# CGLemon/Sayuri

Hardware: AMD Instinct MI355X
Metric: nn_evals_per_sec (higher is better)
Workload: dtype f16

## Files before the change

include/sayuri_hip.h:

```cpp
#ifndef SAYURI_HIP_H
#define SAYURI_HIP_H

#include <stddef.h>
#include <stdint.h>

#ifdef __cplusplus
extern "C" {
#endif

typedef struct sayuri_hip_ctx sayuri_hip_ctx;

enum {
    SAYURI_ACT_IDENTITY = 0, SAYURI_ACT_RELU = 1, SAYURI_ACT_ELU = 2, SAYURI_ACT_SELU = 3,
    SAYURI_ACT_GELU = 4, SAYURI_ACT_MISH = 5, SAYURI_ACT_SWISH = 6, SAYURI_ACT_HARDSWISH = 7
};

enum {
    SAYURI_BLOCK_RESIDUAL = 1, SAYURI_BLOCK_BOTTLENECK = 2, SAYURI_BLOCK_NESTED_BOTTLENECK = 3,
    SAYURI_BLOCK_MIXER = 4
};

typedef struct {
    int32_t type;
    int32_t apply_se;
// ... 42 lines not shown
enum { SAYURI_HIP_LATENCY = 1 };
sayuri_hip_ctx* sayuri_hip_create_ex(int device, const sayuri_hip_netdesc* desc, int max_batch,
                                     int board, int use_fp16, unsigned flags);

int sayuri_hip_load_tensor(sayuri_hip_ctx* ctx, int layer_id, int kind, const float* host, size_t n);

int sayuri_hip_forward(sayuri_hip_ctx* ctx, int n, const float* planes, const int* board_sizes,
                       float* prob, float* pass, float* misc, float* own);

int sayuri_hip_upload(sayuri_hip_ctx* ctx, int n, const float* planes, const int* board_sizes);
int sayuri_hip_run(sayuri_hip_ctx* ctx);
int sayuri_hip_sync(sayuri_hip_ctx* ctx);
int sayuri_hip_download(sayuri_hip_ctx* ctx, float* prob, float* pass, float* misc, float* own);

int sayuri_hip_submit(sayuri_hip_ctx* ctx, int n, const float* planes, const int* board_sizes, float* prob,
                      float* pass, float* misc, float* own, int* ticket);
int sayuri_hip_forward_packed(sayuri_hip_ctx* ctx, int n, const unsigned* records, int binary_planes, const int* board_sizes,
                              float* prob, float* pass, float* misc, float* own);
int sayuri_hip_submit_packed(sayuri_hip_ctx* ctx, int n, const unsigned* records, int binary_planes, const int* board_sizes,
                             float* prob, float* pass, float* misc, float* own, int* ticket);
int sayuri_hip_forward_packed_symm(sayuri_hip_ctx* ctx, int n, const unsigned* records, int n_records, int binary_planes,
                                   const int* board_sizes, const int* src, const int* symm, float* prob, float* pass,
                                   float* misc, float* own);
int sayuri_hip_submit_packed_symm(sayuri_hip_ctx* ctx, int n, const unsigned* records, int n_records, int binary_planes,
                                  const int* board_sizes, const int* src, const int* symm, float* prob, float* pass,
                                  float* misc, float* own, int* ticket);
int sayuri_hip_wait(sayuri_hip_ctx* ctx, int ticket);
int sayuri_hip_query(sayuri_hip_ctx* ctx, int ticket);

int sayuri_hip_time_runs(sayuri_hip_ctx* ctx, int iters, float* total_ms);

typedef struct {
    char name[48];
    int32_t launches;
    float total_ms;
    double flops;
    double bytes;
} sayuri_hip_kernel_stat;
int sayuri_hip_profile_run(sayuri_hip_ctx* ctx, sayuri_hip_kernel_stat* rows, int cap);

int sayuri_hip_mark_kernel(sayuri_hip_ctx* ctx, const char* name);
int sayuri_hip_timed_stat(sayuri_hip_ctx* ctx, sayuri_hip_kernel_stat* row);

void* sayuri_hip_host_alloc(size_t bytes);
void sayuri_hip_host_free(void* p);

size_t sayuri_hip_device_bytes(const sayuri_hip_ctx* ctx);

int sayuri_hip_last_chains(const sayuri_hip_ctx* ctx);

int sayuri_hip_tower_state(const sayuri_hip_ctx* ctx);

int sayuri_hip_latency_state(const sayuri_hip_ctx* ctx);

void sayuri_hip_destroy(sayuri_hip_ctx* ctx);

const char* sayuri_hip_last_error(void);

int sayuri_hip_test_conv(int device, int use_fp16, int n, const int* board_sizes, int max_board,
                         int cin, int cout, int k, int depthwise, int act, int post_residual,
                         const float* x, const float* w, const float* bias, const float* res,
                         float* y);
int sayuri_hip_test_conv_split(int device, int n, const int* board_sizes, int max_board, int cin, int cout, int act,
                               const float* x, const float* w, const float* bias, const float* res, float* y,
                               int channel_tiles, int strips);
int sayuri_hip_test_last_conv_kind(void);
int sayuri_hip_test_se_unit(int device, int use_fp16, int n, const int* board_sizes, int max_board, int channels,
                            int se_size, int act, const float* x, const float* res, const float* w1, const float* b1,
                            const float* w2, const float* b2, float* y, float* gate);
int sayuri_hip_test_head_tail(int device, int use_fp16, int n, const int* board_sizes, int max_board, int policy_channels,
                              int value_channels, int prob_channels, int pass_outs, int misc_outs, int act,
                              const float* pconv, const float* vconv, const float* const* weights12, float* prob,
                              float* pass, float* misc, float* own);

int sayuri_hip_test_conv_se(int device, int n, const int* board_sizes, int max_board, int channels, int se_size, int act,
                            int via_tower, const float* x, const float* w, const float* bias, const float* res, const float* w1,
                            const float* b1, const float* w2, const float* b2, float* y);
int sayuri_hip_test_last_se_form(void);
int sayuri_hip_test_tower_run(int device, int n, const int* board_sizes, int max_board, int channels, int cin0, int nlayers,
                              const int* act, const int* res_from, const float* w, const float* bias, int se_layer, int se_size,
                              const float* w1, const float* b1, const float* w2, const float* b2, int chain, const float* x,
                              float* y);
int sayuri_hip_test_last_tower_run(int out[3]);
int sayuri_hip_test_conv_sx(int device, int n, const int* board_sizes, int max_board, int channels, int se_size, int act,
                            const float* x, const float* w, const float* bias, const float* res, const float* w1,
                            const float* b1, const float* w2, const float* b2, float* y);
int sayuri_hip_test_last_sx_kts(void);
int sayuri_hip_test_head_board(int device, int n, const int* board_sizes, int max_board, int channels, int policy_channels,
                               int value_channels, int prob_channels, int pass_outs, int misc_outs, int act, const float* trunk,
                               const float* p_w, const float* p_b, const float* v_w, const float* v_b,
                               const float* const* weights12, float* prob, float* pass, float* misc, float* own);

#ifdef __cplusplus
}
#endif
#endif
```

sayuri_amd/_lib.py:

```python
from __future__ import annotations

import ctypes
import os

from . import _build

c_float_p = ctypes.POINTER(ctypes.c_float)
c_int_p = ctypes.POINTER(ctypes.c_int)


class KernelStat(ctypes.Structure):
    _fields_ = [("name", ctypes.c_char * 48), ("launches", ctypes.c_int32), ("total_ms", ctypes.c_float),
                ("flops", ctypes.c_double), ("bytes", ctypes.c_double)]


class BlockDesc(ctypes.Structure):
    _fields_ = [(n, ctypes.c_int32) for n in ("type", "apply_se", "se_size", "bottleneck_channels", "feedforward_channels", "dw_filter")]


class NetDesc(ctypes.Structure):
    _fields_ = [(n, ctypes.c_int32) for n in ("version", "input_channels", "residual_channels", "residual_blocks", "policy_head_channels",
                                              "value_head_channels", "probabilities_channels", "pass_probability_outputs",
                                              "ownership_channels", "value_misc_outputs", "default_act", "policy_head_type",
                                              "policy_dw_filter")] + [("blocks", ctypes.POINTER(BlockDesc))]


def fp(a):
    return a.ctypes.data_as(c_float_p)


def ip(a):
    return a.ctypes.data_as(c_int_p)


_I, _U, _Z, _V, _F, _IP = ctypes.c_int, ctypes.c_uint, ctypes.c_size_t, ctypes.c_void_p, c_float_p, c_int_p
_OUT = [_F] * 4
_STAT = ctypes.POINTER(KernelStat)
_W12 = ctypes.POINTER(c_float_p)
HIP_ABI = {
    "sayuri_hip_device_count": (_I, []),
    "sayuri_hip_create": (_V, [_I, _V, _I, _I, _I]),
    "sayuri_hip_create_ex": (_V, [_I, _V, _I, _I, _I, _U]),
    "sayuri_hip_load_tensor": (_I, [_V, _I, _I, _F, _Z]),
    "sayuri_hip_forward": (_I, [_V, _I, _F, _IP] + _OUT),
    "sayuri_hip_upload": (_I, [_V, _I, _F, _IP]),
    "sayuri_hip_run": (_I, [_V]),
    "sayuri_hip_sync": (_I, [_V]),
    "sayuri_hip_download": (_I, [_V] + _OUT),
    "sayuri_hip_submit": (_I, [_V, _I, _F, _IP] + _OUT + [_IP]),
    "sayuri_hip_forward_packed": (_I, [_V, _I, _V, _I, _IP] + _OUT),
    "sayuri_hip_submit_packed": (_I, [_V, _I, _V, _I, _IP] + _OUT + [_IP]),
    "sayuri_hip_forward_packed_symm": (_I, [_V, _I, _V, _I, _I, _IP, _IP, _IP] + _OUT),
    "sayuri_hip_submit_packed_symm": (_I, [_V, _I, _V, _I, _I, _IP, _IP, _IP] + _OUT + [_IP]),
    "sayuri_hip_wait": (_I, [_V, _I]),
    "sayuri_hip_query": (_I, [_V, _I]),
    "sayuri_hip_time_runs": (_I, [_V, _I, _F]),
    "sayuri_hip_profile_run": (_I, [_V, _STAT, _I]),
    "sayuri_hip_mark_kernel": (_I, [_V, ctypes.c_char_p]),
    "sayuri_hip_timed_stat": (_I, [_V, _STAT]),
    "sayuri_hip_host_alloc": (_V, [_Z]),
    "sayuri_hip_host_free": (None, [_V]),
    "sayuri_hip_device_bytes": (_Z, [_V]),
    "sayuri_hip_last_chains": (_I, [_V]),
    "sayuri_hip_tower_state": (_I, [_V]),
    "sayuri_hip_latency_state": (_I, [_V]),
    "sayuri_hip_destroy": (None, [_V]),
    "sayuri_hip_last_error": (ctypes.c_char_p, []),
    "sayuri_hip_test_conv": (_I, [_I] * 3 + [_IP] + [_I] * 7 + [_F] * 5),
    "sayuri_hip_test_conv_split": (_I, [_I] * 2 + [_IP] + [_I] * 4 + [_F] * 5 + [_I] * 2),
    "sayuri_hip_test_last_conv_kind": (_I, []),
    "sayuri_hip_test_se_unit": (_I, [_I] * 3 + [_IP] + [_I] * 4 + [_F] * 8),
    "sayuri_hip_test_head_tail": (_I, [_I] * 3 + [_IP] + [_I] * 7 + [_F, _F, _W12] + _OUT),
    "sayuri_hip_test_conv_se": (_I, [_I] * 2 + [_IP] + [_I] * 5 + [_F] * 9),
    "sayuri_hip_test_last_se_form": (_I, []),
    "sayuri_hip_test_tower_run": (_I, [_I] * 2 + [_IP] + [_I] * 4 + [_IP, _IP, _F, _F, _I, _I] + [_F] * 4 + [_I, _F, _F]),
    "sayuri_hip_test_last_tower_run": (_I, [_IP]),
    "sayuri_hip_test_conv_sx": (_I, [_I] * 2 + [_IP] + [_I] * 4 + [_F] * 9),
    "sayuri_hip_test_last_sx_kts": (_I, []),
    "sayuri_hip_test_head_board": (_I, [_I] * 2 + [_IP] + [_I] * 8 + [_F] * 5 + [_W12] + _OUT),
}
HIP_SYMBOLS = list(HIP_ABI)

_hip = None
_host = None


def _require(path: str) -> str:
    if not os.path.exists(path):
        raise RuntimeError(
            f"native library {path} is missing: run `python -c 'import __graft_entry__ as g; g.build()'` "
            "(there is no CPU fallback for the MI355X forward pipe)")
    return path


def hip() -> ctypes.CDLL:
    global _hip
    if _hip is None:
        path = _build.HIP_SO
        fake = os.environ.get("SAYURI_FAKE_HIP_LIB")
        if fake:
            import sys
            print(f"[sayuri_amd] SAYURI_FAKE_HIP_LIB is set: the device side is the test stand-in {fake}, NOT the MI355X engine",
                  file=sys.stderr)
            path = fake
        lib = ctypes.CDLL(_require(path), mode=ctypes.RTLD_GLOBAL)
        for name, (restype, argtypes) in HIP_ABI.items():
            if hasattr(lib, name):
                fn = getattr(lib, name)
                fn.restype, fn.argtypes = restype, argtypes
        _hip = lib
    return _hip


def host() -> ctypes.CDLL:
    global _host
    if _host is None:
        hip()
        lib = ctypes.CDLL(_require(_build.HOST_SO))
        lib.sayuri_host_last_error.restype = ctypes.c_char_p
        lib.sayuri_weights_load.restype = ctypes.c_void_p
        lib.sayuri_weights_load.argtypes = [ctypes.c_char_p]
        lib.sayuri_weights_free.argtypes = [ctypes.c_void_p]
        lib.sayuri_weights_info.argtypes = [ctypes.c_void_p, c_int_p]
        lib.sayuri_weights_block_info.argtypes = [ctypes.c_void_p, ctypes.c_int, c_int_p]
        lib.sayuri_weights_tensor.restype = ctypes.c_long
        lib.sayuri_weights_tensor.argtypes = [ctypes.c_void_p, ctypes.c_char_p, c_float_p, ctypes.c_long]
        lib.sayuri_pipe_create.restype = ctypes.c_void_p
        lib.sayuri_pipe_create.argtypes = [ctypes.c_char_p, ctypes.c_int, ctypes.c_int, ctypes.c_int, ctypes.c_int,
                                           ctypes.c_int]
        lib.sayuri_pipe_create_ex.restype = ctypes.c_void_p
        lib.sayuri_pipe_create_ex.argtypes = [ctypes.c_char_p, ctypes.c_int, ctypes.c_int, ctypes.c_int, ctypes.c_int,
                                              ctypes.c_int, ctypes.c_uint]
        lib.sayuri_pipe_create_ens.restype = ctypes.c_void_p
        lib.sayuri_pipe_create_ens.argtypes = [ctypes.c_char_p, ctypes.c_int, ctypes.c_int, ctypes.c_int, ctypes.c_int,
                                               ctypes.c_int, ctypes.c_uint, ctypes.c_int]
        lib.sayuri_pipe_accepts_ensemble.argtypes = [ctypes.c_void_p]
        lib.sayuri_pipe_ensemble_fallbacks.restype = ctypes.c_long
        lib.sayuri_pipe_ensemble_fallbacks.argtypes = [ctypes.c_void_p]
        lib.sayuri_pipe_forward_ensemble.argtypes = [ctypes.c_void_p, c_float_p, ctypes.c_int, ctypes.c_float, ctypes.c_int, c_float_p]
        lib.sayuri_pipe_ensemble_mix.argtypes = [ctypes.c_void_p, ctypes.c_int, c_float_p, c_int_p, c_float_p, c_int_p, c_int_p,
                                                 ctypes.c_int, c_float_p, c_int_p]
        lib.sayuri_packed_symmetry.argtypes = [ctypes.c_void_p, ctypes.c_int, ctypes.c_int, ctypes.c_int, ctypes.c_void_p]
        lib.sayuri_pipe_destroy.argtypes = [ctypes.c_void_p]
        lib.sayuri_pipe_num_workers.argtypes = [ctypes.c_void_p]
        lib.sayuri_pipe_ctx.restype = ctypes.c_void_p
        lib.sayuri_pipe_ctx.argtypes = [ctypes.c_void_p, ctypes.c_int]
        lib.sayuri_pipe_reconstruct.argtypes = [ctypes.c_void_p, ctypes.c_int, ctypes.c_int]
        lib.sayuri_pipe_eval.argtypes = [ctypes.c_void_p, ctypes.c_int, ctypes.c_int, ctypes.c_int, c_float_p,
                                         c_int_p, c_float_p, c_int_p, c_float_p]
        lib.sayuri_pipe_pump_times.restype = None
        lib.sayuri_pipe_pump_times.argtypes = [ctypes.c_void_p, ctypes.POINTER(ctypes.c_double),
                                               ctypes.POINTER(ctypes.c_long), ctypes.POINTER(ctypes.c_long)]
        lib.sayuri_pipe_netbench.argtypes = [ctypes.c_void_p, ctypes.c_int, ctypes.c_double, ctypes.c_int,
                                             ctypes.POINTER(ctypes.c_double), ctypes.POINTER(ctypes.c_long)]
        _host = lib
    return _host
```

sayuri_amd/csrc/hip/conv_board.h:

```cpp
#pragma once
#include "common.h"
#include "conv_glds.h"
#include "conv_mfma.h"
#include "small_ops.h"

namespace sayuri {

constexpr int kBoardCols = 24;
constexpr int kBoardPT = kBoardCols * 16;
constexpr int kBoardMaxPos = 512;
constexpr int kBoardMaxSub = 32;
constexpr int kBoardNJ = kBoardCols / 2;
constexpr int kBoardLdsBytes = 160 * 1024;
constexpr int kBoardWaveLds = kBoardLdsBytes / 8;

__host__ __device__ constexpr int board_row_channel(int row) {
    return (row & ~31) + 8 * ((row & 15) >> 2) + 4 * ((row >> 4) & 1) + (row & 3);
}

struct BoardParams {
    ConvParams c;
    const int* tab_src;
    const int2* tab_pix;
    const int* tab_cols;
    int npos;
    int uniform_info;
    unsigned long long* dbg;
    int arith;
    const void* w_next;
    int w_ready;
    int row_order;
};

struct BoardPack {
    int px = 0, pos = 0, cnt = 0, bs0 = 0;
    __host__ __device__ bool fits(int bs) const {
        return (cnt == 0 || bs == bs0) && cnt < kBoardMaxSub && px + bs * bs <= kBoardPT &&
               pos + (bs + 2) * (bs + 2) <= kBoardMaxPos;
    }
    __host__ __device__ void add(int bs) { px += bs * bs; pos += (bs + 2) * (bs + 2); ++cnt; bs0 = bs; }
};

__global__ __launch_bounds__(256) void board_setup_kernel(BatchGeom g, int npos, int* __restrict__ tab_src,
                                                          int2* __restrict__ tab_pix, int* __restrict__ tab_cols) {
    __shared__ int sub[kBoardMaxSub][4];
    __shared__ int hdr[2];
    const int tile = blockIdx.x, tid = threadIdx.x;
    if (tid == 0) {
        int t = 0, s = 0;
        BoardPack pk;
        int cnt = 0;
        for (; s < g.n_samples; ++s) {
            const int bs = g.bsz[s];
            if (pk.cnt > 0 && !pk.fits(bs)) {
                if (t == tile) break;
                ++t;
                pk = BoardPack{};
            }
            if (t == tile) {
                sub[cnt][0] = pk.pos; sub[cnt][1] = pk.px; sub[cnt][2] = bs; sub[cnt][3] = s;
                ++cnt;
            }
            pk.add(bs);
        }
        hdr[0] = cnt;
        hdr[1] = cnt > 0 ? sub[cnt - 1][1] + sub[cnt - 1][2] * sub[cnt - 1][2] : 0;
        tab_cols[tile] = ((hdr[1] + 15) / 16) | (sub[0][2] << 8);
    }
    __syncthreads();
    const int nsub = hdr[0], npx = hdr[1];
    for (int pos = tid; pos < npos; pos += blockDim.x) {
        int src = -1;
        for (int s = 0; s < nsub; ++s) {
            const int bs = sub[s][2], w2 = bs + 2, rel = pos - sub[s][0];
            if (rel >= 0 && rel < w2 * w2) {
                const int r = rel / w2, xc = rel - r * w2;
                const int y = r - 1, x = xc - 1;
                if (y >= 0 && y < bs && x >= 0 && x < bs) src = sub[s][3] * g.slot_pix + y * bs + x;
                break;
            }
        }
        tab_src[(size_t)tile * npos + pos] = src;
    }
    for (int i = tid; i < kBoardPT; i += blockDim.x) {
        int lstr = sub[0][2] + 2, lpos = lstr + 1, orow = -1;
        if (i < npx) {
            for (int s = 0; s < nsub; ++s) {
                const int bs = sub[s][2], pp = i - sub[s][1];
                if (pp >= 0 && pp < bs * bs) {
                    const int y = pp / bs, x = pp - y * bs;
                    lstr = bs + 2;
                    lpos = sub[s][0] + (y + 1) * (bs + 2) + x + 1;
                    orow = sub[s][3] * g.slot_pix + pp;
                    break;
                }
            }
        }
        tab_pix[(size_t)tile * kBoardPT + i] = make_int2(lpos | (lstr << 16), orow);
    }
}

template <int WMT_> struct BoardCfg {
    static constexpr int WMT = WMT_, WAVM = 4, WAVN = 2, NWAVE = 8, NJ = kBoardNJ;
    static constexpr int KO_T = WAVM * WMT * 16;
    static constexpr int A_TAP_BYTES = KO_T * 64;
    static constexpr int A_BYTES = 3 * A_TAP_BYTES;
    static constexpr int A_INSTR = KO_T / 16;
    static constexpr int AI = (A_INSTR + NWAVE - 1) / NWAVE;
    static constexpr int KO_PARTS = KO_T / 64;
    static constexpr size_t ring_bytes(int npos) { return 2 * (size_t)A_BYTES + 2 * (size_t)npos * 64; }
    static constexpr size_t lds_bytes(int npos) { return ring_bytes(npos) <= kBoardLdsBytes ? kBoardLdsBytes : ring_bytes(npos); }
};

#ifndef SAYURI_DROP_STREAM
#define SAYURI_DROP_STREAM 0
#endif
template <int OFF> __device__ __forceinline__ void board_read_a(f16x8& dst, uint32_t addr) {
    if constexpr (SAYURI_DROP_STREAM == 1) asm volatile("" : "+v"(dst) : "v"(addr));
    else ds_read16<OFF>(dst, addr);
}
template <int OFF> __device__ __forceinline__ void board_read_b(f16x8& dst, uint32_t addr) {
    if constexpr (SAYURI_DROP_STREAM == 2) asm volatile("" : "+v"(dst) : "v"(addr));
    else ds_read16<OFF>(dst, addr);
}

namespace board_sched {
constexpr int kNB = 3 * kBoardNJ;
template <int WMT> constexpr int late_a(int b) { return (b >= 0 && b % kBoardNJ == kBoardNJ - 1 && b / kBoardNJ < 2) ? WMT : 0; }
template <int WMT> constexpr int young_b(int b) {
    if (b < 2) return 2;
    return late_a<WMT>(b - 2) + (b + 1 < kNB ? 1 : 0) + late_a<WMT>(b - 1) + (b + 2 < kNB ? 1 : 0);
}
}

template <int N> __device__ __forceinline__ void wait_lgkm1(f16x8& a) {
    asm volatile("s_waitcnt lgkmcnt(%1)" : "+v"(a) : "n"(N));
}
template <int N> __device__ __forceinline__ void wait_lgkm2(f16x8& a, f16x8& b) {
    asm volatile("s_waitcnt lgkmcnt(%2)" : "+v"(a), "+v"(b) : "n"(N));
}
template <int N, int NF, int NA> __device__ __forceinline__ void wait_lgkm_all(f16x8 (&a)[NA], f16x8& b) {
    static_assert(NF >= 2 && NF <= 4 && NF <= NA, "2..4 A fragments per tap");
    if constexpr (NF == 2) asm volatile("s_waitcnt lgkmcnt(%3)" : "+v"(a[0]), "+v"(a[1]), "+v"(b) : "n"(N));
    else if constexpr (NF == 3) asm volatile("s_waitcnt lgkmcnt(%4)" : "+v"(a[0]), "+v"(a[1]), "+v"(a[2]), "+v"(b) : "n"(N));
    else asm volatile("s_waitcnt lgkmcnt(%5)" : "+v"(a[0]), "+v"(a[1]), "+v"(a[2]), "+v"(a[3]), "+v"(b) : "n"(N));
}

__device__ __forceinline__ void swap16(f32x4& a, f32x4& b) {
    float a0 = a[0], a1 = a[1], a2 = a[2], a3 = a[3], b0 = b[0], b1 = b[1], b2 = b[2], b3 = b[3];
    asm("s_nop 1\n\tv_permlane16_swap_b32 %0, %4\n\tv_permlane16_swap_b32 %1, %5\n\tv_permlane16_swap_b32 %2, %6\n\t"
        "v_permlane16_swap_b32 %3, %7"
        : "+v"(a0), "+v"(a1), "+v"(a2), "+v"(a3), "+v"(b0), "+v"(b1), "+v"(b2), "+v"(b3));
    a = f32x4{a0, a1, a2, a3};
    b = f32x4{b0, b1, b2, b3};
}

typedef float f32x2 __attribute__((ext_vector_type(2)));
__device__ __forceinline__ f32x2 mish2(f32x2 x) {
    const f32x2 xl = x * 1.4426950408889634f;
    f32x2 e;
    e[0] = __builtin_amdgcn_exp2f(xl[0]);
    e[1] = __builtin_amdgcn_exp2f(xl[1]);
    const f32x2 t = __builtin_elementwise_fma(e, e + 2.f, f32x2{2.f, 2.f});
    f32x2 r;
    r[0] = __builtin_amdgcn_rcpf(t[0]);
    r[1] = __builtin_amdgcn_rcpf(t[1]);
    return x * __builtin_elementwise_fma(r, f32x2{-2.f, -2.f}, f32x2{1.f, 1.f});
}

__device__ __forceinline__ void mma_agpr(f32x4& acc, const f16x8& a, const f16x8& b) {
    asm volatile("v_mfma_f32_16x16x32_f16 %0, %1, %2, %0" : "+a"(acc) : "v"(a), "v"(b));
}
__device__ __forceinline__ void mma_vgpr(f32x4& acc, const f16x8& a, const f16x8& b) {
    asm volatile("v_mfma_f32_16x16x32_f16 %0, %1, %2, %0" : "+v"(acc) : "v"(a), "v"(b));
}
template <int WMT, int I, int J> __device__ __forceinline__ void mma_tile(f32x4& acc, const f16x8& a, const f16x8& b) {
    if constexpr (WMT * J + I < 32) mma_agpr(acc, a, b);
    else mma_vgpr(acc, a, b);
}

__device__ __forceinline__ void glds16_s(uint32_t voff, const void* sbase, uint32_t lds_dst) {
    unsigned keep;
    asm volatile("s_mov_b32 %0, m0\n\ts_mov_b32 m0, %3\n\ts_nop 4\n\tglobal_load_lds_dwordx4 %1, %2\n\ts_mov_b32 m0, %0"
                 : "=&s"(keep)
                 : "v"(voff), "s"(sbase), "s"(lds_dst)
                 : "memory");
}

__device__ __forceinline__ void gload16_s(f16x8& dst, uint32_t voff, const void* sbase) {
    asm volatile("global_load_dwordx4 %0, %1, %2" : "=v"(dst) : "v"(voff), "s"(sbase) : "memory");
}

template <int N, int ND, int NA> __device__ __forceinline__ void wait_vm_regs(f16x8 (&r)[NA]) {
    static_assert(ND == 0 || ND == 2 || ND == 4, "0, 2 or 4 register pieces");
    if constexpr (ND == 4) asm volatile("s_waitcnt vmcnt(%4)" : "+v"(r[0]), "+v"(r[1]), "+v"(r[2]), "+v"(r[3]) : "n"(N) : "memory");
    else if constexpr (ND == 2) asm volatile("s_waitcnt vmcnt(%2)" : "+v"(r[0]), "+v"(r[1]) : "n"(N) : "memory");
    else asm volatile("s_waitcnt vmcnt(%0)" ::"n"(N) : "memory");
}

template <int WMT, bool DBG = false, int CHAIN = 0>
__device__ __forceinline__ void board_mainloop(const BoardParams& bp, unsigned char* smem, f32x4 (&acc)[WMT][kBoardNJ], int tile,
                                               int kt, int wave, int lane, int col0, bool full, int bs,
                                               unsigned long long* dbg = nullptr,
                                               const __attribute__((address_space(4))) BoardParams* chain = nullptr) {
    using Cfg = BoardCfg<WMT>;
    using namespace board_sched;
    constexpr int KO_T = Cfg::KO_T, NJ = Cfg::NJ, AI = Cfg::AI, NA = WMT;
    const ConvParams& p = bp.c;
    const int npos = bp.npos, b_bytes = npos * 64;
    const uint32_t a_ring = (uint32_t)(uintptr_t)smem;
    const uint32_t b_ring = a_ring + 2 * Cfg::A_BYTES;
    const int wave_m = wave & 3;
    const int kg = lane >> 4;
    const int ls16 = (bs + 2) * 16;

    const unsigned char* gin0 = (const unsigned char*)p.in - kZeroPrefix;
    const unsigned char* gw = (const unsigned char*)p.w;
    const int nbinstr = npos / 64 * 4;
    const int nchunks = p.cin_s / kChunk;
    const int ngroups = nchunks * 3;
    const uint32_t lane16 = lane * 16;
    const size_t tap_stride = (size_t)nchunks * 4 * p.ko_pad * 16;
    const size_t chunk_stride = (size_t)4 * p.ko_pad * 16;
    auto issue_a = [&](int G, int dx, int i) {
        const int q = wave + 8 * i;
        if (q >= Cfg::A_INSTR) return;
        const int kgq = q / Cfg::KO_PARTS, part = q % Cfg::KO_PARTS;
        const int chunk = G / 3, row = G - chunk * 3;
        const unsigned char* base = gw + (size_t)(row * 3 + dx) * tap_stride + (size_t)chunk * chunk_stride +
                                    (size_t)((kgq * p.ko_pad + kt * KO_T + part * 64) * 16);
        glds16_s(lane16, base, a_ring + (G & 1) * Cfg::A_BYTES + dx * Cfg::A_TAP_BYTES + (kgq * KO_T + part * 64) * 16);
    };
    if (!CHAIN || !bp.w_ready) {
#pragma unroll
        for (int dx = 0; dx < 3; ++dx)
#pragma unroll
            for (int i = 0; i < AI; ++i) issue_a(0, dx, i);
    }

    int src[4];
    int lp[NJ];
    if (bp.arith) {
        const int w2 = bs + 2, npix = bs * bs;
        const float r_w2 = __builtin_amdgcn_rcpf((float)w2), r_bs = __builtin_amdgcn_rcpf((float)bs);
#pragma unroll
        for (int i = 0; i < 4; ++i) {
            const int q = wave + 8 * i, pos = (q >> 2) * 64 + lane;
            const int r = (int)(((float)pos + 0.5f) * r_w2), xc = pos - r * w2;
            const bool in = q < nbinstr && r >= 1 && r <= bs && xc >= 1 && xc <= bs;
            src[i] = in ? tile * p.g.slot_pix + (r - 1) * bs + (xc - 1) : -1;
        }
#pragma unroll
        for (int j = 0; j < NJ; ++j) {
            const int px = (col0 + j) * 16 + (lane & 15);
            const int y = (int)(((float)px + 0.5f) * r_bs), x = px - y * bs;
            lp[j] = px < npix ? (y + 1) * w2 + x + 1 : w2 + 1;
        }
    } else {
#pragma unroll
        for (int i = 0; i < 4; ++i) {
            const int q = wave + 8 * i;
            src[i] = q < nbinstr ? bp.tab_src[(size_t)tile * npos + (q >> 2) * 64 + lane] : -1;
        }
#pragma unroll
        for (int j = 0; j < NJ; ++j) lp[j] = bp.tab_pix[(size_t)tile * kBoardPT + (col0 + j) * 16 + (lane & 15)].x;
    }
    f32x4 b4[WMT];
#pragma unroll
    for (int i = 0; i < WMT; ++i) b4[i] = *(const f32x4*)(p.bias + kt * KO_T + (wave_m * WMT + i) * 16 + 4 * kg);

    uint32_t boff[4];
#pragma unroll
    for (int i = 0; i < 4; ++i)
        boff[i] = (src[i] >= 0 ? (uint32_t)kZeroPrefix + (uint32_t)src[i] * (uint32_t)(p.cin_s * 2) : 0u) + ((wave + 8 * i) & 3) * 16;
    auto issue_b = [&](int chunk, int i) {
        const int q = wave + 8 * i;
        if (q >= nbinstr) return;
        glds16_s(boff[i], gin0 + chunk * (kChunk * 2), b_ring + (chunk & 1) * b_bytes + ((q & 3) * npos + (q >> 2) * 64) * 16);
    };
#pragma unroll
    for (int i = 0; i < 4; ++i) issue_b(0, i);

    uint32_t bb[NJ];
#pragma unroll
    for (int j = 0; j < NJ; ++j)
        bb[j] = b_ring + (((uint32_t)lp[j] & 0xffffu) - 1) * 16 + (uint32_t)kg * npos * 16 - ls16;
#pragma unroll
    for (int i = 0; i < WMT; ++i)
#pragma unroll
        for (int j = 0; j < NJ; ++j) acc[i][j] = b4[i];

    const uint32_t arow_off = (uint32_t)((kg * KO_T + wave_m * WMT * 16 + (lane & 15)) * 16);
    unsigned long long t_sync = 0;
    if constexpr (DBG) { if (dbg) dbg[1] = __builtin_amdgcn_s_memtime(); }

    for (int chunk = 0; chunk < nchunks; ++chunk) {
        const bool more_b = chunk + 1 < nchunks;
        static_for<3>([&](auto rowc) {
            constexpr int row = decltype(rowc)::value;
            const int G = chunk * 3 + row;
            unsigned long long t0 = 0;
            if constexpr (DBG) t0 = __builtin_amdgcn_s_memtime();
            wait_vmcnt<0>();
            __builtin_amdgcn_s_barrier();
            if constexpr (DBG) {
                const unsigned long long t1 = __builtin_amdgcn_s_memtime();
                t_sync += t1 - t0;
                if (dbg && G == 0) dbg[2] = t1;
            }
            bool more_a = G + 1 < ngroups;
            int Gn = G + 1;
            if constexpr (CHAIN == 2 && row == 2) {
                if (!more_a) {
                    const __attribute__((address_space(4))) BoardParams* bq = chain;
                    asm volatile("" : "+s"(bq));
                    const unsigned char* wn = (const unsigned char*)bq->w_next;
                    asm volatile("s_waitcnt lgkmcnt(0)" : "+s"(wn)::"memory");
                    if (wn) { gw = wn; Gn = 0; more_a = true; }
                }
            }
            const uint32_t abase = a_ring + (G & 1) * Cfg::A_BYTES + arow_off;
#if SAYURI_DROP_STREAM
            f16x8 afr[NA] = {}, bfr[3] = {};
#else
            f16x8 afr[NA], bfr[3];
#endif
            board_read_b<0>(bfr[0], bb[0]);
            static_for<WMT>([&](auto ic) {
                constexpr int i = decltype(ic)::value;
                board_read_a<i * 256>(afr[i], abase);
            });
            board_read_b<0>(bfr[1], bb[1]);
            static_for<kNB>([&](auto bc) {
                constexpr int b = decltype(bc)::value;
                constexpr int dx = b / NJ, j = b % NJ;
                if constexpr (b % 3 == 0 && b / 3 < 3 * AI) {
                    if (more_a) issue_a(Gn, (b / 3) / AI, (b / 3) % AI);
                }
                if constexpr ((b == 1 || b == 4) && row < 2) {
                    if (more_b) issue_b(chunk + 1, row * 2 + (b == 4 ? 1 : 0));
                }
                if constexpr (b + 2 < kNB) {
                    constexpr int b2 = b + 2;
                    board_read_b<16 * (b2 / NJ)>(bfr[b2 % 3], bb[b2 % NJ]);
                }
                if constexpr (b == 0) wait_lgkm_all<young_b<WMT>(0), WMT>(afr, bfr[0]);
                else if constexpr (j > 0) wait_lgkm1<young_b<WMT>(b)>(bfr[b % 3]);
                static_for<WMT>([&](auto ic) {
                    constexpr int i = decltype(ic)::value;
                    if constexpr (j == 0 && dx > 0) wait_lgkm2<WMT - i>(afr[i], bfr[b % 3]);
                    if constexpr (j == NJ - 1) {
                        if (full) mma_tile<WMT, i, j>(acc[i][j], afr[i], bfr[b % 3]);
                    } else {
                        mma_tile<WMT, i, j>(acc[i][j], afr[i], bfr[b % 3]);
                    }
                    if constexpr (j == NJ - 1 && dx < 2)
                        board_read_a<(dx + 1) * Cfg::A_TAP_BYTES + i * 256>(afr[i], abase);
                });
            });
            const int delta = row < 2 ? ls16 : ((chunk & 1) ? -b_bytes : b_bytes) - 2 * ls16;
#pragma unroll
            for (int j = 0; j < NJ; ++j) bb[j] += (uint32_t)delta;
        });
    }
    asm volatile("s_nop 15\n\ts_nop 15" ::: "memory");
    if constexpr (DBG) { if (dbg) { dbg[3] = __builtin_amdgcn_s_memtime(); dbg[5] = t_sync; } }
}

template <int ACT> __device__ __forceinline__ f16x8 board_act8(const float (&v)[8]) {
    f16x8 h;
    if constexpr (ACT == kMish) {
#pragma unroll
        for (int q = 0; q < 8; q += 2) {
            const f32x2 y = mish2(f32x2{v[q], v[q + 1]});
            h[q] = (f16)y[0];
            h[q + 1] = (f16)y[1];
        }
    } else {
#pragma unroll
        for (int q = 0; q < 8; ++q) h[q] = (f16)activate(v[q], ACT);
    }
    return h;
}

template <int ACT>
__device__ __forceinline__ void board_store_pair(f32x4 a, f32x4 b, bool with_res, const f16x8& rr, unsigned char* __restrict__ gbase,
                                                 uint32_t voff, bool ok) {
    swap16(a, b);
    float v[8] = {a[0], a[1], a[2], a[3], b[0], b[1], b[2], b[3]};
    if (with_res) {
#pragma unroll
        for (int q = 0; q < 8; ++q) v[q] += (float)rr[q];
    }
    const f16x8 h = board_act8<ACT>(v);
    if (ok) *(f16x8*)(gbase + voff) = h;
}

template <int WMT, int ACT>
__device__ __forceinline__ void board_epilogue(const BoardParams& bp, unsigned char* smem, f32x4 (&acc)[WMT][kBoardNJ], int tile, int kt,
                                               int wave, int lane, int col0, int nj) {
    using Cfg = BoardCfg<WMT>;
    constexpr int NJ = Cfg::NJ, NPAIR = WMT / 2;
    constexpr bool LONE = (WMT & 1) != 0;
    const ConvParams& p = bp.c;
    const int R = lane >> 4, px = lane & 15, wave_m = wave & 3;
    const f16* __restrict__ gres = (const f16*)p.res;
    f16* __restrict__ gout = (f16*)p.out;
    const int ko_w = kt * Cfg::KO_T + wave_m * WMT * 16;
    const int2* pix = bp.tab_pix + (size_t)tile * kBoardPT + col0 * 16 + px;
    int cb[NPAIR > 0 ? NPAIR : 1];
#pragma unroll
    for (int pr = 0; pr < NPAIR; ++pr) cb[pr] = ko_w + (2 * pr + (R & 1)) * 16 + (R >> 1) * 8;

    if constexpr (!LONE) {
        constexpr int kWaveLds = kBoardWaveLds, kLdsPieces = kWaveLds / 1024;
        constexpr int kPieces = NJ * NPAIR;
        constexpr int ND = kPieces > kLdsPieces ? kPieces - kLdsPieces : 0;
        static_assert(ND % (NPAIR > 0 ? NPAIR : 1) == 0, "whole column tiles");
        int orow[NJ];
        f16x8 rrd[ND > 0 ? ND : 1];
        const bool with_res = gres != nullptr;
        int row_bytes = p.cout_s * 2;
        asm volatile("" : "+v"(row_bytes));
        uint32_t cb2[NPAIR > 0 ? NPAIR : 1];
        bool cok[NPAIR > 0 ? NPAIR : 1];
#pragma unroll
        for (int pr = 0; pr < NPAIR; ++pr) {
            cb2[pr] = (uint32_t)cb[pr] * 2u;
            cok[pr] = cb[pr] * 2 < row_bytes;
        }
        const uint32_t my_lds = (uint32_t)(uintptr_t)smem + wave * kWaveLds;
        constexpr int JH = NJ / 2, NRT = ND / NPAIR;
        auto load_orow = [&] {
            if (bp.arith) {
                const int npix = (bp.uniform_info >> 8) * (bp.uniform_info >> 8);
#pragma unroll
                for (int j = 0; j < NJ; ++j) {
                    const int pxl = (col0 + j) * 16 + px;
                    orow[j] = (j < nj && pxl < npix) ? tile * p.g.slot_pix + pxl : -1;
                }
            } else {
#pragma unroll
                for (int j = 0; j < NJ; ++j) orow[j] = j < nj ? pix[j * 16].y : -1;
#pragma unroll
                for (int j = 0; j < NJ; ++j) asm volatile("" : "+v"(orow[j]));
            }
        };
        auto lds_slot = [](int j, int pr) { return (j < JH ? j : j - NRT) * NPAIR + pr; };
        if (with_res) {
            asm volatile("s_waitcnt lgkmcnt(0)" ::: "memory");
            __builtin_amdgcn_s_barrier();
            load_orow();
            auto roff = [&](int j, int pr) -> uint32_t {
                return (orow[j] >= 0 && cb[pr] < p.cout_s) ? ((uint32_t)orow[j] * (uint32_t)p.cout_s + (uint32_t)cb[pr]) * 2u : 0u;
            };
            static_for<NJ>([&](auto jc) {
                constexpr int j = decltype(jc)::value;
                if constexpr (j < JH || j >= JH + NRT) {
                    if (j < nj) {
#pragma unroll
                        for (int pr = 0; pr < NPAIR; ++pr) glds16_s(roff(j, pr), gres, my_lds + lds_slot(j, pr) * 1024);
                    }
                }
            });
#pragma unroll
            for (int k = 0; k < ND; ++k)
                if (JH + k / NPAIR < nj) gload16_s(rrd[k], roff(JH + k / NPAIR, k % NPAIR), gres);
            const int late = (nj > JH ? nj - JH : 0) * NPAIR;
            static_for<(NJ - JH) + 1>([&](auto tc) {
                constexpr int t = decltype(tc)::value;
                if (late == t * NPAIR) asm volatile("s_waitcnt vmcnt(%0)" ::"n"(t * NPAIR) : "memory");
            });
        } else {
            load_orow();
        }
        static_for<NJ>([&](auto jc) {
            constexpr int j = decltype(jc)::value;
            if constexpr (j == JH) {
                if (with_res) wait_vm_regs<0, ND>(rrd);
            }
            if (j < nj) {
#pragma unroll
                for (int pr = 0; pr < NPAIR; ++pr) {
                    f16x8 rr = {0, 0, 0, 0, 0, 0, 0, 0};
                    if (with_res) {
                        if constexpr (j >= JH && j < JH + NRT) rr = rrd[(j - JH) * NPAIR + pr];
                        else rr = *(const f16x8*)(smem + wave * kWaveLds + lds_slot(j, pr) * 1024 + lane * 16);
                    }
                    board_store_pair<ACT>(acc[2 * pr][j], acc[2 * pr + 1][j], with_res, rr, (unsigned char*)gout,
                                          __umul24((unsigned)(orow[j] >= 0 ? orow[j] : 0), (unsigned)row_bytes) + cb2[pr], orow[j] >= 0 && cok[pr]);
                }
            }
        });
        return;
    }

    const int cl = ko_w + (WMT - 1) * 16 + 4 * R;
    auto res8 = [&](int orow, int pr) -> f16x8 {
        if (gres && orow >= 0 && cb[pr] < p.cout_s) return *(const f16x8*)(gres + (size_t)orow * p.cout_s + cb[pr]);
        return f16x8{0, 0, 0, 0, 0, 0, 0, 0};
    };
    auto res4 = [&](int orow) -> f16x4 {
        if (gres && orow >= 0 && cl < p.cout_s) return *(const f16x4*)(gres + (size_t)orow * p.cout_s + cl);
        return f16x4{0, 0, 0, 0};
    };
    int orow[3];
    f16x8 rr[2][NPAIR > 0 ? NPAIR : 1];
    f16x4 rl[2];
    orow[0] = nj > 0 ? pix[0].y : -1;
    orow[1] = nj > 1 ? pix[16].y : -1;
#pragma unroll
    for (int pr = 0; pr < NPAIR; ++pr) rr[0][pr] = res8(orow[0], pr);
    rl[0] = res4(orow[0]);
    static_for<NJ>([&](auto jc) {
        constexpr int j = decltype(jc)::value;
        if (j < nj) {
            if constexpr (j + 2 < NJ) orow[(j + 2) % 3] = j + 2 < nj ? pix[(j + 2) * 16].y : -1;
            if constexpr (j + 1 < NJ) {
#pragma unroll
                for (int pr = 0; pr < NPAIR; ++pr) rr[(j + 1) & 1][pr] = res8(orow[(j + 1) % 3], pr);
                rl[(j + 1) & 1] = res4(orow[(j + 1) % 3]);
            }
// ... 180 lines not shown
        __syncthreads();
        if (dbg) dbg[4] = __builtin_amdgcn_s_memtime();
    } else {
        for (int c = tid; c < C; c += 512) {
            const float mean = (psum[c] + psum[KO_T + c]) / npix;
            pool[c] = mean;
            pool[C + c] = mean * (bd / 10.f);
            pool[2 * C + c] = fmaxf(pmax[c], pmax[KO_T + c]);
        }
        __syncthreads();
        se_fc4<U>(sp.squeeze, pool, red, tid);
        __syncthreads();
        for (int o = tid; o < so; o += 512) {
            float a = sp.squeeze.b[o];
            const int parts = 512 / (so / 4);
            for (int k = 0; k < parts; ++k) a += red[k * so + o];
            mid[o] = activate(a, p.act);
        }
        __syncthreads();
        if (dbg) dbg[3] = __builtin_amdgcn_s_memtime();
        se_fc4<U>(sp.excite, mid, red, tid);
        __syncthreads();
        {
            const int eo = sp.excite.out, parts = 512 / (eo / 4);
            for (int o = tid; o < eo; o += 512) {
                float a = sp.excite.b[o];
                for (int k = 0; k < parts; ++k) a += red[k * eo + o];
                gate[o < C ? o : KO_T + (o - C)] = o < C ? 1.0f / (1.0f + fast_exp(-a)) : a;
            }
        }
        __syncthreads();
        if (dbg) dbg[4] = __builtin_amdgcn_s_memtime();
    }
}

template <int WMT>
__device__ __forceinline__ void board_se_gate(const BoardSeParams& sp, unsigned char* smem, f32x4 (&acc)[WMT][kBoardNJ], int wave, int lane) {
    using Cfg = BoardCfg<WMT>;
    constexpr int NJ = Cfg::NJ, KO_T = Cfg::KO_T;
    const int q = lane >> 4, wave_m = wave & 3;
    const int w_bytes = sp.w1h != nullptr ? sp.w1_bytes + sp.w2_bytes : 0;
    const float* gate = (const float*)(smem + w_bytes + SeLds<WMT>::gate);
#pragma unroll
    for (int i = 0; i < WMT; ++i) {
        const int c0 = wave_m * WMT * 16 + i * 16 + 4 * q;
        const f32x4 g = *(const f32x4*)(gate + c0), be = *(const f32x4*)(gate + KO_T + c0);
        static_for<NJ>([&](auto jc) {
            constexpr int j = decltype(jc)::value;
#pragma unroll
            for (int r = 0; r < 4; ++r) acc[i][j][r] = __builtin_fmaf(g[r], acc[i][j][r], be[r]);
        });
    }
}

template <int WMT>
__device__ __forceinline__ void board_se_stage(const BoardSeParams& sp, unsigned char* smem, f32x4 (&acc)[WMT][kBoardNJ], int tile,
                                               int wave, int lane, int col0, int nj, int bs, unsigned long long* dbg = nullptr) {
    board_se_pool<WMT>(sp, smem, acc, tile, wave, lane, col0, nj, bs);
    board_se_fc<WMT>(sp, smem, wave * 64 + lane, bs, dbg);
    board_se_gate<WMT>(sp, smem, acc, wave, lane);
}

template <int WMT>
__global__ __launch_bounds__(512, 2) void conv_board_se_kernel(const BoardSeParams sp) {
    extern __shared__ __attribute__((aligned(16))) unsigned char smem[];
    const BoardParams& bp = sp.b;
    const ConvParams& p = bp.c;
    const int tid = threadIdx.x, lane = tid & 63;
    const int wave = __builtin_amdgcn_readfirstlane(tid >> 6);
    const int tile = blockIdx.x;
    const int info = bp.uniform_info >= 0 ? bp.uniform_info : __builtin_amdgcn_readfirstlane(bp.tab_cols[tile]);
    const int ncols = info & 0xff, bs = info >> 8;
    const int nj0 = (ncols + 1) >> 1;
    const int wave_n = wave >> 2;
    const int col0 = wave_n ? nj0 : 0;
    const int nj = wave_n ? ncols - nj0 : nj0;

    unsigned long long* dbg = nullptr;
    if (bp.dbg && blockIdx.x < 4 && lane == 0) {
        dbg = bp.dbg + ((size_t)blockIdx.x * 8 + wave) * 8;
        dbg[0] = __builtin_amdgcn_s_memtime();
    }
    f32x4 acc[WMT][kBoardNJ];
    board_mainloop<WMT>(bp, smem, acc, tile, 0, wave, lane, col0, nj == kBoardNJ, bs);
    if (dbg) dbg[1] = __builtin_amdgcn_s_memtime();
    board_se_stage<WMT>(sp, smem, acc, tile, wave, lane, col0, nj, bs, dbg);
    asm volatile("s_waitcnt lgkmcnt(0)" ::: "memory");
    __builtin_amdgcn_s_barrier();
    if (dbg) dbg[5] = __builtin_amdgcn_s_memtime();

    switch (p.act) {
    case kMish: board_epilogue<WMT, kMish>(bp, smem, acc, tile, 0, wave, lane, col0, nj); break;
    case kIdentity: board_epilogue<WMT, kIdentity>(bp, smem, acc, tile, 0, wave, lane, col0, nj); break;
    case kReLU: board_epilogue<WMT, kReLU>(bp, smem, acc, tile, 0, wave, lane, col0, nj); break;
    case kSwish: board_epilogue<WMT, kSwish>(bp, smem, acc, tile, 0, wave, lane, col0, nj); break;
    case kELU: board_epilogue<WMT, kELU>(bp, smem, acc, tile, 0, wave, lane, col0, nj); break;
    case kSELU: board_epilogue<WMT, kSELU>(bp, smem, acc, tile, 0, wave, lane, col0, nj); break;
    case kGELU: board_epilogue<WMT, kGELU>(bp, smem, acc, tile, 0, wave, lane, col0, nj); break;
    default: board_epilogue<WMT, kHardSwish>(bp, smem, acc, tile, 0, wave, lane, col0, nj); break;
    }
    if (dbg) {
        asm volatile("s_waitcnt vmcnt(0)" ::: "memory");
        dbg[6] = __builtin_amdgcn_s_memtime();
    }
}

template <int WMT, bool DBG = false>
__global__ __launch_bounds__(512, 2) void conv_board_kernel(const BoardParams bp) {
    extern __shared__ __attribute__((aligned(16))) unsigned char smem[];
    unsigned long long* dbg = nullptr;
    if constexpr (DBG) {
        if (bp.dbg && blockIdx.x < 4 && (threadIdx.x & 63) == 0) {
            dbg = bp.dbg + ((size_t)blockIdx.x * 8 + (threadIdx.x >> 6)) * 8;
            dbg[0] = __builtin_amdgcn_s_memtime();
        }
    }
    const ConvParams& p = bp.c;
    const int tid = threadIdx.x, lane = tid & 63;
    const int wave = __builtin_amdgcn_readfirstlane(tid >> 6);
    const int tile = p.npos + blockIdx.x % p.num_pix_tiles;
    const int kt = blockIdx.x / p.num_pix_tiles;
    const int info = bp.uniform_info >= 0 ? bp.uniform_info : __builtin_amdgcn_readfirstlane(bp.tab_cols[tile]);
    const int ncols = info & 0xff, bs = info >> 8;
    const int nj0 = (ncols + 1) >> 1;
    const int wave_n = wave >> 2;
    const int col0 = wave_n ? nj0 : 0;
    const int nj = wave_n ? ncols - nj0 : nj0;

    f32x4 acc[WMT][kBoardNJ];
    board_mainloop<WMT, DBG>(bp, smem, acc, tile, kt, wave, lane, col0, nj == kBoardNJ, bs, dbg);

    switch (p.act) {
    case kMish: board_epilogue<WMT, kMish>(bp, smem, acc, tile, kt, wave, lane, col0, nj); break;
    case kIdentity: board_epilogue<WMT, kIdentity>(bp, smem, acc, tile, kt, wave, lane, col0, nj); break;
    case kReLU: board_epilogue<WMT, kReLU>(bp, smem, acc, tile, kt, wave, lane, col0, nj); break;
    case kSwish: board_epilogue<WMT, kSwish>(bp, smem, acc, tile, kt, wave, lane, col0, nj); break;
    case kELU: board_epilogue<WMT, kELU>(bp, smem, acc, tile, kt, wave, lane, col0, nj); break;
    case kSELU: board_epilogue<WMT, kSELU>(bp, smem, acc, tile, kt, wave, lane, col0, nj); break;
    case kGELU: board_epilogue<WMT, kGELU>(bp, smem, acc, tile, kt, wave, lane, col0, nj); break;
    default: board_epilogue<WMT, kHardSwish>(bp, smem, acc, tile, kt, wave, lane, col0, nj); break;
    }
    if constexpr (DBG) {
        if (dbg) {
            asm volatile("s_waitcnt vmcnt(0)" ::: "memory");
            dbg[4] = __builtin_amdgcn_s_memtime();
        }
    }
}

}
```

sayuri_amd/csrc/hip/conv_board_sx.h:

```cpp
#pragma once
#include "conv_board.h"

namespace sayuri {

constexpr int kSxMaxSub = 4;
constexpr int kSxSlots = 128;
typedef __attribute__((address_space(1))) unsigned long long sx_gu64;

struct BoardSxParams {
    BoardParams b;
    const void* w1t;
    const void* w2t;
    int w1_bytes, w2_bytes;
    int nsizes;
    int se, kts;
    unsigned long long* xchg;
    unsigned epoch;
    unsigned* err;
    int dbg_stall;
};

struct SxLds {
    static constexpr int kPitch = 68;
    static constexpr int stage = 0, stage_bytes = kBoardPT * kPitch * 4;
    static constexpr int psum = stage + stage_bytes;
    static constexpr int pmax = psum + kSxMaxSub * 8 * 128 * 4;
    static constexpr int red = psum;
    static constexpr int pool = red + kSxMaxSub * 2048 * 4;
    static constexpr int part = pool + kSxMaxSub * 256 * 4;
    static constexpr int mid = part + 4 * kSxMaxSub * 128 * 4;
    static constexpr int gate = mid + kSxMaxSub * 128 * 4;
    static constexpr int end = gate + kSxMaxSub * 256 * 4;
};
static_assert(SxLds::end <= 160 * 1024, "the SE stage must fit the LDS");

__device__ __forceinline__ void sx_barrier() { asm volatile("s_waitcnt lgkmcnt(0)\n\ts_barrier" ::: "memory"); }

template <int WMT>
__global__ __launch_bounds__(512, 2) void conv_board_sx_kernel(const BoardSxParams sp) {
    static_assert(WMT == 2, "128-channel tiles");
    extern __shared__ __attribute__((aligned(16))) unsigned char smem[];
    using Cfg = BoardCfg<WMT>;
    constexpr int NJ = Cfg::NJ;
    const BoardParams& bp = sp.b;
    const ConvParams& p = bp.c;
    const int tid = threadIdx.x, lane = tid & 63;
    const int wave = __builtin_amdgcn_readfirstlane(tid >> 6);
    const int kts = sp.kts;
    const int grp = blockIdx.x / (8 * kts), rem = blockIdx.x - grp * 8 * kts;
    const int kt = rem >> 3, tl = grp * 8 + (rem & 7);
    if (tl >= p.num_pix_tiles) return;
    const int tile = p.npos + tl;
    const int info = bp.uniform_info >= 0 ? bp.uniform_info : __builtin_amdgcn_readfirstlane(bp.tab_cols[tile]);
    const int ncols = info & 0xff, bs = info >> 8;
    const int nj0 = (ncols + 1) >> 1;
    const int wave_m = wave & 3, wave_n = wave >> 2;
    const int col0 = wave_n ? nj0 : 0;
    const int nj = wave_n ? ncols - nj0 : nj0;
    const int npix = bs * bs;
    int nsub = (ncols * 16) / npix;
    nsub = nsub < 1 ? 1 : (nsub > kSxMaxSub ? kSxMaxSub : nsub);

    unsigned long long* dbg = nullptr;
    if (bp.dbg && tid == 0 && (blockIdx.x == 0 || blockIdx.x == 8 || blockIdx.x == 16 || blockIdx.x == 1)) {
        dbg = bp.dbg + (size_t)(blockIdx.x == 1 ? 3 : blockIdx.x >> 3) * 64;
        dbg[0] = __builtin_amdgcn_s_memtime();
    }
    f32x4 acc[WMT][kBoardNJ];
    board_mainloop<WMT>(bp, smem, acc, tile, kt, wave, lane, col0, nj == kBoardNJ, bs);
    if (dbg) dbg[1] = __builtin_amdgcn_s_memtime();

    float* stage = (float*)(smem + SxLds::stage);
    float* psum = (float*)(smem + SxLds::psum);
    float* pmax = (float*)(smem + SxLds::pmax);
    float* pool = (float*)(smem + SxLds::pool);
    float* red = (float*)(smem + SxLds::red);
    float* part = (float*)(smem + SxLds::part);
    float* mid = (float*)(smem + SxLds::mid);
    float* gate = (float*)(smem + SxLds::gate);
    const int q = lane >> 4, px = lane & 15;
    const int se = sp.se;

    const int quads = se >> 2, parts = min(32, 512 / quads);
    const int oq = tid % quads, pt = tid / quads;

    sx_barrier();
    const int per = (npix + 7) >> 3;
#pragma unroll
    for (int half = 0; half < 2; ++half) {
        if ((wave_m >> 1) == half) {
            static_for<NJ>([&](auto jc) {
                constexpr int j = decltype(jc)::value;
                if (j < nj) {
                    const int slot = (col0 + j) * 16 + px;
#pragma unroll
                    for (int i = 0; i < WMT; ++i)
                        *(f32x4*)(stage + slot * SxLds::kPitch + (wave_m & 1) * 32 + i * 16 + 4 * q) = acc[i][j];
                }
            });
        }
        sx_barrier();
        {
            const int c = lane, e = wave;
            const int p0 = e * per, p1 = min(npix, p0 + per);
            for (int s = 0; s < nsub; ++s) {
                const float* src = stage + (s * npix + p0) * SxLds::kPitch + c;
                float a = 0.f, m = -5000.f;
                int pp = p0;
                for (; pp + 8 <= p1; pp += 8) {
                    float v[8];
#pragma unroll
                    for (int u = 0; u < 8; ++u) v[u] = src[u * SxLds::kPitch];
                    src += 8 * SxLds::kPitch;
#pragma unroll
                    for (int u = 0; u < 8; ++u) { a += v[u]; m = max_raw(m, v[u]); }
                }
                for (; pp < p1; ++pp) {
                    const float v = *src;
                    src += SxLds::kPitch;
                    a += v;
                    m = max_raw(m, v);
                }
                psum[(s * 8 + e) * 128 + half * 64 + c] = a;
                pmax[(s * 8 + e) * 128 + half * 64 + c] = m;
            }
        }
        sx_barrier();
    }

    {
        const int n1 = sp.w1_bytes >> 10, n2 = sp.w2_bytes >> 10;
        const unsigned char* g1 = (const unsigned char*)sp.w1t + ((size_t)kt * sp.nsizes + (bs - 2)) * sp.w1_bytes;
        const unsigned char* g2 = (const unsigned char*)sp.w2t + (size_t)kt * sp.w2_bytes;
        const uint32_t l0 = (uint32_t)(uintptr_t)smem;
        for (int k = wave; k < n1; k += 8) glds16_s(lane * 16, g1 + k * 1024, l0 + k * 1024);
        for (int k = wave; k < n2; k += 8) glds16_s(lane * 16, g2 + k * 1024, l0 + sp.w1_bytes + k * 1024);
    }
    {
        const float inv = 1.0f / (float)npix;
        for (int k = tid; k < nsub * 128; k += 512) {
            const int s = k >> 7, c = k & 127;
            const float* a = psum + s * 8 * 128 + c;
            const float* m = pmax + s * 8 * 128 + c;
            float t = a[0], x = m[0];
#pragma unroll
            for (int e = 1; e < 8; ++e) { t += a[e * 128]; x = max_raw(x, m[e * 128]); }
            pool[s * 256 + c] = t * inv;
            pool[s * 256 + 128 + c] = x;
        }
    }
    asm volatile("s_waitcnt vmcnt(0)" ::: "memory");
    sx_barrier();
// ... 124 lines not shown
```

sayuri_amd/csrc/hip/conv_tower.h:

```cpp
#pragma once
#include "conv_board.h"

namespace sayuri {

constexpr int kTowerStride = 320;

struct alignas(16) TowerLayer {
    const TowerLayer* self;
    int last;
    int has_se;
    BoardSeParams sp;
    char pad[kTowerStride - 16 - sizeof(BoardSeParams)];
};
static_assert(sizeof(TowerLayer) == kTowerStride, "tower_seam.py steps the table by kTowerStride bytes");
static_assert(offsetof(TowerLayer, self) == 0, "the compiled bodies load their argument from s[0:1] + 0: the element itself");

typedef const __attribute__((address_space(4))) TowerLayer* TowerLayerCP;
__device__ __forceinline__ TowerLayerCP tower_launder(TowerLayerCP p) {
    asm volatile("" : "+s"(p));
    return p;
}

constexpr int kTowerFreeVgpr = 66;
constexpr int kTowerFreeSgprs = 64;
#define SAYURI_TOWER_CLOBBER_V                                                                                                            \
    "v66", "v67", "v68", "v69", "v70", "v71", "v72", "v73", "v74", "v75", "v76", "v77", "v78", "v79", "v80", "v81", "v82", "v83", "v84",   \
        "v85", "v86", "v87", "v88", "v89", "v90", "v91", "v92", "v93", "v94", "v95", "v96", "v97", "v98", "v99", "v100", "v101", "v102",  \
        "v103", "v104", "v105", "v106", "v107", "v108", "v109", "v110", "v111", "v112", "v113", "v114", "v115", "v116", "v117", "v118",   \
        "v119", "v120", "v121", "v122", "v123", "v124", "v125", "v126", "v127"
#define SAYURI_TOWER_CLOBBER_S                                                                                                            \
    "s0", "s1", "s2", "s3", "s4", "s5", "s6", "s7", "s8", "s9", "s10", "s11", "s12", "s13", "s14", "s15", "s16", "s17", "s18", "s19",     \
        "s20", "s21", "s22", "s23", "s24", "s25", "s26", "s27", "s28", "s29", "s30", "s31", "s32", "s33", "s34", "s35", "s36", "s37",     \
        "s38", "s39", "s40", "s41", "s42", "s43", "s44", "s45", "s46", "s47", "s48", "s49", "s50", "s51", "s52", "s53", "s54", "s55",     \
        "s56", "s57", "s58", "s59", "s60", "s61", "s62", "s63"

template <int WMT, int SIDE, int K> __device__ __forceinline__ void tower_anchor_tile(f32x4& t) {
    constexpr int i = K % WMT, j = K / WMT;
    if constexpr (K < 32) asm volatile("; TOWER_ACC %1 %2 %3 %0" : "+a"(t) : "n"(SIDE), "n"(i), "n"(j));
    else asm volatile("; TOWER_ACC %1 %2 %3 %0" : "+v"(t) : "n"(SIDE), "n"(i), "n"(j));
}
template <int WMT, int SIDE> __device__ __forceinline__ void tower_anchor(f32x4 (&acc)[WMT][kBoardNJ]) {
    static_for<WMT * kBoardNJ>([&](auto kc) {
        constexpr int k = decltype(kc)::value;
        tower_anchor_tile<WMT, SIDE, k>(acc[k % WMT][k / WMT]);
    });
}

template <int WMT>
__global__ __launch_bounds__(512, 2) void conv_tower_kernel(const TowerLayer* layer) {
    extern __shared__ __attribute__((aligned(16))) unsigned char smem[];
    const TowerLayerCP L = (TowerLayerCP)layer;
    const int tid = threadIdx.x, lane = tid & 63;
    const int wave = __builtin_amdgcn_readfirstlane(tid >> 6);
    const int tile = blockIdx.x;
    const int ui = L->sp.b.uniform_info;
    const int info = ui >= 0 ? ui : __builtin_amdgcn_readfirstlane(L->sp.b.tab_cols[tile]);
    const int ncols = info & 0xff, bs = info >> 8;
    const int nj0 = (ncols + 1) >> 1;
    const int wave_n = wave >> 2;
    const int col0 = wave_n ? nj0 : 0;
    const int nj = wave_n ? ncols - nj0 : nj0;

    f32x4 acc[WMT][kBoardNJ];
    {
        const BoardParams& bp = *(const BoardParams*)&L->sp.b;
        board_mainloop<WMT, false, 2>(bp, smem, acc, tile, 0, wave, lane, col0, nj == kBoardNJ, bs, nullptr,
                                      (const __attribute__((address_space(4))) BoardParams*)&L->sp.b);
    }
    TowerLayerCP L2 = L;
    int tid2 = tid;
    tower_anchor<WMT, 0>(acc);
    asm volatile("; TOWER_SE_HOOK elem=%0 tid=%1 wmt=%2 ui=%3 cols=%4 w1h=%5 w2h=%6 w1b=%7 w2b=%8 psum=%9 pmax=%10 gate=%11 kot=%12 "
                 "res=%13 out=%14 couts=%15 slotpix=%16 act=%17 arith=%18 mish=%19 roword=%20 relu=%21 identity=%22 "
                 "stride=%23 last=%24 hasse=%25 freev=%26 frees=%27 nj=%28 epilds=%29 lds=%30"
                 : "+s"(L2), "+v"(tid2)
                 : "n"(WMT), "n"(offsetof(TowerLayer, sp.b.uniform_info)), "n"(offsetof(TowerLayer, sp.b.tab_cols)),
                   "n"(offsetof(TowerLayer, sp.w1h)), "n"(offsetof(TowerLayer, sp.w2h)), "n"(offsetof(TowerLayer, sp.w1_bytes)),
                   "n"(offsetof(TowerLayer, sp.w2_bytes)), "n"(SeLds<WMT>::psum), "n"(SeLds<WMT>::pmax), "n"(SeLds<WMT>::gate),
                   "n"(BoardCfg<WMT>::KO_T), "n"(offsetof(TowerLayer, sp.b.c.res)), "n"(offsetof(TowerLayer, sp.b.c.out)),
                   "n"(offsetof(TowerLayer, sp.b.c.cout_s)), "n"(offsetof(TowerLayer, sp.b.c.g.slot_pix)), "n"(offsetof(TowerLayer, sp.b.c.act)),
                   "n"(offsetof(TowerLayer, sp.b.arith)), "n"((int)kMish), "n"(offsetof(TowerLayer, sp.b.row_order)), "n"((int)kReLU), "n"((int)kIdentity),
                   "n"(kTowerStride), "n"(offsetof(TowerLayer, last)), "n"(offsetof(TowerLayer, has_se)), "n"(kTowerFreeVgpr),
                   "n"(kTowerFreeSgprs), "n"(kBoardNJ), "n"(kBoardWaveLds), "n"(kBoardLdsBytes)
                 : "memory", "vcc", "scc", SAYURI_TOWER_CLOBBER_V, SAYURI_TOWER_CLOBBER_S);
    const BoardSeParams& sp = *(const BoardSeParams*)&L2->sp;
    const BoardParams& bp = sp.b;
    const int lane2 = tid2 & 63, wave2 = __builtin_amdgcn_readfirstlane(tid2 >> 6);
    const int ui2 = bp.uniform_info;
    const int info2 = ui2 >= 0 ? ui2 : __builtin_amdgcn_readfirstlane(bp.tab_cols[tile]);
    const int ncols2 = info2 & 0xff, nj02 = (ncols2 + 1) >> 1;
    const int col02 = (wave2 >> 2) ? nj02 : 0, nj2 = (wave2 >> 2) ? ncols2 - nj02 : nj02;
    switch (bp.c.act) {
    case kMish: board_epilogue<WMT, kMish>(bp, smem, acc, tile, 0, wave2, lane2, col02, nj2); break;
    case kIdentity: board_epilogue<WMT, kIdentity>(bp, smem, acc, tile, 0, wave2, lane2, col02, nj2); break;
    case kReLU: board_epilogue<WMT, kReLU>(bp, smem, acc, tile, 0, wave2, lane2, col02, nj2); break;
    case kSwish: board_epilogue<WMT, kSwish>(bp, smem, acc, tile, 0, wave2, lane2, col02, nj2); break;
    case kELU: board_epilogue<WMT, kELU>(bp, smem, acc, tile, 0, wave2, lane2, col02, nj2); break;
    case kSELU: board_epilogue<WMT, kSELU>(bp, smem, acc, tile, 0, wave2, lane2, col02, nj2); break;
    case kGELU: board_epilogue<WMT, kGELU>(bp, smem, acc, tile, 0, wave2, lane2, col02, nj2); break;
    default: board_epilogue<WMT, kHardSwish>(bp, smem, acc, tile, 0, wave2, lane2, col02, nj2); break;
    }
}

template <int WMT>
__global__ __launch_bounds__(512) void tower_se_fc_kernel(const TowerLayer* layer) {
    extern __shared__ __attribute__((aligned(16))) unsigned char smem[];
    const int tid = threadIdx.x, tile = blockIdx.x;
    const BoardSeParams& sp = layer->sp;
    const int ui = sp.b.uniform_info;
    const int info = ui >= 0 ? ui : __builtin_amdgcn_readfirstlane(sp.b.tab_cols[tile]);
    board_se_fc<WMT, 4>(sp, smem, tid, info >> 8);
}

}
```

sayuri_amd/csrc/hip/engine_graph.h:

```cpp
#pragma once
#include "engine_plan.h"

namespace sayuri {

struct SymmReq {
    int n_records = 0;
    const int* src = nullptr;
    const int* symm = nullptr;
};

class EngineBase {
public:
    virtual ~EngineBase() {}
    virtual int load_tensor(int layer, int kind, const float* host, size_t n) = 0;
    virtual int upload(int n, const float* planes, const int* board_sizes, const unsigned* packed = nullptr, int binary = 0,
                       const SymmReq* sy = nullptr) = 0;
    virtual int run() = 0;
    virtual int sync() = 0;
    virtual int download(float* prob, float* pass, float* misc, float* own) = 0;
    virtual int time_runs(int iters, float* ms) = 0;
    virtual int profile_run(sayuri_hip_kernel_stat* rows, int cap) = 0;
    virtual int submit(int n, const float* planes, const int* bsz, float* prob, float* pass, float* misc, float* own,
                       int* ticket, const unsigned* packed = nullptr, int binary = 0, const SymmReq* sy = nullptr) = 0;
    virtual int wait(int ticket) = 0;
// ... 844 lines not shown
            if (match) {
                group_counts_.back() += 1;
                light_flops_ = flops;
                light_bytes_ = bytes;
            }
            return 0;
        }
        HIP_OK(hipEventRecord(ev0_, f.stream));
        launch();
        HIP_OK(hipGetLastError());
        rows_reset();
        HIP_OK(hipEventRecord(ev1_, f.stream));
        HIP_OK(hipEventSynchronize(ev1_));
        float ms = 0.f;
        HIP_OK(hipEventElapsedTime(&ms, ev0_, ev1_));
        Stat& s = stats_[name];
        s.launches += 1;
        s.ms += ms;
        s.flops += flops;
        s.bytes += bytes;
        return 0;
    }

    int choose_tile(int wmt, int kot_tiles, TileChoice<T>* out) {
        auto it = tile_cache_.find(wmt * 1024 + kot_tiles);
        if (it != tile_cache_.end()) { *out = it->second; return 0; }
        if (!pick_tile<T>(geom_, wmt, kot_tiles, false, out)) return fail("no conv tile configuration fits this batch geometry");
        tile_cache_[wmt * 1024 + kot_tiles] = *out;
        return 0;
    }

    int tile_tabs(Fwd& f, const GldsEntry& e, const TileTabs** out) {
        TileTabs& t = f.io.tabs[e.wnt];
        if (!t.src) {
            const size_t max_tiles = ((size_t)max_batch_ * slot_pix_ + e.pt - 1) / e.pt;
            if (dev_alloc(&t.src, max_tiles * e.npos) || dev_alloc(&t.pix, max_tiles * e.pt)) return -1;
        }
        if (!t.fresh) {
            const int ntiles = (geom_.total + e.pt - 1) / e.pt;
            hipLaunchKernelGGL(e.setup, dim3(ntiles), dim3(256), 0, f.stream, dgeom(f.io), t.src, t.pix);
            HIP_OK(hipGetLastError());
            t.fresh = true;
        }
        *out = &t;
        return 0;
    }
    int board_tabs(Fwd& f, const BoardTabs** out) {
        BoardTabs& t = f.io.board;
        if (!t.src) {
            if (dev_alloc(&t.src, (size_t)max_batch_ * kBoardMaxPos) || dev_alloc(&t.pix, (size_t)max_batch_ * kBoardPT) ||
                dev_alloc(&t.cols, max_batch_))
                return -1;
        }
        if (!t.fresh || t.npos_built != board_plan_.npos || board_plan_.ntiles > t.ntiles_built) {
            hipLaunchKernelGGL(board_setup_kernel, dim3(board_plan_.ntiles), dim3(256), 0, f.stream, dgeom(f.io), board_plan_.npos, t.src,
                               t.pix, t.cols);
            HIP_OK(hipGetLastError());
            t.fresh = true;
            t.npos_built = board_plan_.npos;
            t.ntiles_built = board_plan_.ntiles;
        }
        *out = &t;
        return 0;
    }
    const BoardPlan& plan() {
        if (!board_plan_valid_) { board_plan_ = board_plan(geom_, flags_.conv); board_plan_valid_ = true; }
        return board_plan_;
    }
    const ConvRoute& route(const ConvLayerDev& L) {
        const BoardPlan& bp = plan();
        auto it = route_cache_.find(L.k * 65536 + L.ko_pad);
        if (it == route_cache_.end())
            it = route_cache_.emplace(L.k * 65536 + L.ko_pad, route_conv(sizeof(T) == 2, L.k, L.ko_pad, geom_, bp, flags_.conv, flags_.board_kot, flags_.latency)).first;
        return it->second;
    }

    int board_launch(Fwd& f, const char* name, const ConvLayerDev& L, const BoardEntry* be, BoardFn fn, BoardSeParams& sp, bool has_se,
                     bool to_run, int grid, double flops, double bytes) {
        BoardParams& bp = sp.b;
        ConvParams& p = bp.c;
        if (!f.chained && tower_ok(be->kot) && L.w_board && L.bias_board && board_row_order_ok(bp, be->kot, flags_.tower_gen_epi)) {
            p.w = L.w_board; p.bias = L.bias_board; bp.row_order = 1;
        }
        if (!f.run.empty() && !(to_run && f.run_kot == be->kot) && tower_flush(f)) return -1;
        if (rows_use(f, p, name)) return -1;
        if (to_run) return tower_append(f, be->kot, sp, has_se, flops, bytes);
        const size_t lds = be->lds(board_plan_.npos);
        return timed(f, name, flops, bytes, [&] {
            if (has_se) hipLaunchKernelGGL(be->fn_se, dim3(grid), dim3(512), lds, f.stream, sp);
            else hipLaunchKernelGGL(fn, dim3(grid), dim3(512), lds, f.stream, bp);
        });
    }

    struct SeSplit { int f0, f1, r0, r1; };
    template <typename Rule> SeSplit se_split(const Fwd& f, Rule fused) const {
        int s = 0, tile = 0;
        while (s < geom_.n && fused(geom_.bsz[s])) ++s;
        while (tile < board_plan_.ntiles && board_plan_.tile_first[tile] < s) ++tile;
        const int t1 = f.tile0 + f.ntiles;
        return SeSplit{f.tile0, std::min(t1, tile), std::max(f.tile0, tile), t1};
    }
    int se_tail(Fwd& f, const ConvLayerDev& L, const FcLayerDev& sq, const FcLayerDev& ex, const BoardEntry* be, const BoardParams& bp,
                int kts, int r0, int r1, T* out, const T* res, int C, int act) {
        BoardParams rest = bp;
        rest.row_order = 0;
        rest.c.w = L.w; rest.c.bias = L.bias; rest.c.res = nullptr; rest.c.act = kIdentity;
        rest.c.npos = r0; rest.c.num_pix_tiles = r1 - r0;
        const int s0 = board_plan_.tile_first[r0], s1 = board_plan_.tile_first[r1];
        const ConvCost cost = conv_cost(geom_.off[s1] - geom_.off[s0], L.cin, L.cout, 9, false, sizeof(T));
        const auto fn = be->fn;
        const size_t lds = be->lds(board_plan_.npos);
        const int grid = (r1 - r0) * kts;
        if (timed(f, "conv3x3_tower", cost.flops, cost.bytes, [&] { hipLaunchKernelGGL(fn, dim3(grid), dim3(512), lds, f.stream, rest); }))
            return -1;
        return se_unit(f, sq, ex, out, res, C, round_up(C, 32), act, s0, s1 - s0);
    }

    int conv_se(Fwd& f, const ConvLayerDev& L, const FcLayerDev& sq, const FcLayerDev& ex, const T* in, T* out, const T* res, int C, int act) {
        const bool off = !flags_.se_fused;
        const BoardEntry* be = nullptr;
        if (!off && route(L).board)
            for (const auto& e : kBoardEntries)
                if (e.fn_se && e.kot == L.ko_pad && e.lds(board_plan_.npos) <= kMaxLds) be = &e;
        if (!be || C > be->kot) return 1;
        const bool staged = sq.img16 && ex.img16;
        if (!staged && (sq.out % 4 || sq.out > 512 || ex.out % 4 || ex.out > 2048 || 512 % (sq.out / 4) || 512 % (ex.out / 4))) return 1;
        if constexpr (sizeof(T) != 2) return 1;
        const auto [f0, f1, r0, r1] = se_split(f, [](int bs) { return 2 * bs * bs > kBoardPT; });
        if (f1 <= f0) return 1;
        if (f0 > 0) return fail("chained forward: conv_board_se_kernel starts at tile 0");
        const BoardTabs* tabs = nullptr;
        if (board_tabs(f, &tabs)) return -1;
        BoardSeParams sp;
        std::memset(&sp, 0, sizeof(sp));
        BoardParams& bp = sp.b;
        board_params(bp, board_plan_, tabs->src, tabs->pix, tabs->cols, flags_.arith);
        ConvParams& p = bp.c;
        conv_params(p, in, L.w, L.bias, res, out, dgeom(f.io), L.cin_s, L.cout_s, L.ko_pad, 9, act);
        p.npos = 0; p.num_pix_tiles = f.ntiles;
        sp.squeeze = sq.dev(); sp.excite = ex.dev(); sp.C = C;
        sp.w1h = staged ? sq.img16 : nullptr; sp.w2h = staged ? ex.img16 : nullptr;
        sp.w1_bytes = sq.img_bytes; sp.w2_bytes = ex.img_bytes;
#ifdef SAYURI_EXPERIMENTS
        if (flags_.board_dbg < 0) {
            if (!d_dbg_ && dev_alloc(&d_dbg_, 4 * 8 * 8)) return -1;
            if (++f.dbg_se_call == -flags_.board_dbg) { bp.dbg = d_dbg_; dbg_is_se_ = true; }
        }
#endif
        const ConvCost cost = conv_cost(f.px, L.cin, L.cout, 9, res, sizeof(T));
        const double flops = cost.flops + 2.0 * f.ns * ((double)sq.in * sq.out + (double)ex.in * ex.out);
        const bool to_run = r1 <= r0 && !f.chained && tower_ok(be->kot) && !bp.dbg;
        if (board_launch(f, "conv3x3_tower_se", L, be, be->fn, sp, true, to_run, f1 - f0, flops, cost.bytes)) return -1;
        if (r1 > r0 && se_tail(f, L, sq, ex, be, bp, 1, r0, r1, out, res, C, act)) return -1;
        return 0;
    }

    int conv_sx(Fwd& f, const ConvLayerDev& L, const FcLayerDev& sq, const FcLayerDev& ex, const T* in, T* out, const T* res, int C, int act) {
        if constexpr (sizeof(T) != 2) return 1;
        if (!flags_.se_split || sx_disabled_ || !sq.sx_img || !ex.sx_img || !sx_kts_ || L.ko_pad != sx_kts_ * 128 || L.cout_s != L.ko_pad) return 1;
        if (!route(L).board) return 1;
        const BoardEntry* be = sx_board_entry(board_plan_.npos);
        if (!be) return 1;
        const auto [f0, f1, r0, r1] = se_split(f, sx_board_fused);
        if (!f.run.empty() && tower_flush(f)) return -1;
        const BoardTabs* tabs = nullptr;
        if (board_tabs(f, &tabs)) return -1;
// ... 480 lines not shown
```

sayuri_amd/csrc/hip/engine_plan.h:

```cpp
#pragma once
namespace sayuri {

static thread_local std::string g_err;
static std::atomic<unsigned> g_host_free_gen{0};
static thread_local int g_test_conv_kind = 0;
static int fail(const std::string& m) { g_err = m; return -1; }

#define HIP_OK(expr)                                                                      \
    do {                                                                                  \
        hipError_t e_ = (expr);                                                           \
        if (e_ != hipSuccess) {                                                           \
            g_err = std::string(#expr) + ": " + hipGetErrorString(e_);                    \
            return -1;                                                                    \
        }                                                                                 \
    } while (0)

static inline int round_up(int v, int m) { return (v + m - 1) / m * m; }
constexpr size_t kMaxLds = 160 * 1024;
constexpr int kNumCU = 256;

template <typename T> struct ConvKernelTable {
    typedef void (*Fn)(const ConvParams);
    struct Entry { int wmt, wnt; Fn fn; size_t (*lds)(int); int npos_cap; };
    static std::vector<Entry>& entries() {
        static std::vector<Entry> e;
        return e;
    }
};

template <typename T, int WMT, int WNT> static void register_conv() {
    typedef ConvCfg<T, WMT, WNT> Cfg;
    auto fn = &conv_mfma_kernel<T, WMT, WNT>;
    ConvKernelTable<T>::entries().push_back({WMT, WNT, fn, &Cfg::lds_bytes, Cfg::NPOS_CAP});
}

template <typename T> static void register_all_convs();
template <> void register_all_convs<f16>() {
    if (!ConvKernelTable<f16>::entries().empty()) return;
    register_conv<f16, 1, 4>(); register_conv<f16, 2, 4>(); register_conv<f16, 3, 4>();
    register_conv<f16, 4, 4>(); register_conv<f16, 6, 4>(); register_conv<f16, 8, 4>();
    register_conv<f16, 1, 2>(); register_conv<f16, 2, 2>(); register_conv<f16, 3, 2>();
    register_conv<f16, 4, 2>(); register_conv<f16, 6, 2>(); register_conv<f16, 8, 2>();
    register_conv<f16, 6, 3>(); register_conv<f16, 8, 3>();
}
template <> void register_all_convs<float>() {
    if (!ConvKernelTable<float>::entries().empty()) return;
    register_conv<float, 1, 4>(); register_conv<float, 2, 4>(); register_conv<float, 3, 4>();
    register_conv<float, 4, 4>();
    register_conv<float, 1, 2>(); register_conv<float, 2, 2>(); register_conv<float, 3, 2>();
    register_conv<float, 4, 2>();
}

struct GldsEntry {
    int wmt, wnt;
    void (*fn)(const GldsParams);
    void (*setup)(BatchGeom, int*, int2*);
    size_t lds;
    int npos_cap, npos, pt;
};
static std::vector<GldsEntry>& glds_entries() {
    static std::vector<GldsEntry> e;
    return e;
}
template <int WMT, int WNT> static void register_glds() {
    typedef GldsCfg<WMT, WNT> Cfg;
    glds_entries().push_back({WMT, WNT, &conv_glds_kernel<WMT, WNT>, &tile_setup_kernel<Cfg::PT, Cfg::NPOS>, Cfg::lds_bytes(),
                              Cfg::NPOS_CAP, Cfg::NPOS, Cfg::PT});
}
static void register_all_glds() {
    if (!glds_entries().empty()) return;
    register_glds<8, 3>(); register_glds<8, 2>(); register_glds<8, 1>();
    register_glds<4, 3>(); register_glds<4, 2>(); register_glds<4, 1>();
}
template <typename T> static std::vector<T> board_row_order(const std::vector<T>& img, int ko_pad, int row = 8) {
    std::vector<T> out(img.size());
    const size_t planes = img.size() / ((size_t)ko_pad * row);
    for (size_t pl = 0; pl < planes; ++pl)
        for (int r = 0; r < ko_pad; ++r)
            std::copy_n(img.begin() + (pl * ko_pad + board_row_channel(r)) * row, row, out.begin() + (pl * ko_pad + r) * row);
    return out;
}
static bool board_uses_row_order(int kot) { return (kot / 64) % 2 == 0; }
typedef void (*BoardFn)(const BoardParams);
typedef void (*BoardSeFn)(const BoardSeParams);
struct BoardEntry { int kot; BoardFn fn; BoardSeFn fn_se; size_t (*lds)(int); };
static const BoardEntry kBoardEntries[] = {
    {256, &conv_board_kernel<4>, &conv_board_se_kernel<4>, &BoardCfg<4>::lds_bytes},
    {192, &conv_board_kernel<3>, nullptr, &BoardCfg<3>::lds_bytes},
    {128, &conv_board_kernel<2>, &conv_board_se_kernel<2>, &BoardCfg<2>::lds_bytes},
};
typedef void (*SplitFn)(const SplitParams);
struct SplitEntry { int nj; SplitFn fn; };
static const SplitEntry kSplitEntries[] = {
    {1, &conv_split_kernel<1>}, {2, &conv_split_kernel<2>}, {3, &conv_split_kernel<3>}, {6, &conv_split_kernel<6>}, {12, &conv_split_kernel<12>},
};
typedef void (*HeadFn)(const HeadBoardParams);
struct HeadEntry { int rt, depth; HeadFn fn; };
static const HeadEntry kHeadEntries[] = {
    {2, 5, &head_board_kernel<2, 5>}, {4, 5, &head_board_kernel<4, 5>}, {4, 3, &head_board_kernel<4, 3>},
    {6, 3, &head_board_kernel<6, 3>}, {6, 2, &head_board_kernel<6, 2>},
};
static void enable_big_lds_glds() {
    register_all_glds();
    for (const auto& e : glds_entries())
        (void)hipFuncSetAttribute((const void*)e.fn, hipFuncAttributeMaxDynamicSharedMemorySize, (int)kMaxLds);
    (void)hipFuncSetAttribute((const void*)&conv_board_kernel<4, true>, hipFuncAttributeMaxDynamicSharedMemorySize, (int)kMaxLds);
    for (const auto& e : kHeadEntries) (void)hipFuncSetAttribute((const void*)e.fn, hipFuncAttributeMaxDynamicSharedMemorySize, (int)kMaxLds);
    (void)hipFuncSetAttribute((const void*)&conv_board_sx_kernel<2>, hipFuncAttributeMaxDynamicSharedMemorySize, (int)kMaxLds);
    for (const auto& e : kSplitEntries) (void)hipFuncSetAttribute((const void*)e.fn, hipFuncAttributeMaxDynamicSharedMemorySize, (int)kMaxLds);
    for (const auto& e : kBoardEntries) {
        (void)hipFuncSetAttribute((const void*)e.fn, hipFuncAttributeMaxDynamicSharedMemorySize, (int)kMaxLds);
        if (e.fn_se) (void)hipFuncSetAttribute((const void*)e.fn_se, hipFuncAttributeMaxDynamicSharedMemorySize, (int)kMaxLds);
    }
}
struct ConvOverride {
    bool v0 = false, no_board = false;
    int wnt = 0;
};
struct EngineFlags {
    ConvOverride conv;
    bool tower = true, se_fused = true, heads_fused = true, arith = true;
    bool latency = false;
    int latency_split = 0;
    bool tower_chain = true;
    bool tower_gen_epi = true;
    bool se_split = true;
    int tower_noepi_after = -1;
    unsigned dbg_sx_epoch0 = 0;
    bool dbg_sx_stall = false;
    int sx_dbg = 0;
    int dbg_recycle_input = 0;
    int chains = 0;
    bool chains_serial = false;
    bool tower_sync = false;
    bool fwdstat = false;
    int board_kot = 0;
    int act_override = -1;
    int board_dbg = 0, heads_dbg = 0;
    static bool off(const char* name) { const char* e = getenv(name); return e && atoi(e) == 0; }
    static EngineFlags from_env() {
        EngineFlags f;
        if (const char* e = getenv("SAYURI_CONV")) {
            if (!strncmp(e, "v0", 2)) { f.conv.v0 = true; f.conv.no_board = true; }
            else if (!strncmp(e, "glds", 4)) { f.conv.no_board = true; (void)sscanf(e, "glds:%d", &f.conv.wnt); }
        }
        f.tower = !off("SAYURI_TOWER");
        f.tower_chain = !off("SAYURI_TOWER_CHAIN");
        f.tower_gen_epi = !off("SAYURI_TOWER_GEN_EPI");
        if (const char* e = getenv("SAYURI_DEBUG_RECYCLE_INPUT")) f.dbg_recycle_input = atoi(e);
        f.se_split = !off("SAYURI_SE_SPLIT");
        if (const char* e = getenv("SAYURI_SX_DBG")) f.sx_dbg = atoi(e);
        f.dbg_sx_stall = getenv("SAYURI_DEBUG_SX_STALL") != nullptr;
        if (const char* e = getenv("SAYURI_DEBUG_SX_EPOCH0")) f.dbg_sx_epoch0 = (unsigned)strtoul(e, nullptr, 0);
        if (const char* e = getenv("SAYURI_TOWER_NOEPI_AFTER")) f.tower_noepi_after = atoi(e);
        f.se_fused = !off("SAYURI_SE_FUSED");
        f.heads_fused = !off("SAYURI_HEADS_FUSED");
        f.arith = !getenv("SAYURI_NO_ARITH");
        if (const char* e = getenv("SAYURI_CHAINS")) f.chains = std::max(0, std::min(atoi(e), 4));
        f.chains_serial = getenv("SAYURI_CHAINS_SERIAL") != nullptr;
        f.tower_sync = getenv("SAYURI_TOWER_SYNC") != nullptr;
        f.fwdstat = getenv("SAYURI_HIP_FWDSTAT") != nullptr;
        if (const char* e = getenv("SAYURI_LATENCY_SPLIT")) f.latency_split = std::max(0, atoi(e));
#ifdef SAYURI_EXPERIMENTS
        if (const char* e = getenv("SAYURI_BOARD_KOT")) f.board_kot = atoi(e);
        if (const char* e = getenv("SAYURI_ACT_OVERRIDE")) f.act_override = atoi(e);
        if (const char* e = getenv("SAYURI_BOARD_DBG")) f.board_dbg = atoi(e);
        if (getenv("SAYURI_HEADS_DBG")) f.heads_dbg = 1;
        if (f.board_dbg || f.heads_dbg || f.act_override >= 0) f.tower = false;
#endif
        return f;
    }
    EngineFlags for_latency() const {
        EngineFlags f = *this;
        f.latency = true;
        f.tower = false; f.se_fused = false; f.se_split = false; f.chains = 1;
        return f;
    }
};

template <typename T> static void enable_big_lds() {
    register_all_convs<T>();
    for (const auto& e : ConvKernelTable<T>::entries())
        (void)hipFuncSetAttribute((const void*)e.fn, hipFuncAttributeMaxDynamicSharedMemorySize, (int)kMaxLds);
}

static int pick_wmt(int cout_s, bool fp16) {
    const int opts16[] = {1, 2, 3, 4, 6, 8};
    const int opts32[] = {1, 2, 3, 4};
    const int* opts = fp16 ? opts16 : opts32;
    const int nopts = fp16 ? 6 : 4;
    for (int i = 0; i < nopts; ++i)
        if (opts[i] * 32 >= cout_s) return opts[i];
    int best = opts[nopts - 1], best_pad = 1 << 30;
    for (int i = nopts - 1; i >= 0; --i) {
        const int kot = opts[i] * 32, pad = round_up(cout_s, kot) - cout_s;
        if (pad < best_pad) { best_pad = pad; best = opts[i]; }
    }
    return best;
}

struct HostGeom {
    std::vector<int> bsz, off;
    int n = 0, total = 0;
    void tile_bounds(int PT, int* npos_out, int* nsub_out) const {
        int max_pos = 0, max_sub = 0;
        int s = 0;
        for (int g0 = 0; g0 < total; g0 += PT) {
            const int g1 = std::min(g0 + PT, total);
            while (s + 1 < n && off[s + 1] <= g0) ++s;
            int pos = 0, sub = 0;
            for (int m = s; m < n && off[m] < g1; ++m) {
                const int bs = bsz[m];
                const int a = std::max(g0, off[m]) - off[m], b = std::min(g1, off[m + 1]) - off[m];
                const int rows = (b - 1) / bs - a / bs + 3;
                pos += rows * (bs + 2);
                ++sub;
            }
            max_pos = std::max(max_pos, pos);
            max_sub = std::max(max_sub, sub);
        }
        *npos_out = round_up(std::max(max_pos, 16), 16);
        *nsub_out = max_sub;
    }
};

static bool tile_fits(const HostGeom& geom, int PT, int npos_cap, int* npos) {
    int nsub;
    geom.tile_bounds(PT, npos, &nsub);
    return *npos <= npos_cap && nsub <= kMaxSub;
}
static double tile_cost(const HostGeom& geom, int PT, int kot_tiles, int* ntiles) {
// ... 67 lines not shown
    bp.single = bp.ntiles == geom.n;
    bp.ok = true;
    return bp;
}
static const BoardEntry* pick_board(const BoardPlan& bp, int ko_pad, int* kot_tiles, int force = 0) {
    if (!bp.ok) return nullptr;
    const BoardEntry* best = nullptr;
    long best_cost = 0;
    for (const auto& e : kBoardEntries) {
        if (ko_pad % e.kot != 0 || e.lds(bp.npos) > kMaxLds) continue;
        if (force && force != e.kot) continue;
        const long kts = ko_pad / e.kot, rounds = (bp.ntiles * kts + kNumCU - 1) / kNumCU, cost = rounds * e.kot;
        if (!best || cost < best_cost) { best = &e; best_cost = cost; *kot_tiles = (int)kts; }
    }
    return best;
}
enum ConvFamily { kConvGeneric = 0, kConvGlds = 1, kConvBoard = 2, kConvDepthwise = 3, kConvSplit = 4, kConvBoardSx = 5 };
struct ConvRoute {
    ConvFamily family = kConvGeneric;
    const BoardEntry* board = nullptr;
    const GldsEntry* glds = nullptr;
    int tiles = 0;
};
static ConvRoute route_conv(bool fp16, int k, int ko_pad, const HostGeom& geom, const BoardPlan& plan, const ConvOverride& ov, int force_kot = 0,
                            bool latency = false) {
    ConvRoute r;
    if (!fp16 || k != 3) return r;
    if (latency && ko_pad % kSplitKO == 0) { r.family = kConvSplit; return r; }
    if ((r.board = pick_board(plan, ko_pad, &r.tiles, force_kot))) r.family = kConvBoard;
    else if ((r.glds = pick_glds(geom, ko_pad, &r.tiles, ov))) r.family = kConvGlds;
    return r;
}

constexpr int kSplitAutoMax = 19;
struct SplitPlan {
    bool ok = false;
    int strips = 0, smax = 0, kts = 0, npos = 0, grid = 0;
    const SplitEntry* e = nullptr;
    size_t lds = 0;
};
static int split_auto(int ns, int kts) { return std::max(1, std::min(kSplitAutoMax, kNumCU / std::max(1, ns * kts))); }
static SplitPlan split_plan(const HostGeom& geom, int n0, int ns, int ko_pad, int strips) {
    SplitPlan sp;
    if (ns <= 0 || n0 < 0 || n0 + ns > geom.n || ko_pad <= 0 || ko_pad % kSplitKO) return sp;
    sp.kts = ko_pad / kSplitKO;
    sp.strips = strips > 0 ? strips : split_auto(ns, sp.kts);
    int max_pos = 0, max_cols = 0;
    for (int s = n0; s < n0 + ns; ++s) {
        const int bs = geom.bsz[s], rp = split_rows(bs, sp.strips);
        sp.smax = std::max(sp.smax, (bs + rp - 1) / rp);
        max_pos = std::max(max_pos, (rp + 2) * (bs + 2));
        max_cols = std::max(max_cols, (rp * bs + 15) / 16);
    }
    sp.npos = round_up(max_pos, 64);
    if (sp.npos > kSplitMaxPos || max_cols > kSplitMaxCols) return sp;
    for (const auto& e : kSplitEntries)
        if (!sp.e && 2 * e.nj >= max_cols) sp.e = &e;
    sp.lds = split_lds_bytes(sp.npos);
    sp.grid = ns * sp.smax * sp.kts;
    sp.ok = sp.e != nullptr && sp.lds <= kMaxLds;
    return sp;
}
static void split_params(SplitParams& q, const SplitPlan& sp, int n0) {
    q.c.npos = sp.npos; q.c.num_pix_tiles = 0;
    q.strips = sp.strips; q.smax = sp.smax; q.kts = sp.kts; q.n0 = n0;
}
static void split_launch(const SplitPlan& sp, const SplitParams& q, hipStream_t s) {
    hipLaunchKernelGGL(sp.e->fn, dim3(sp.grid), dim3(256), sp.lds, s, q);
}

static void conv_params(ConvParams& p, const void* in, const void* w, const float* bias, const void* res, void* out, const BatchGeom& g,
                        int cin_s, int cout_s, int ko_pad, int taps, int act) {
    p.in = in; p.w = w; p.bias = bias; p.res = res; p.out = out;
    p.g = g;
    p.cin_s = cin_s; p.cout_s = cout_s; p.ko_pad = ko_pad;
    p.taps = taps; p.act = act;
}
static void board_params(BoardParams& bp, const BoardPlan& plan, const int* tab_src, const int2* tab_pix, const int* tab_cols, bool arith) {
    std::memset(&bp, 0, sizeof(bp));
    bp.tab_src = tab_src; bp.tab_pix = tab_pix; bp.tab_cols = tab_cols;
    bp.npos = plan.npos;
    bp.uniform_info = plan.uniform_info;
    bp.arith = plan.single && plan.uniform_info >= 0 && arith ? 1 : 0;
}
static bool board_row_order_ok(const BoardParams& bp, int kot, bool gen_epi) {
    const ConvParams& p = bp.c;
    return gen_epi && !bp.dbg && board_uses_row_order(kot) && bp.arith && (p.act == kMish || p.act == kReLU || p.act == kIdentity) &&
           p.cout_s == kot && p.ko_pad == kot;
}
static TowerLayer tower_element(const BoardSeParams& sp, bool has_se) {
    TowerLayer t;
    std::memset(&t, 0, sizeof(t));
    t.sp = sp;
    t.has_se = has_se ? 1 : 0;
    ConvParams& c = t.sp.b.c;
    c.num_pix_tiles = 0;
    c.g.n_samples = 0;
    c.g.total_pix = 0;
    return t;
}
static int tower_link(std::vector<TowerLayer>& run, const TowerLayer* dev_base, bool chain) {
    const int n = (int)run.size();
    for (int i = 0; i < n; ++i) {
        run[i].self = dev_base + i;
        run[i].last = i + 1 == n ? 1 : 0;
    }
    int links = 0;
    for (int i = 0; i + 1 < n && chain; ++i) {
        const ConvParams &a = run[i].sp.b.c, &b = run[i + 1].sp.b.c;
        if (run[i].has_se || a.res || a.cin_s != b.cin_s || a.ko_pad != b.ko_pad || (a.cin_s / kChunk) % 2) continue;
        run[i].sp.b.w_next = b.w;
        run[i + 1].sp.b.w_ready = 1;
        ++links;
    }
    return links;
}
static int glds_params(GldsParams& gp, const GldsEntry& e, const int* tab_src, const int2* tab_pix, const float* zeros, int ntiles) {
    gp.tab_src = tab_src; gp.tab_pix = tab_pix; gp.zeros = zeros;
    gp.c.npos = 0; gp.c.num_pix_tiles = ntiles;
    return ntiles * (gp.c.ko_pad / (e.wmt * 32));
}
static bool sx_board_fused(int bs) {
    BoardPack pk;
    int k = 0;
    while (pk.fits(bs)) { pk.add(bs); ++k; }
    return k <= kSxMaxSub;
}
static const BoardEntry* sx_board_entry(int npos) {
    const BoardEntry* be = nullptr;
    for (const auto& e : kBoardEntries)
        if (e.kot == 128 && e.lds(npos) <= kMaxLds) be = &e;
    return be;
}
static void sx_params(BoardSxParams& sp, const void* w1t, const void* w2t, int w1_bytes, int w2_bytes, int board, int se, int kts,
                      unsigned long long* xchg, unsigned epoch, unsigned* err, bool dbg_stall) {
    sp.w1t = w1t; sp.w2t = w2t; sp.w1_bytes = w1_bytes; sp.w2_bytes = w2_bytes;
    sp.nsizes = board - 1; sp.se = se; sp.kts = kts;
    sp.xchg = xchg; sp.epoch = epoch; sp.err = err;
    sp.dbg_stall = dbg_stall ? 1 : 0;
}
static int sx_grid(int tiles, int kts) { return (tiles + 7) / 8 * 8 * kts; }

struct ConvCost { double flops, bytes; };
static ConvCost conv_cost(double px, int cin, int cout, int taps, bool res, size_t elem_bytes) {
    return ConvCost{2.0 * px * cin * cout * taps, elem_bytes * (px * cin + px * cout * (res ? 2 : 1) + (double)cin * cout * taps)};
}

struct Stat {
    int launches = 0;
    float ms = 0.f;
    double flops = 0, bytes = 0;
};

struct ConvLayerDev {
    int cin = 0, cout = 0, k = 0;
    bool depthwise = false;
    std::vector<float> hw, hb;
    int cin_s = 0, cout_s = 0, wmt = 0, ko_pad = 0;
    void* w = nullptr;
    void* w_board = nullptr;
    float* bias_board = nullptr;
    float* bias = nullptr;
    float* w32 = nullptr;
};
struct FcLayerDev {
    int in = 0, out = 0;
// ... 190 lines not shown
```

sayuri_amd/csrc/hip/engine_taps.h:

```cpp
#pragma once
#include "engine_graph.h"

namespace sayuri {

struct TestGeom {
    HostGeom hg;
    int slot = 0;
    int* d_off = nullptr;
    int* d_bsz = nullptr;
    BatchGeom g{};
};

class TestArena {
public:
    ~TestArena() { for (void* p : ptrs_) (void)hipFree(p); }
    void* alloc(size_t bytes) {
        void* p = nullptr;
        if (hipMalloc(&p, std::max<size_t>(bytes, 256)) != hipSuccess) return nullptr;
        (void)hipMemset(p, 0, std::max<size_t>(bytes, 256));
        ptrs_.push_back(p);
        return p;
    }
    template <typename U> U* upload(const std::vector<U>& h) {
        U* d = (U*)alloc(h.size() * sizeof(U));
        if (d && hipMemcpy(d, h.data(), h.size() * sizeof(U), hipMemcpyHostToDevice) != hipSuccess) return nullptr;
        return d;
    }
    template <typename U> U* upload_prefixed(const std::vector<U>& h) {
        U* d = (U*)alloc(h.size() * sizeof(U) + kZeroPrefix);
        if (!d) return nullptr;
        d += kZeroPrefix / sizeof(U);
        return hipMemcpy(d, h.data(), h.size() * sizeof(U), hipMemcpyHostToDevice) == hipSuccess ? d : nullptr;
    }
private:
    std::vector<void*> ptrs_;
};

static int make_test_geom(TestArena& A, int n, const int* board_sizes, int max_board, TestGeom* tg) {
    tg->hg.n = n;
    tg->hg.bsz.assign(board_sizes, board_sizes + n);
    tg->hg.off.assign(n + 1, 0);
    for (int i = 0; i < n; ++i) {
        if (tg->hg.bsz[i] < 2 || tg->hg.bsz[i] > max_board) return fail("test tap: bad board size");
        tg->hg.off[i + 1] = tg->hg.off[i] + tg->hg.bsz[i] * tg->hg.bsz[i];
    }
    tg->hg.total = tg->hg.off[n];
    tg->slot = max_board * max_board;
    tg->d_off = A.upload(tg->hg.off);
    tg->d_bsz = A.upload(tg->hg.bsz);
    if (!tg->d_off || !tg->d_bsz) return fail("test tap: hipMalloc failed");
    tg->g = BatchGeom{tg->d_off, tg->d_bsz, n, tg->hg.total, tg->slot};
    return 0;
}
template <typename T> static std::vector<T> nchw_to_nhwc(const TestGeom& tg, const float* src, int C, int cs) {
    std::vector<T> h((size_t)tg.hg.n * tg.slot * cs, (T)0.f);
    size_t so = 0;
    for (int i = 0; i < tg.hg.n; ++i) {
        const int S = tg.hg.bsz[i] * tg.hg.bsz[i];
        for (int c = 0; c < C; ++c)
            for (int p = 0; p < S; ++p) h[((size_t)i * tg.slot + p) * cs + c] = (T)src[so + (size_t)c * S + p];
        so += (size_t)C * S;
    }
    return h;
}
template <typename T> static int nhwc_to_nchw(const TestGeom& tg, const T* dev, int C, int cs, float* dst) {
    std::vector<T> h((size_t)tg.hg.n * tg.slot * cs);
    HIP_OK(hipMemcpy(h.data(), dev, h.size() * sizeof(T), hipMemcpyDeviceToHost));
    size_t so = 0;
    for (int i = 0; i < tg.hg.n; ++i) {
        const int S = tg.hg.bsz[i] * tg.hg.bsz[i];
        for (int c = 0; c < C; ++c)
            for (int p = 0; p < S; ++p) dst[so + (size_t)c * S + p] = (float)h[((size_t)i * tg.slot + p) * cs + c];
        so += (size_t)C * S;
    }
    return 0;
}
struct TestBoardTabs { int* src; int2* pix; int* cols; };
static bool make_board_tabs(TestArena& A, const TestGeom& tg, const BoardPlan& plan, TestBoardTabs* t) {
    t->src = (int*)A.alloc(sizeof(int) * (size_t)plan.ntiles * plan.npos);
    t->pix = (int2*)A.alloc(sizeof(int2) * (size_t)plan.ntiles * kBoardPT);
    t->cols = (int*)A.alloc(sizeof(int) * (size_t)plan.ntiles);
    if (!t->src || !t->pix || !t->cols) return false;
    hipLaunchKernelGGL(board_setup_kernel, dim3(plan.ntiles), dim3(256), 0, 0, tg.g, plan.npos, t->src, t->pix, t->cols);
    return true;
}

template <typename T>
static int test_conv_impl(int device, int n, const int* board_sizes, int max_board, int cin, int cout, int k,
                          int depthwise, int act, int post_residual, const float* x, const float* w, const float* bias,
                          const float* res, float* y) {
    HIP_OK(hipSetDevice(device));
    enable_big_lds<T>();
    if (sizeof(T) == 2 && k == 3) enable_big_lds_glds();
    TestArena A;
    TestGeom tg;
    if (make_test_geom(A, n, board_sizes, max_board, &tg)) return -1;
    const HostGeom& hg = tg.hg;
    const int cin_s = round_up(depthwise ? cout : cin, 32), cout_s = round_up(cout, 32);
    const T* dx = A.upload_prefixed(nchw_to_nhwc<T>(tg, x, depthwise ? cout : cin, cin_s));
    const T* dres = res ? A.upload(nchw_to_nhwc<T>(tg, res, cout, cout_s)) : nullptr;
    T* dy = (T*)A.alloc((size_t)n * tg.slot * cout_s * sizeof(T));
    if (!dx || !dy || (res && !dres)) return fail("test_conv: hipMalloc failed");
    if (depthwise) {
        g_test_conv_kind = kConvDepthwise;
        const float* dw = A.upload(depthwise_image(w, cout, k * k, cout_s));
        const float* db = A.upload(padded_bias(bias, cout, cout_s));
        if (!dw || !db) return fail("test_conv: hipMalloc failed");
        const size_t total = (size_t)hg.total * (cout_s / ElemTraits<T>::kPieceElems);
        hipLaunchKernelGGL(depthwise_kernel<T>, dim3((unsigned)((total + 255) / 256)), dim3(256), 0, 0, dx, post_residual ? dres : (const T*)nullptr,
                           dy, dw, db, tg.g, cout, cout_s, k, act);
    } else {
        int wmt, ko_pad;
        conv_tile(cout_s, sizeof(T) == 2, &wmt, &ko_pad);
        const T* dw = A.upload(conv_image<T>(w, cin, cout, k * k, ko_pad));
        const float* db = A.upload(padded_bias(bias, cout, ko_pad));
        if (!dw || !db) return fail("test_conv: hipMalloc failed");
        const ConvOverride ov = EngineFlags::from_env().conv;
        const BoardPlan plan = board_plan(hg, ov);
        const ConvRoute r = route_conv(sizeof(T) == 2, k, ko_pad, hg, plan, ov);
        g_test_conv_kind = r.family;
        if (r.board) {
            TestBoardTabs tabs;
            if (!make_board_tabs(A, tg, plan, &tabs)) return fail("test_conv: hipMalloc failed");
            BoardParams bp;
            board_params(bp, plan, tabs.src, tabs.pix, tabs.cols, true);
            conv_params(bp.c, dx, dw, db, dres, dy, tg.g, cin_s, cout_s, ko_pad, 9, act);
            bp.c.npos = 0; bp.c.num_pix_tiles = plan.ntiles;
            hipLaunchKernelGGL(r.board->fn, dim3(plan.ntiles * r.tiles), dim3(512), r.board->lds(plan.npos), 0, bp);
        } else if (r.glds) {
            const float* dz = (const float*)A.alloc(256);
            int* tsrc = (int*)A.alloc(sizeof(int) * (size_t)r.tiles * r.glds->npos);
            int2* tpix = (int2*)A.alloc(sizeof(int2) * (size_t)r.tiles * r.glds->pt);
            if (!dz || !tsrc || !tpix) return fail("test_conv: hipMalloc failed");
            hipLaunchKernelGGL(r.glds->setup, dim3(r.tiles), dim3(256), 0, 0, tg.g, tsrc, tpix);
            GldsParams gp;
            conv_params(gp.c, dx, dw, db, dres, dy, tg.g, cin_s, cout_s, ko_pad, 9, act);
            const int grid = glds_params(gp, *r.glds, tsrc, tpix, dz, r.tiles);
            hipLaunchKernelGGL(r.glds->fn, dim3(grid), dim3(512), r.glds->lds, 0, gp);
        } else {
            TileChoice<T> tc;
            if (!pick_tile<T>(hg, wmt, ko_pad / (wmt * 32), true, &tc)) return fail("test_conv: no tile configuration fits");
            ConvParams p;
            conv_params(p, dx, dw, db, dres, dy, tg.g, cin_s, cout_s, ko_pad, k * k, act);
            p.npos = tc.npos; p.num_pix_tiles = tc.ntiles;
            hipLaunchKernelGGL(tc.e->fn, dim3(tc.ntiles * (ko_pad / (wmt * 32))), dim3(512), tc.e->lds(tc.npos), 0, p);
        }
    }
    HIP_OK(hipGetLastError());
    HIP_OK(hipDeviceSynchronize());
    return nhwc_to_nchw(tg, dy, cout, cout_s, y);
}

static int test_conv_split_impl(int device, int n, const int* board_sizes, int max_board, int cin, int cout, int act, const float* x,
                                const float* w, const float* bias, const float* res, float* y, int channel_tiles, int strips) {
    typedef f16 T;
    HIP_OK(hipSetDevice(device));
    enable_big_lds_glds();
    TestArena A;
    TestGeom tg;
    if (make_test_geom(A, n, board_sizes, max_board, &tg)) return -1;
    const int cin_s = round_up(cin, 32), cout_s = round_up(cout, 32);
    int wmt, ko_pad;
    conv_tile(cout_s, true, &wmt, &ko_pad);
    const ConvRoute r = route_conv(true, 3, ko_pad, tg.hg, BoardPlan{}, ConvOverride{}, 0, true);
    if (r.family != kConvSplit) return fail("test_conv_split: a layer of " + std::to_string(ko_pad) + " weight rows is not whole 64-channel tiles: it keeps the default route");
    if (channel_tiles && channel_tiles != ko_pad / kSplitKO)
        return fail("test_conv_split: the split kernel's channel tile is 64: this layer has " + std::to_string(ko_pad / kSplitKO) + " channel tiles");
    if (strips < 0) return fail("test_conv_split: bad strip count");
    const SplitPlan sp = split_plan(tg.hg, 0, n, ko_pad, strips);
    if (!sp.ok) return fail("test_conv_split: no split fits this batch geometry");
    const T* dx = A.upload_prefixed(nchw_to_nhwc<T>(tg, x, cin, cin_s));
    const T* dres = res ? A.upload(nchw_to_nhwc<T>(tg, res, cout, cout_s)) : nullptr;
    T* dy = (T*)A.alloc((size_t)n * tg.slot * cout_s * sizeof(T));
    const T* dw = A.upload(conv_image<T>(w, cin, cout, 9, ko_pad));
    const float* db = A.upload(padded_bias(bias, cout, ko_pad));
    if (!dx || !dy || (res && !dres) || !dw || !db) return fail("test_conv_split: hipMalloc failed");
    g_test_conv_kind = kConvSplit;
    SplitParams q;
    std::memset(&q, 0, sizeof(q));
    conv_params(q.c, dx, dw, db, dres, dy, tg.g, cin_s, cout_s, ko_pad, 9, act);
    split_params(q, sp, 0);
    split_launch(sp, q, nullptr);
    HIP_OK(hipGetLastError());
    HIP_OK(hipDeviceSynchronize());
    return nhwc_to_nchw(tg, dy, cout, cout_s, y);
}

template <typename T>
static int test_se_unit_impl(int device, int n, const int* board_sizes, int max_board, int C, int se, int act, const float* x,
                             const float* res, const float* w1, const float* b1, const float* w2, const float* b2, float* y,
                             float* gate_out) {
    HIP_OK(hipSetDevice(device));
    TestArena A;
    TestGeom tg;
    if (make_test_geom(A, n, board_sizes, max_board, &tg)) return -1;
    const int cs = round_up(C, 32);
    T* dx = A.upload(nchw_to_nhwc<T>(tg, x, C, cs));
    T* dres = res ? A.upload(nchw_to_nhwc<T>(tg, res, C, cs)) : nullptr;
    float* dw1 = A.upload(fc_transposed(w1, 3 * C, se));
    float* dw2 = A.upload(fc_transposed(w2, se, 2 * C));
    float* db1 = A.upload(std::vector<float>(b1, b1 + se));
    float* db2 = A.upload(std::vector<float>(b2, b2 + 2 * C));
    float* separt = (float*)A.alloc(sizeof(float) * (size_t)n * kSeSplit * 2 * cs);
    float* gate = (float*)A.alloc(sizeof(float) * (size_t)n * 2 * cs);
    if (!dx || (res && !dres) || !dw1 || !dw2 || !db1 || !db2 || !separt || !gate) return fail("test_se_unit: hipMalloc failed");
    if (se_unit_launches<T>(nullptr, tg.g, tg.hg.total, dx, dres, separt, gate, FcDev{dw1, db1, 3 * C, se}, FcDev{dw2, db2, se, 2 * C}, C, cs, act, 0, n,
                            [](const char*, double, double, auto&& launch) { launch(); return 0; }))
        return -1;
    HIP_OK(hipGetLastError());
    HIP_OK(hipDeviceSynchronize());
// ... 67 lines not shown
    HIP_OK(hipDeviceSynchronize());
    return o.download(prob, pass, misc, own);
}

static thread_local int g_test_se_form = 0;
static int test_conv_se_impl(int device, int n, const int* board_sizes, int max_board, int C, int se, int act, int via_tower,
                             const float* x, const float* w, const float* bias, const float* res, const float* w1, const float* b1,
                             const float* w2, const float* b2, float* y) {
    typedef f16 T;
    g_test_se_form = 0;
    HIP_OK(hipSetDevice(device));
    enable_big_lds_glds();
    TestArena A;
    TestGeom tg;
    if (make_test_geom(A, n, board_sizes, max_board, &tg)) return -1;
    const int cs = round_up(C, 32);
    int wmt, ko_pad;
    conv_tile(cs, true, &wmt, &ko_pad);
    const BoardPlan plan = board_plan(tg.hg, ConvOverride{});
    const BoardEntry* be = nullptr;
    if (plan.ok)
        for (const auto& e : kBoardEntries)
            if (e.fn_se && e.kot == ko_pad && e.lds(plan.npos) <= kMaxLds) be = &e;
    if (!be || !plan.single || C > be->kot) return 1;
    std::vector<f16> img1;
    std::vector<unsigned char> img2;
    int w1_bytes = 0, w2_bytes = 0;
    const bool staged = make_se_images(C, se, max_board, w1, b1, w2, b2, &img1, &img2, &w1_bytes, &w2_bytes);
    if (!staged && (se % 4 || se > 512 || (2 * C) % 4 || 512 % (se / 4) || 512 % (2 * C / 4))) return 1;
    const T* dx = A.upload_prefixed(nchw_to_nhwc<T>(tg, x, C, cs));
    const T* dres = res ? A.upload(nchw_to_nhwc<T>(tg, res, C, cs)) : nullptr;
    T* dy = (T*)A.alloc((size_t)n * tg.slot * cs * sizeof(T));
    TestBoardTabs tabs;
    if (!dx || (res && !dres) || !dy || !make_board_tabs(A, tg, plan, &tabs)) return fail("test_conv_se: hipMalloc failed");
    BoardSeParams sp;
    std::memset(&sp, 0, sizeof(sp));
    BoardParams& bp = sp.b;
    board_params(bp, plan, tabs.src, tabs.pix, tabs.cols, true);
    ConvParams& p = bp.c;
    conv_params(p, dx, nullptr, nullptr, dres, dy, tg.g, cs, cs, ko_pad, 9, act);
    p.num_pix_tiles = plan.ntiles;
    bp.row_order = via_tower && board_row_order_ok(bp, be->kot, !EngineFlags::off("SAYURI_TOWER_GEN_EPI")) ? 1 : 0;
    const std::vector<T> img = conv_image<T>(w, C, C, 9, ko_pad);
    const std::vector<float> hb = padded_bias(bias, C, ko_pad);
    p.w = A.upload(bp.row_order ? board_row_order(img, ko_pad) : img);
    p.bias = A.upload(bp.row_order ? board_row_order(hb, ko_pad, 1) : hb);
    sp.squeeze = FcDev{A.upload(fc_transposed(w1, 3 * C, se)), A.upload(std::vector<float>(b1, b1 + se)), 3 * C, se};
    sp.excite = FcDev{A.upload(fc_transposed(w2, se, 2 * C)), A.upload(std::vector<float>(b2, b2 + 2 * C)), se, 2 * C};
    sp.C = C;
    sp.w1h = staged ? A.upload(img1) : nullptr;
    sp.w2h = staged ? A.upload(img2) : nullptr;
    sp.w1_bytes = w1_bytes; sp.w2_bytes = w2_bytes;
    if (!p.w || !p.bias || !sp.squeeze.wt || !sp.squeeze.b || !sp.excite.wt || !sp.excite.b || (staged && (!sp.w1h || !sp.w2h)))
        return fail("test_conv_se: hipMalloc failed");
    hipModule_t mod = nullptr;
    g_test_se_form = sp.w1h ? 1 : 2;
    if (via_tower) {
        hipFunction_t fn[2] = {nullptr, nullptr};
        if (load_tower_module(&mod, fn)) return -1;
        TowerLayer t;
        std::memset(&t, 0, sizeof(t));
        TowerLayer* dt = (TowerLayer*)A.alloc(sizeof(TowerLayer));
        if (!dt) return fail("test_conv_se: hipMalloc failed");
        t.self = dt; t.last = 1; t.has_se = 1; t.sp = sp;
        HIP_OK(hipMemcpy(dt, &t, sizeof(t), hipMemcpyHostToDevice));
        const TowerLayer* arg = dt;
        void* params[] = {(void*)&arg};
        HIP_OK(hipModuleLaunchKernel(fn[be->kot == 256 ? 0 : 1], plan.ntiles, 1, 1, 512, 1, 1, 0, nullptr, params, nullptr));
    } else {
        hipLaunchKernelGGL(be->fn_se, dim3(plan.ntiles), dim3(512), be->lds(plan.npos), 0, sp);
    }
    HIP_OK(hipGetLastError());
    HIP_OK(hipDeviceSynchronize());
    if (mod) (void)hipModuleUnload(mod);
    return nhwc_to_nchw(tg, dy, C, cs, y);
}

static thread_local int g_test_tower_run[3] = {0, 0, 0};
struct TestSeUnit { int layer, se; const float *w1, *b1, *w2, *b2; };
static int test_tower_run_impl(int device, int n, const int* board_sizes, int max_board, int C, int cin0, int nlayers, const int* act,
                               const int* res_from, const float* w, const float* bias, const TestSeUnit& se, int chain, const float* x, float* y) {
    typedef f16 T;
    g_test_tower_run[0] = g_test_tower_run[1] = g_test_tower_run[2] = 0;
    g_test_se_form = 0;
    if (C != 128 && C != 256) return fail("test_tower_run: the run's channels are a channel tile of the tower kernel, 128 or 256");
    if (nlayers < 1 || nlayers > 8) return fail("test_tower_run: 1 to 8 layers");
    if (cin0 < 1 || cin0 > 512) return fail("test_tower_run: bad input channel count");
    if (se.layer >= nlayers) return fail("test_tower_run: the SE layer is not a layer of the run");
    for (int l = 0; l < nlayers; ++l) {
        if (act[l] < 0 || act[l] > 7) return fail("test_tower_run: bad activation");
        if (res_from[l] < -1 || res_from[l] > l) return fail("test_tower_run: a layer's residual is the run's input or an earlier layer's output");
        if (res_from[l] == 0 && cin0 != C) return fail("test_tower_run: the run's input has " + std::to_string(cin0) + " channels, a residual has " + std::to_string(C));
    }
    HIP_OK(hipSetDevice(device));
    TestArena A;
    TestGeom tg;
    if (make_test_geom(A, n, board_sizes, max_board, &tg)) return -1;
    const EngineFlags flags = EngineFlags::from_env();
    const int cin0_s = round_up(cin0, 32);
    int wmt, ko_pad;
    conv_tile(C, true, &wmt, &ko_pad);
    const BoardPlan plan = board_plan(tg.hg, ConvOverride{});
    const BoardEntry* be = nullptr;
    if (plan.ok)
        for (const auto& e : kBoardEntries)
            if (e.kot == ko_pad && e.lds(plan.npos) <= kMaxLds) be = &e;
    if (!be) return 1;
    const bool has_unit = se.layer >= 0;
    std::vector<f16> img1;
    std::vector<unsigned char> img2;
    int w1_bytes = 0, w2_bytes = 0;
    bool staged = false;
    if (has_unit) {
        if (!se.w1 || !se.b1 || !se.w2 || !se.b2) return fail("test_tower_run: the SE layer's weights are missing");
        if (!be->fn_se || !plan.single) return fail("test_tower_run: the SE stage needs one sample per tile");
        staged = make_se_images(C, se.se, max_board, se.w1, se.b1, se.w2, se.b2, &img1, &img2, &w1_bytes, &w2_bytes);
        if (!staged && (se.se <= 0 || se.se % 4 || se.se > 512 || (2 * C) % 4 || 512 % (se.se / 4) || 512 % (2 * C / 4)))
            return fail("test_tower_run: no form of the SE stage takes this SE width");
    }
    const size_t act_bytes = (size_t)n * tg.slot * C * sizeof(T);
    const T* dx = A.upload_prefixed(nchw_to_nhwc<T>(tg, x, cin0, cin0_s));
    TestBoardTabs tabs;
    if (!dx || !make_board_tabs(A, tg, plan, &tabs)) return fail("test_tower_run: hipMalloc failed");
    T* out[8];
    for (int l = 0; l < nlayers; ++l) {
        unsigned char* raw = (unsigned char*)A.alloc(act_bytes + kZeroPrefix);
        if (!raw) return fail("test_tower_run: hipMalloc failed");
        out[l] = (T*)(raw + kZeroPrefix);
        HIP_OK(hipMemset(out[l], 0xff, act_bytes));
    }
    std::vector<TowerLayer> run;
    size_t w_off = 0;
    int row_ordered = 0;
    for (int l = 0; l < nlayers; ++l) {
        const int cin = l ? C : cin0, cin_s = l ? C : cin0_s;
        const bool unit = l == se.layer;
        BoardSeParams sp;
        std::memset(&sp, 0, sizeof(sp));
        BoardParams& bp = sp.b;
        board_params(bp, plan, tabs.src, tabs.pix, tabs.cols, flags.arith);
        ConvParams& p = bp.c;
        const T* res = res_from[l] < 0 ? nullptr : res_from[l] == 0 ? dx : out[res_from[l] - 1];
        conv_params(p, l ? out[l - 1] : dx, nullptr, nullptr, res, out[l], tg.g, cin_s, C, ko_pad, 9, act[l]);
        p.npos = 0; p.num_pix_tiles = plan.ntiles;
        bp.row_order = board_row_order_ok(bp, be->kot, flags.tower_gen_epi) ? 1 : 0;
        row_ordered += bp.row_order;
        const std::vector<T> img = conv_image<T>(w + w_off, cin, C, 9, ko_pad);
        const std::vector<float> hb = padded_bias(bias + (size_t)l * C, C, ko_pad);
        w_off += (size_t)C * cin * 9;
        p.w = A.upload(bp.row_order ? board_row_order(img, ko_pad) : img);
        p.bias = A.upload(bp.row_order ? board_row_order(hb, ko_pad, 1) : hb);
        if (!p.w || !p.bias) return fail("test_tower_run: hipMalloc failed");
        if (unit) {
            sp.squeeze = FcDev{A.upload(fc_transposed(se.w1, 3 * C, se.se)), A.upload(std::vector<float>(se.b1, se.b1 + se.se)), 3 * C, se.se};
            sp.excite = FcDev{A.upload(fc_transposed(se.w2, se.se, 2 * C)), A.upload(std::vector<float>(se.b2, se.b2 + 2 * C)), se.se, 2 * C};
            sp.C = C;
            sp.w1h = staged ? A.upload(img1) : nullptr;
            sp.w2h = staged ? A.upload(img2) : nullptr;
            sp.w1_bytes = w1_bytes; sp.w2_bytes = w2_bytes;
            if (!sp.squeeze.wt || !sp.squeeze.b || !sp.excite.wt || !sp.excite.b || (staged && (!sp.w1h || !sp.w2h)))
                return fail("test_tower_run: hipMalloc failed");
        }
        run.push_back(tower_element(sp, unit));
    }
    TowerLayer* dt = (TowerLayer*)A.alloc(sizeof(TowerLayer) * nlayers);
    if (!dt) return fail("test_tower_run: hipMalloc failed");
    const int links = tower_link(run, dt, chain != 0);
    HIP_OK(hipMemcpy(dt, run.data(), sizeof(TowerLayer) * nlayers, hipMemcpyHostToDevice));
    hipModule_t mod = nullptr;
    hipFunction_t fn[2] = {nullptr, nullptr};
    if (load_tower_module(&mod, fn)) return -1;
    if (has_unit) g_test_se_form = staged ? 1 : 2;
    g_test_tower_run[0] = nlayers; g_test_tower_run[1] = row_ordered; g_test_tower_run[2] = links;
    const TowerLayer* arg = dt;
    void* params[] = {(void*)&arg};
    hipError_t rc = hipModuleLaunchKernel(fn[be->kot == 256 ? 0 : 1], plan.ntiles, 1, 1, 512, 1, 1, 0, nullptr, params, nullptr);
    if (rc == hipSuccess) rc = hipGetLastError();
    if (rc == hipSuccess) rc = hipDeviceSynchronize();
    (void)hipModuleUnload(mod);
    if (rc != hipSuccess) return fail(std::string("test_tower_run: ") + hipGetErrorString(rc));
    const size_t per_layer = (size_t)C * tg.hg.total;
    for (int l = 0; l < nlayers; ++l)
        if (nhwc_to_nchw(tg, out[l], C, C, y + l * per_layer)) return -1;
    return 0;
}

struct TestHostWord {
    unsigned *host = nullptr, *dev = nullptr;
    ~TestHostWord() { if (host) (void)hipHostFree(host); }
    bool alloc() {
        if (hipHostMalloc((void**)&host, 64, hipHostMallocMapped) != hipSuccess) { host = nullptr; return false; }
        std::memset(host, 0, 64);
        return hipHostGetDevicePointer((void**)&dev, host, 0) == hipSuccess;
    }
};
static thread_local int g_test_sx_kts = 0;
static int test_conv_sx_impl(int device, int n, const int* board_sizes, int max_board, int C, int se, int act, const float* x,
                             const float* w, const float* bias, const float* res, const float* w1, const float* b1, const float* w2,
                             const float* b2, float* y) {
    typedef f16 T;
    constexpr unsigned kEpoch = 0x5e17u;
    g_test_sx_kts = 0;
    HIP_OK(hipSetDevice(device));
    enable_big_lds_glds();
    TestArena A;
    TestGeom tg;
    if (make_test_geom(A, n, board_sizes, max_board, &tg)) return -1;
    const int cs = round_up(C, 32), kts = round_up(C, 128) / 128;
    int wmt, ko_pad;
    conv_tile(cs, true, &wmt, &ko_pad);
    if (cs != kts * 128 || ko_pad != kts * 128) return 1;
    std::vector<f16> img1;
    std::vector<unsigned char> img2;
    int w1_bytes = 0, w2_bytes = 0;
    if (!make_sx_images(C, se, kts, max_board, w1, b1, w2, b2, &img1, &img2, &w1_bytes, &w2_bytes)) return 1;
    const BoardPlan plan = board_plan(tg.hg, ConvOverride{});
    const BoardEntry* be = plan.ok ? sx_board_entry(plan.npos) : nullptr;
    if (!be) return 1;
    for (int i = 0; i < n; ++i)
        if (!sx_board_fused(tg.hg.bsz[i])) return 1;
    const T* dx = A.upload_prefixed(nchw_to_nhwc<T>(tg, x, C, cs));
    const T* dres = res ? A.upload(nchw_to_nhwc<T>(tg, res, C, cs)) : nullptr;
    T* dy = (T*)A.alloc((size_t)n * tg.slot * cs * sizeof(T));
    const T* dw = A.upload(conv_image<T>(w, C, C, 9, ko_pad));
    const float* db = A.upload(padded_bias(bias, C, ko_pad));
    const f16* d1 = A.upload(img1);
    const unsigned char* d2 = A.upload(img2);
    unsigned long long* xchg = (unsigned long long*)A.alloc(sizeof(unsigned long long) * (size_t)plan.ntiles * kts * kSxMaxSub * kSxSlots);
    TestBoardTabs tabs;
    TestHostWord err;
    if (!dx || (res && !dres) || !dy || !dw || !db || !d1 || !d2 || !xchg || !make_board_tabs(A, tg, plan, &tabs) || !err.alloc())
        return fail("test_conv_sx: hipMalloc failed");
    BoardSxParams sp;
    std::memset(&sp, 0, sizeof(sp));
    board_params(sp.b, plan, tabs.src, tabs.pix, tabs.cols, true);
    conv_params(sp.b.c, dx, dw, db, dres, dy, tg.g, cs, cs, ko_pad, 9, act);
    sp.b.c.npos = 0; sp.b.c.num_pix_tiles = plan.ntiles;
    sx_params(sp, d1, d2, w1_bytes, w2_bytes, max_board, se, kts, xchg, kEpoch, err.dev, false);
    HIP_OK(hipMemset(dy, 0xff, (size_t)n * tg.slot * cs * sizeof(T)));
    g_test_conv_kind = kConvBoardSx;
    g_test_sx_kts = kts;
    hipLaunchKernelGGL(conv_board_sx_kernel<2>, dim3(sx_grid(plan.ntiles, kts)), dim3(512), be->lds(plan.npos), 0, sp);
    HIP_OK(hipGetLastError());
    HIP_OK(hipDeviceSynchronize());
    if (*(volatile unsigned*)err.host) return fail("test_conv_sx: a workgroup's wait for its sibling channel tiles ran out");
    return nhwc_to_nchw(tg, dy, C, cs, y);
}

static int test_head_board_impl(int device, int n, const int* board_sizes, int max_board, int C, int Cp, int Cv, int prob_ch,
                                int pass_outs, int misc_outs, int act, const float* trunk, const float* p_w, const float* p_b,
                                const float* v_w, const float* v_b, const float* const* w, float* prob, float* pass, float* misc,
                                float* own) {
    typedef f16 T;
    HIP_OK(hipSetDevice(device));
    enable_big_lds_glds();
    TestArena A;
    TestGeom tg;
    if (make_test_geom(A, n, board_sizes, max_board, &tg)) return -1;
    HeadImages hi;
    const HeadFn fn = make_head_images(C, Cp, Cv, prob_ch, max_board, p_w, p_b, v_w, v_b, w[8], w[10], &hi);
    if (!fn) return 1;
    const int cs = round_up(C, 32);
    const T* dt = A.upload(nchw_to_nhwc<T>(tg, trunk, C, cs));
    const f16* d_img = A.upload(hi.img);
    const f16* d_img2 = A.upload(hi.img2);
    const float* d_bias = A.upload(hi.bias);
    HeadWeights hw;
    TestHeadOut o;
    if (!dt || !d_img || !d_img2 || !d_bias || !upload_head_weights(A, w, Cp, Cv, prob_ch, pass_outs, misc_outs, &hw) ||
        !o.alloc(A, n, prob_ch, pass_outs, misc_outs, max_board * max_board))
        return fail("test_head_board: hipMalloc failed");
    HeadBoardParams hp;
    std::memset(&hp, 0, sizeof(hp));
    hp.h = head_params(hw, Cp, Cv, prob_ch, act, max_board, o.prob, o.pass, o.misc, o.own, nullptr);
    hp.trunk = dt; hp.w = d_img; hp.w2 = d_img2; hp.bias = d_bias; hp.g = tg.g; hp.cs = cs; hp.PT = hi.PT; hp.VT = hi.VT;
    hipLaunchKernelGGL(fn, dim3(n), dim3(512), kMaxLds, 0, hp);
    HIP_OK(hipGetLastError());
    HIP_OK(hipDeviceSynchronize());
    return o.download(prob, pass, misc, own);
}

}

extern "C" int sayuri_hip_test_conv_se(int device, int n, const int* board_sizes, int max_board, int channels, int se_size, int act,
                                       int via_tower, const float* x, const float* w, const float* bias, const float* res,
                                       const float* w1, const float* b1, const float* w2, const float* b2, float* y) {
    if (!board_sizes || !x || !w || !w1 || !b1 || !w2 || !b2 || !y || n <= 0) return fail("test_conv_se: bad argument");
    return test_conv_se_impl(device, n, board_sizes, max_board, channels, se_size, act, via_tower, x, w, bias, res, w1, b1, w2, b2, y);
}

extern "C" int sayuri_hip_test_conv_sx(int device, int n, const int* board_sizes, int max_board, int channels, int se_size, int act,
                                       const float* x, const float* w, const float* bias, const float* res, const float* w1,
                                       const float* b1, const float* w2, const float* b2, float* y) {
    if (!board_sizes || !x || !w || !w1 || !b1 || !w2 || !b2 || !y || n <= 0) return fail("test_conv_sx: bad argument");
    return test_conv_sx_impl(device, n, board_sizes, max_board, channels, se_size, act, x, w, bias, res, w1, b1, w2, b2, y);
}

extern "C" int sayuri_hip_test_last_se_form(void) { return sayuri::g_test_se_form; }

extern "C" int sayuri_hip_test_tower_run(int device, int n, const int* board_sizes, int max_board, int channels, int cin0, int nlayers,
                                         const int* act, const int* res_from, const float* w, const float* bias, int se_layer, int se_size,
                                         const float* w1, const float* b1, const float* w2, const float* b2, int chain, const float* x,
                                         float* y) {
    if (!board_sizes || !act || !res_from || !w || !bias || !x || !y || n <= 0 || (chain != 0 && chain != 1))
        return fail("test_tower_run: bad argument");
    return test_tower_run_impl(device, n, board_sizes, max_board, channels, cin0, nlayers, act, res_from, w, bias,
                               TestSeUnit{se_layer < 0 ? -1 : se_layer, se_size, w1, b1, w2, b2}, chain, x, y);
}
extern "C" int sayuri_hip_test_last_tower_run(int out[3]) {
    if (!out) return fail("test_last_tower_run: bad argument");
    std::copy(sayuri::g_test_tower_run, sayuri::g_test_tower_run + 3, out);
    return 0;
}

extern "C" int sayuri_hip_test_last_sx_kts(void) { return sayuri::g_test_sx_kts; }

extern "C" int sayuri_hip_test_head_board(int device, int n, const int* board_sizes, int max_board, int channels, int policy_channels,
                                          int value_channels, int prob_channels, int pass_outs, int misc_outs, int act, const float* trunk,
                                          const float* p_w, const float* p_b, const float* v_w, const float* v_b,
                                          const float* const* weights12, float* prob, float* pass, float* misc, float* own) {
    if (!board_sizes || !trunk || !p_w || !p_b || !v_w || !v_b || !weights12 || !prob || !pass || !misc || !own || n <= 0)
        return fail("test_head_board: bad argument");
    return test_head_board_impl(device, n, board_sizes, max_board, channels, policy_channels, value_channels, prob_channels, pass_outs,
                                misc_outs, act, trunk, p_w, p_b, v_w, v_b, weights12, prob, pass, misc, own);
}

extern "C" int sayuri_hip_test_se_unit(int device, int use_fp16, int n, const int* board_sizes, int max_board, int channels, int se_size,
                                       int act, const float* x, const float* res, const float* w1, const float* b1, const float* w2,
                                       const float* b2, float* y, float* gate) {
    if (!board_sizes || !x || !w1 || !b1 || !w2 || !b2 || !y || n <= 0) return fail("test_se_unit: bad argument");
    if (use_fp16) return test_se_unit_impl<f16>(device, n, board_sizes, max_board, channels, se_size, act, x, res, w1, b1, w2, b2, y, gate);
    return test_se_unit_impl<float>(device, n, board_sizes, max_board, channels, se_size, act, x, res, w1, b1, w2, b2, y, gate);
}

extern "C" int sayuri_hip_test_head_tail(int device, int use_fp16, int n, const int* board_sizes, int max_board, int policy_channels,
                                         int value_channels, int prob_channels, int pass_outs, int misc_outs, int act, const float* pconv,
                                         const float* vconv, const float* const* weights12, float* prob, float* pass, float* misc,
                                         float* own) {
    if (!board_sizes || !pconv || !vconv || !weights12 || !prob || !pass || !misc || !own || n <= 0) return fail("test_head_tail: bad argument");
    if (use_fp16)
        return test_head_tail_impl<f16>(device, n, board_sizes, max_board, policy_channels, value_channels, prob_channels, pass_outs,
                                        misc_outs, act, pconv, vconv, weights12, prob, pass, misc, own);
    return test_head_tail_impl<float>(device, n, board_sizes, max_board, policy_channels, value_channels, prob_channels, pass_outs,
                                      misc_outs, act, pconv, vconv, weights12, prob, pass, misc, own);
}

extern "C" int sayuri_hip_test_conv_split(int device, int n, const int* board_sizes, int max_board, int cin, int cout, int act, const float* x,
                                          const float* w, const float* bias, const float* res, float* y, int channel_tiles, int strips) {
    if (!board_sizes || !x || !w || !y || n <= 0) return fail("test_conv_split: bad argument");
    return test_conv_split_impl(device, n, board_sizes, max_board, cin, cout, act, x, w, bias, res, y, channel_tiles, strips);
}

extern "C" int sayuri_hip_test_last_conv_kind(void) { return sayuri::g_test_conv_kind; }

extern "C" int sayuri_hip_test_conv(int device, int use_fp16, int n, const int* board_sizes, int max_board, int cin,
                                    int cout, int k, int depthwise, int act, int post_residual, const float* x,
                                    const float* w, const float* bias, const float* res, float* y) {
    if (!board_sizes || !x || !w || !y || n <= 0) return fail("test_conv: bad argument");
    if (use_fp16)
        return test_conv_impl<f16>(device, n, board_sizes, max_board, cin, cout, k, depthwise, act, post_residual, x, w,
                                   bias, res, y);
    return test_conv_impl<float>(device, n, board_sizes, max_board, cin, cout, k, depthwise, act, post_residual, x, w,
                                 bias, res, y);
}
```

sayuri_amd/csrc/hip/tower_seam.py:

```python
#!/usr/bin/env python3
import argparse
import re
import sys
from types import SimpleNamespace

FC_SGPR_CAP = 40

CONV_RE = re.compile(r"^(_ZN6sayuri17conv_tower_kernelILi(\d+)EEEvPKNS_10TowerLayerE):")
FC_RE = re.compile(r"^(_ZN6sayuri18tower_se_fc_kernelILi(\d+)EEEvPKNS_10TowerLayerE):")

ABI = (("user_sgpr_count", 2), ("user_sgpr_kernarg_segment_ptr", 1), ("system_sgpr_workgroup_id_x", 1),
       ("system_sgpr_workgroup_id_y", 0), ("system_sgpr_workgroup_id_z", 0), ("system_vgpr_workitem_id", 0),
       ("kernarg_size", 8), ("group_segment_fixed_size", 0), ("user_sgpr_kernarg_preload_length", 0),
       ("uses_dynamic_stack", 0), ("private_segment_fixed_size", 0))

HOOK_KEYS = ("elem", "tid", "wmt", "ui", "cols", "w1h", "w2h", "w1b", "w2b", "psum", "pmax", "gate", "kot", "res", "out", "couts",
             "slotpix", "act", "arith", "mish", "relu", "identity", "roword",
             "stride", "last", "hasse", "freev", "frees", "nj", "epilds", "lds")


def die(msg):
    sys.stderr.write("tower_seam.py: " + msg + "\n")
    sys.exit(1)


class Reg:

    def __init__(self, cls, lo, n=1):
        self.cls, self.lo, self.n = cls, lo, n

    def __str__(self):
        return f"{self.cls}{self.lo}" if self.n == 1 else f"{self.cls}[{self.lo}:{self.lo + self.n - 1}]"

    def __getitem__(self, k):
        if isinstance(k, slice):
            return Reg(self.cls, self.lo + k.start, k.stop - k.start)
        return Reg(self.cls, self.lo + k)

    def __iter__(self):
        return (self[k] for k in range(self.n))


def far_jump(sym, t=Reg("s", 4, 2)):
    return [f"\ts_getpc_b64 {t}",
            f"\ts_add_u32 {t[0]}, {t[0]}, {sym}@rel32@lo+4",
            f"\ts_addc_u32 {t[1]}, {t[1]}, {sym}@rel32@hi+12",
            f"\ts_setpc_b64 {t}"]


def is_instruction(ln):
    s = ln.strip()
    return bool(s) and ln.startswith("\t") and not s.startswith(".") and not s.startswith(";")


def rename_vgprs(ln, shift):
    code, sep, comment = ln.partition(";")
    code = re.sub(r"\bv\[(\d+):(\d+)\]", lambda m: f"v[{int(m.group(1)) + shift}:{int(m.group(2)) + shift}]", code)
    code = re.sub(r"\bv(\d+)\b", lambda m: f"v{int(m.group(1)) + shift}", code)
    return code + sep + comment


def max_reg(body, cls):
    hi = -1
    for ln in body:
        code = ln.split(";")[0]
        for m in re.finditer(r"\b%s\[(\d+):(\d+)\]" % cls, code):
            hi = max(hi, int(m.group(2)))
        for m in re.finditer(r"\b%s(\d+)\b" % cls, code):
            hi = max(hi, int(m.group(1)))
    return hi


def quad_channel(i):
    return (i >> 1) * 32 + 4 * (i & 1)


def lds_slot(j, pr, p):
    return (j if j < p.JH else j - p.NRT) * p.npair + pr



class Index:

    def __init__(self, lines):
        self.lines, self.funcs, self.desc, self.meta = lines, {}, {}, {}
        body = block = entry = None
        for k, ln in enumerate(lines):
            if body is None:
                m = CONV_RE.match(ln) or FC_RE.match(ln)
                if m:
                    body = dict(name=m.group(1), begin=k)
                    self.funcs[(int(m.group(2)), "conv" if m.re is CONV_RE else "fc")] = body
            elif ln.startswith("\t.section\t.rodata"):
                body["end"] = k
                body = None
            s = ln.strip()
            if s.startswith(".amdhsa_kernel "):
                block = self.desc.setdefault(s[len(".amdhsa_kernel "):], {})
            elif s == ".end_amdhsa_kernel":
                block = None
            elif block is not None and s.startswith(".amdhsa_"):
# ... 51 lines not shown
    for tok in lines[hooks[0]].split("TOWER_SE_HOOK", 1)[1].split():
        key, _, val = tok.partition("=")
        named[key] = val if key in ("elem", "tid") else int(val, 0)
    for key in HOOK_KEYS:
        if key not in named:
            die(f"{name}: the hook statement names no `{key}`")
    hook = SimpleNamespace(**named)
    if hook.wmt != w:
        die(f"{name}: the hook says wmt={hook.wmt}")
    m = re.match(r"^s\[(\d+):(\d+)\]$", hook.elem)
    if not m or int(m.group(1)) < hook.frees or not re.match(r"^v\d+$", hook.tid) or int(hook.tid[1:]) >= hook.freev:
        die(f"{name}: hook operands {hook.elem} / {hook.tid} sit inside the clobbered ranges")
    hook.elem = Reg("s", int(m.group(1)), int(m.group(2)) - int(m.group(1)) + 1)
    hook.tid = Reg("v", int(hook.tid[1:]))
    if w % 2:
        die("the SE hook is written for even row-tile counts (board_row_channel order)")
    if hook.w2b != hook.w1b + 4:
        die("w1_bytes / w2_bytes are not adjacent in BoardSeParams")
    if epi_pieces(hook).nd % (w // 2):
        die("epilogue: register pieces are not whole column tiles")
    return hooks[0], hook


def check_fc_body(ix, fc, hook):
    name = fc["name"]
    fbody = [ix.lines[k] for k in ix.body(fc)]
    if any(re.search(r"\ba\d+\b|\ba\[\d+:\d+\]|v_accvgpr|v_mfma", ln.split(";")[0]) for ln in fbody):
        die(f"{name}: touches AGPRs (they hold the accumulators)")
    fv, fs = max_reg(fbody, "v"), max_reg(fbody, "s")
    if fv + hook.freev > 127:
        die(f"{name}: v{fv} does not fit behind v{hook.freev} (128 - {hook.freev} VGPRs belong to the hook)")
    if fs >= FC_SGPR_CAP:
        die(f"{name}: s{fs} -- the hook keeps its own values from s{FC_SGPR_CAP} on")
    if any(re.search(r"\bm0\b|ttmp|flat_scratch|s_getpc|s_setpc|s_swappc|s_call", ln.split(";")[0]) for ln in fbody):
        die(f"{name}: uses m0 / calls (not expected in the FC body)")
    return fv


def read_anchors(ix, conv, hk, hook):
    lines, name, w = ix.lines, conv["name"], hook.wmt
    acc, first_anchor = {}, None
    for k in ix.body(conv):
        m = re.search(r"; TOWER_ACC (\d+) (\d+) (\d+) ([av])\[(\d+):(\d+)\]", lines[k])
        if not m:
            continue
        side, ti, tj, kind, lo, hi = int(m.group(1)), int(m.group(2)), int(m.group(3)), m.group(4), int(m.group(5)), int(m.group(6))
        if side != 0 or hi != lo + 3 or (ti, tj) in acc or k > hk:
            die(f"{name}: unexpected anchor {lines[k].strip()!r}")
        if kind == "v" and lo + 3 >= hook.freev:
            die(f"{name}: accumulator tile ({ti}, {tj}) lives in v[{lo}:{hi}], inside the hook's range")
        acc[(ti, tj)] = Reg(kind, lo, 4)
        first_anchor = k if first_anchor is None else first_anchor
    if len(acc) != w * hook.nj:
        die(f"{name}: {len(acc)} anchors for {w * hook.nj} output tiles")
    regs = sorted((t.cls, t.lo) for t in acc.values())
    if any(regs[n][0] == regs[n + 1][0] and regs[n][1] + 4 > regs[n + 1][1] for n in range(len(regs) - 1)):
        die(f"{name}: overlapping accumulator tiles")
    stray = [lines[k].strip() for k in range(first_anchor, hk) if is_instruction(lines[k])]
    if stray:
        die(f"{name}: instructions between the anchors and the hook ({stray[:3]}): the tiles may have moved")
    before = [lines[k].strip() for k in range(conv["begin"] + 1, first_anchor) if is_instruction(lines[k])][-2:]
    if before != ["s_nop 15", "s_nop 15"]:
        die(f"{name}: {before} in front of the anchors, expected the K loop's two s_nop 15")
    written = set()
    for k in range(conv["begin"] + 1, first_anchor):
        m = re.match(r"\tv_mfma_\w+ ([av])\[(\d+):(\d+)\]", lines[k])
        if m:
            written.add((m.group(1), int(m.group(2))))
    if written != set(regs):
        die(f"{name}: the MFMA stream writes {len(written)} tiles, the anchors name {len(set(regs))} (or others)")
    if any(t.cls == "v" and t.lo % 2 for t in acc.values()):
        die("epilogue: an accumulator tile in VGPRs is not even-aligned")
    return acc


def find_exits(ix, conv):
    ends = [k for k in ix.body(conv) if ix.lines[k].strip() == "s_endpgm"]
    if not ends:
        die(f"{conv['name']}: no s_endpgm")
    return ends


def choose_parked(w, conv, fc, fv, hook):
    B = (max(conv["sgprs"], fc["sgprs"]) + 1) & ~1
    if B + 5 > 102:
        die(f"width {w}: no five SGPRs left above the compiler's {B}")
    B = max(B, hook.frees + 2)
    if conv["accum"] < hook.freev + fv + 1:
        die(f"width {w}: accum_offset {conv['accum']} below the FC body's renamed VGPRs")
    s = Reg("s", B, 5)
    return SimpleNamespace(all=s, tab=s[0:2], wg=s[2], wave=s[3], has_se=s[4])



class Emitter:

    def __init__(self, prefix, hook):
        self.lines, self.prefix, self.freev, self.frees = [], prefix, hook.freev, hook.frees
        self.s_keep = FC_SGPR_CAP
        self.release()

    def release(self):
        self.v_next, self.s_low = self.freev, 4

    def __call__(self, text):
        self.lines.append("\t" + text)

    def at(self, name):
        return f"{self.prefix}_{name}"

    def label(self, name):
        self.lines.append(self.at(name) + ":")

    def v(self, n=1, align=1):
        lo = (self.v_next + align - 1) // align * align
        self.v_next = lo + n
        if self.v_next > 128:
            die("the hook ran out of VGPRs")
        return Reg("v", lo, n)

    def s(self, n=1, keep=False):
        lo = ((self.s_keep if keep else self.s_low) + n - 1) // n * n
        if keep:
            self.s_keep = lo + n
            if self.s_keep > self.frees:
                die("the hook ran out of SGPRs")
        else:
            self.s_low = lo + n
            if self.s_low > FC_SGPR_CAP:
                die("the hook ran out of scratch SGPRs")
        return Reg("s", lo, n)


def wave_geometry(e, g, info, wave, t0):
    e(f"s_and_b32 {g.ncols}, {info}, 0xff")
    e(f"s_lshr_b32 {g.bs}, {info}, 8")
    e(f"s_add_u32 {g.nj0}, {g.ncols}, 1")
    e(f"s_lshr_b32 {g.nj0}, {g.nj0}, 1")
    e(f"s_lshr_b32 {g.wave_n}, {wave}, 2")
    e(f"s_and_b32 {g.wave_m}, {wave}, 3")
    e(f"s_sub_u32 {t0}, {g.ncols}, {g.nj0}")
    e(f"s_cmp_eq_u32 {g.wave_n}, 0")
    e(f"s_cselect_b32 {g.col0}, 0, {g.nj0}")
    e(f"s_cselect_b32 {g.nj}, {g.nj0}, {t0}")


def read_tile(e, t, tmp):
    if t.cls == "v":
        return t
    for r in range(4):
        e(f"v_accvgpr_read_b32 {tmp[r]}, {t[r]}")
    return tmp


def se_hook(w, hook, acc, park, fc_label):
    e = Emitter(f".Ltower{w}_se", hook)
    r = SimpleNamespace()
    r.m0 = e.s(keep=True)
    r.w1h, r.w2h = e.s(2, keep=True), e.s(2, keep=True)
    r.wb = e.s(2, keep=True)
    r.wbytes = e.s(keep=True)
    r.wave_m = e.s(keep=True)
    r.info, r.ncols, r.bs, r.nj0, r.wave_n, r.col0, r.nj, r.njm1 = (e.s() for _ in range(8))
    r.t0, r.t1, r.k, r.n = (e.s() for _ in range(4))
    r.p = e.s(2)
    r.valid, r.px0, r.save = e.s(2), e.s(2), e.s(2)
    r.lane, r.lane16, r.px, r.q, r.t, r.addr, r.addr2 = (e.v() for _ in range(7))
    r.ro = e.s(keep=True)
    r.sets = [(e.v(4, 4), e.v(4, 4)) for _ in range(2)]
    r.xs = [e.v(4, 4) for _ in range(2)]

    e(f"; ---- tower_seam.py: the SE unit (width {w}: {hook.wmt} row tiles x {hook.nj} column tiles per wave)")
    e(f"s_cmp_eq_u32 {park.has_se}, 0")
# ... 132 lines not shown
        e(f"ds_write_b128 {r.addr}, {M4} offset:{i * 64 + hook.pmax - hook.psum}")
        e.label(f"pse{i}")
        e(f"s_mov_b64 exec, {r.save}")
    e("s_waitcnt vmcnt(0) lgkmcnt(0)")
    e("s_barrier")


def se_call_fc(e, w, hook, park, fc_label):
    e(f"s_mov_b32 s0, {hook.elem[0]}")
    e(f"s_mov_b32 s1, {hook.elem[1]}")
    e(f"s_mov_b32 s2, {park.wg}")
    e(f"v_mov_b32_e32 v{hook.freev}, {hook.tid}")
    e("s_mov_b64 exec, -1")
    e.lines.extend(far_jump(fc_label))
    e.lines.append(f"tower{w}_se_return:")
    e("s_mov_b64 exec, -1")
    e.release()


def se_gate(e, hook, acc, r):
    wmt, kot = hook.wmt, hook.kot
    g_lane, g_q, g_addr = e.v(), e.v(), e.v()
    gs = [(e.v(4, 4), e.v(4, 4)) for _ in range(wmt)]
    gx = [e.v(4, 4) for _ in range(2)]
    s_t = e.s()
    e(f"v_and_b32_e32 {g_lane}, 63, {hook.tid}")
    e(f"v_lshrrev_b32_e32 {g_q}, 4, {g_lane}")
    e(f"s_mul_i32 {s_t}, {r.wave_m}, {wmt * 16 * 4}")
    e(f"s_add_u32 {s_t}, {s_t}, {r.wbytes}")
    e(f"s_add_u32 {s_t}, {s_t}, {hook.gate}")
    e(f"s_cmp_eq_u32 {r.ro}, 0")
    e(f"s_cbranch_scc1 {e.at('gnat')}")
    e(f"v_lshl_add_u32 {g_addr}, {g_q}, 5, {s_t}")
    for i in range(wmt):
        e(f"ds_read_b128 {gs[i][0]}, {g_addr} offset:{quad_channel(i) * 4}")
        e(f"ds_read_b128 {gs[i][1]}, {g_addr} offset:{quad_channel(i) * 4 + kot * 4}")
    e(f"s_branch {e.at('gread')}")
    e.label("gnat")
    e(f"v_lshl_add_u32 {g_addr}, {g_q}, 4, {s_t}")
    for i in range(wmt):
        e(f"ds_read_b128 {gs[i][0]}, {g_addr} offset:{i * 64}")
        e(f"ds_read_b128 {gs[i][1]}, {g_addr} offset:{i * 64 + kot * 4}")
    e.label("gread")
    e("s_waitcnt lgkmcnt(0)")
    e("s_barrier")

    def fma_tile(i, t):
        G, Bt = gs[i]
        if t.lo % 2 == 0:
            e(f"v_pk_fma_f32 {t[0:2]}, {G[0:2]}, {t[0:2]}, {Bt[0:2]}")
            e(f"v_pk_fma_f32 {t[2:4]}, {G[2:4]}, {t[2:4]}, {Bt[2:4]}")
        else:
            for k in range(4):
                e(f"v_fma_f32 {t[k]}, {G[k]}, {t[k]}, {Bt[k]}")

    tiles = [(i, j) for i in range(wmt) for j in range(hook.nj)]
    agpr = [t for t in tiles if acc[t].cls == "a"]
    for k in range(0, len(agpr), 2):
        pair = list(zip(agpr[k:k + 2], gx))
        for t, x in pair:
            read_tile(e, acc[t], x)
        for t, x in pair:
            fma_tile(t[0], x)
        for t, x in pair:
            for k4 in range(4):
                e(f"v_accvgpr_write_b32 {acc[t][k4]}, {x[k4]}")
    for t in tiles:
        if acc[t].cls == "v":
            fma_tile(t[0], acc[t])


def epi_pieces(hook):
    npair = hook.wmt // 2
    nd = max(hook.nj * npair - hook.epilds // 1024, 0)
    return SimpleNamespace(npair=npair, nd=nd, JH=hook.nj // 2, NRT=nd // npair)


def epi_hook(w, hook, acc, park):
    p = epi_pieces(hook)
    e = Emitter(f".Ltower{w}_ep", hook)
    r = SimpleNamespace()
    r.res, r.out, r.l2e, r.valid, r.save = e.s(2), e.s(2), e.s(2), e.s(2), e.s(2)
    (r.arith, r.act, r.couts, r.slotpix, r.ui, r.ncols, r.bs, r.nj0, r.wave_n, r.wave_m, r.col0, r.nj, r.npix, r.t0, r.t1, r.late,
     r.step, r.mylds) = (e.s() for _ in range(18))
    r.lane, r.R, r.px, r.cb, r.off, r.pxl, r.t, r.lds, r.a, r.r, r.so = (e.v() for _ in range(11))
    r.rreg = [e.v(4, 4) for _ in range(p.nd)]
    r.X, r.Y, r.RR = e.v(4, 4), e.v(4, 4), e.v(4, 4)
    r.Tm, r.U = e.v(8, 2), e.v(8, 4)

    E = hook.elem
    e(f"; ---- tower_seam.py: the epilogue (width {w}) for Mish layers with computed table entries; others take the compiled one below")
    e(f"s_load_dword {r.arith}, {E}, {hex(hook.roword)}")
    e(f"s_load_dword {r.act}, {E}, {hex(hook.act)}")
    e(f"s_load_dword {r.couts}, {E}, {hex(hook.couts)}")
    e(f"s_load_dword {r.slotpix}, {E}, {hex(hook.slotpix)}")
    e(f"s_load_dword {r.ui}, {E}, {hex(hook.ui)}")
    e(f"s_load_dwordx2 {r.res}, {E}, {hex(hook.res)}")
    e(f"s_load_dwordx2 {r.out}, {E}, {hex(hook.out)}")
    e("s_waitcnt lgkmcnt(0)")
    e(f"s_cmp_eq_u32 {r.arith}, 0")
    e(f"s_cbranch_scc1 {e.at('compiled')}")
    e(f"s_cmp_eq_u32 {r.arith}, 3")
    e(f"s_cbranch_scc1 {e.at('done')}")
    epi_geometry(e, hook, park, r)
    e(f"s_cmp_eq_u64 {r.res}, 0")
    e(f"s_cbranch_scc1 {e.at('tiles_nores')}")
    epi_request_residual(e, hook, p, r)
    epi_wait_ladder(e, hook, p, r)
    kinds = (("mish", hook.mish), ("relu", hook.relu), ("identity", hook.identity))
    for with_res in (True, False):
        e.label("tiles" if with_res else "tiles_nores")
        tags = {kind: ("r" if with_res else "n") + kind for kind, _ in kinds}
        for kind, code in kinds[1:]:
            e(f"s_cmp_eq_u32 {r.act}, {code}")
            e(f"s_cbranch_scc1 {e.at(tags[kind])}")
        for kind, _ in kinds:
            if kind != "mish":
                e.label(tags[kind])
            epi_tiles(e, hook, p, acc, r, with_res, kind)
    e.label("done")
    e.lines.extend(far_jump(f"tower{w}_seam"))
    e.label("compiled")
    return e.lines


def epi_geometry(e, hook, park, r):
    e(f"v_and_b32_e32 {r.lane}, 63, {hook.tid}")
    e(f"v_lshrrev_b32_e32 {r.R}, 4, {r.lane}")
    e(f"v_and_b32_e32 {r.px}, 15, {r.lane}")
    wave_geometry(e, r, r.ui, park.wave, r.t0)
    e(f"s_mul_i32 {r.npix}, {r.bs}, {r.bs}")
    e(f"s_mul_i32 {r.t0}, {r.wave_m}, {hook.wmt * 16}")
    e(f"v_lshl_add_u32 {r.cb}, {r.R}, 3, {r.t0}")
    e(f"s_lshl_b32 {r.t1}, {r.col0}, 4")
    e(f"v_add_u32_e32 {r.pxl}, {r.t1}, {r.px}")
    e(f"s_mul_i32 {r.t0}, {park.wg}, {r.slotpix}")
    e(f"v_add_u32_e32 {r.off}, {r.t0}, {r.pxl}")
    e(f"v_mul_lo_u32 {r.off}, {r.off}, {r.couts}")
    e(f"v_add_u32_e32 {r.off}, {r.off}, {r.cb}")
    e(f"v_lshlrev_b32_e32 {r.off}, 1, {r.off}")
    e(f"s_lshl_b32 {r.step}, {r.couts}, 5")
    e(f"s_mul_i32 {r.mylds}, {park.wave}, {hook.epilds}")
    e(f"v_lshlrev_b32_e32 {r.lds}, 4, {r.lane}")
    e(f"v_add_u32_e32 {r.lds}, {r.mylds}, {r.lds}")
    e(f"s_mov_b32 {r.l2e[0]}, 0x3fb8aa3b")
    e(f"s_mov_b32 {r.l2e[1]}, 0x3fb8aa3b")


def epi_request_residual(e, hook, p, r):
    e("s_waitcnt lgkmcnt(0)")
    e("s_barrier")

    def tile_offset(j):
        e(f"v_add_u32_e32 {r.t}, {16 * j}, {r.pxl}")
        e(f"v_cmp_gt_u32_e32 vcc, {r.npix}, {r.t}")
        e(f"s_mul_i32 {r.t0}, {r.step}, {j}")
        e(f"v_add_u32_e32 {r.a}, {r.t0}, {r.off}")

    for j in (j for j in range(hook.nj) if not p.JH <= j < p.JH + p.NRT):
        e(f"s_cmp_le_u32 {r.nj}, {j}")
        e(f"s_cbranch_scc1 {e.at('lds_issued')}")
        tile_offset(j)
        for pr in range(p.npair):
            if pr:
                e(f"v_add_u32_e32 {r.a}, 64, {r.a}")
            e(f"v_cndmask_b32_e32 {r.r}, 0, {r.a}, vcc")
            e(f"s_add_u32 {r.t1}, {r.mylds}, {lds_slot(j, pr, p) * 1024}")
            e(f"s_mov_b32 m0, {r.t1}")
            e("s_nop 1")
            e(f"global_load_lds_dwordx4 {r.r}, {r.res}")
    e.label("lds_issued")
    for k in range(p.nd):
        j, pr = p.JH + k // p.npair, k % p.npair
        if pr == 0:
            e(f"s_cmp_le_u32 {r.nj}, {j}")
            e(f"s_cbranch_scc1 {e.at('reg_issued')}")
            tile_offset(j)
        else:
            e(f"v_add_u32_e32 {r.a}, 64, {r.a}")
        e(f"v_cndmask_b32_e32 {r.r}, 0, {r.a}, vcc")
        e(f"global_load_dwordx4 {r.rreg[k]}, {r.r}, {r.res}")
    e.label("reg_issued")


def epi_wait_ladder(e, hook, p, r):
    e(f"s_sub_i32 {r.late}, {r.nj}, {p.JH}")
    e(f"s_max_i32 {r.late}, {r.late}, 0")
    for t in range(hook.nj - p.JH + 1):
        e(f"s_cmp_eq_u32 {r.late}, {t}")
        e(f"s_cbranch_scc1 {e.at(f'late{t}')}")
    e(f"s_branch {e.at('late0')}")
    for t in range(hook.nj - p.JH, -1, -1):
        e.label(f"late{t}")
        e(f"s_waitcnt vmcnt({t * p.npair})")
        e(f"s_branch {e.at('tiles')}")


def act8(e, r, kind, x_pairs, h):
    if kind == "mish":
        t = [r.Tm[2 * k:2 * k + 2] for k in range(4)]
        u = [r.U[2 * k:2 * k + 2] for k in range(4)]
        for k in range(4):
            e(f"v_pk_mul_f32 {t[k]}, {x_pairs[k]}, {r.l2e}")
        for k in range(8):
            e(f"v_exp_f32_e32 {r.Tm[k]}, {r.Tm[k]}")
        for k in range(4):
            e(f"v_pk_add_f32 {u[k]}, {t[k]}, 2.0 op_sel_hi:[1,0]")
        for k in range(4):
            e(f"v_pk_fma_f32 {t[k]}, {t[k]}, {u[k]}, 2.0 op_sel_hi:[1,1,0]")
        for k in range(8):
            e(f"v_rcp_f32_e32 {r.Tm[k]}, {r.Tm[k]}")
        for k in range(4):
            e(f"v_pk_fma_f32 {t[k]}, {t[k]}, -2.0, 1.0 op_sel_hi:[1,0,0]")
        for k in range(4):
            e(f"v_pk_mul_f32 {x_pairs[k]}, {x_pairs[k]}, {t[k]}")
    elif kind == "relu":
        for x in (x for pair in x_pairs for x in pair):
            e(f"v_cmp_lt_f32_e32 vcc, 0, {x}")
            e(f"v_cndmask_b32_e32 {x}, 0, {x}, vcc")
    for k in range(4):
        e(f"v_cvt_pk_f16_f32 {h[k]}, {x_pairs[k][0]}, {x_pairs[k][1]}")


def epi_tiles(e, hook, p, acc, r, with_res, kind):
    Hs = [r.U[0:4], r.U[4:8]]
    nstore = 0
    for j in range(hook.nj):
        e(f"s_cmp_le_u32 {r.nj}, {j}")
        e(f"s_cbranch_scc1 {e.at('done')}")
        if j == p.JH and with_res:
            e("s_waitcnt vmcnt(0)")
        e(f"v_add_u32_e32 {r.t}, {16 * j}, {r.pxl}")
        e(f"v_cmp_gt_u32_e64 {r.valid}, {r.npix}, {r.t}")
        e(f"s_mul_i32 {r.t0}, {r.step}, {j}")
        e(f"v_add_u32_e32 {r.so}, {r.t0}, {r.off}")
        for pr in range(p.npair):
            in_lds = not (p.JH <= j < p.JH + p.NRT)
            rr = r.RR
            if with_res and in_lds:
                e(f"ds_read_b128 {r.RR}, {r.lds} offset:{lds_slot(j, pr, p) * 1024}")
            elif with_res:
                rr = r.rreg[(j - p.JH) * p.npair + pr]
            xa, xb = read_tile(e, acc[(2 * pr, j)], r.X), read_tile(e, acc[(2 * pr + 1, j)], r.Y)
            if with_res:
                if in_lds:
                    e("s_waitcnt lgkmcnt(0)")
                for q, x in enumerate([*xa, *xb]):
                    e(f"v_fma_mix_f32 {x}, {rr[q // 2]}, 1.0, {x} op_sel:[{q & 1},0,0] op_sel_hi:[1,0,0]")
            h = Hs[nstore & 1]
            nstore += 1
            act8(e, r, kind, [xa[0:2], xa[2:4], xb[0:2], xb[2:4]], h)
            e(f"s_and_saveexec_b64 {r.save}, {r.valid}")
            e(f"global_store_dwordx4 {r.so}, {h}, {r.out}" + (f" offset:{64 * pr}" if pr else ""))
            e(f"s_mov_b64 exec, {r.save}")
    e(f"s_branch {e.at('done')}")



def fc_body_edits(ix, fc, w, hook):
    lines, edits = ix.lines, {}
    for k in ix.body(fc):
        if lines[k].strip() == "s_endpgm":
            edits[k] = far_jump(f"tower{w}_se_return")
        elif is_instruction(lines[k]):
            edits[k] = [rename_vgprs(lines[k], hook.freev)]
    edits[fc["begin"]] = [lines[fc["begin"]], f"tower{w}_body_fc:", "\t; ---- compiled body (FCs of the SE unit), VGPRs renamed by tower_seam.py"]
    return edits


def entry_edits(ix, conv, w, hook, park, opt):
    disp, body_conv = f"tower{w}_dispatch", f"tower{w}_body_conv"
    place = ([f"\t.p2align {opt.align}"] if opt.align else []) + (["\ts_nop 0"] * (opt.pad // 4))
    entry = [f"\t; ---- tower_seam.py: entry stub (table {park.tab}, workgroup {park.wg}, wave {park.wave}, has_se {park.has_se})",
             f"\ts_load_dwordx2 {park.tab}, s[0:1], 0x0",
             f"\ts_mov_b32 {park.wg}, s2",
             f"\tv_readfirstlane_b32 {park.wave}, v0",
             "\ts_nop 0",
             f"\ts_lshr_b32 {park.wave}, {park.wave}, 6",
             "\ts_waitcnt lgkmcnt(0)",
             f"{disp}:",
             f"\ts_load_dword {park.has_se}, {park.tab}, {hex(hook.hasse)}",
             "\ts_mov_b64 exec, -1",
             f"\ts_mov_b32 s0, {park.tab[0]}",
             f"\ts_mov_b32 s1, {park.tab[1]}",
             f"\ts_mov_b32 s2, {park.wg}",
             "\tv_mbcnt_lo_u32_b32 v0, -1, 0",
             "\tv_mbcnt_hi_u32_b32 v0, -1, v0",
             f"\tv_lshl_or_b32 v0, {park.wave}, 6, v0",
             "\ts_waitcnt lgkmcnt(0)",
             f"\ts_branch {body_conv}"] + place + [
             f"{body_conv}:",
             "\t; ---- compiled body (convolution: K loop, hook, epilogue)"]
    return {conv["begin"]: [ix.lines[conv["begin"]]] + entry}


def seam_edits(ends, w, hook, park, opt):
    seam, done = f".Ltower{w}_seam", f".Ltower{w}_done"
    tail = [f"{seam}:",
            f"tower{w}_seam:",
            "\ts_waitcnt vmcnt(0) lgkmcnt(0)",
            f"\ts_load_dword s4, {park.tab}, {hex(hook.last)}",
            "\ts_waitcnt lgkmcnt(0)",
            "\ts_barrier"]
    if opt.inv:
        tail.append("\tbuffer_inv sc1")
    tail += ["\ts_sleep 127"] * (opt.sleep // 127) + ([f"\ts_sleep {opt.sleep % 127}"] if opt.sleep % 127 else [])
    tail += ["\ts_cmp_lg_u32 s4, 0",
             f"\ts_cbranch_scc1 {done}",
             f"\ts_add_u32 {park.tab[0]}, {park.tab[0]}, {hook.stride}",
             f"\ts_addc_u32 {park.tab[1]}, {park.tab[1]}, 0"] + far_jump(f"tower{w}_dispatch") + [
             f"{done}:",
             "\ts_endpgm"]
    edits = {k: [f"\ts_branch {seam}"] for k in ends}
    edits[ends[-1]] = edits[ends[-1]] + tail
    return edits


def resource_edits(ix, conv, hook, park):
# ... 66 lines not shown
```

Baseline: 74650.

## Reorder board pixels so edge tiles let 3x3 conv skip zero-padding MFMAs

Adds an edge-first slot-to-pixel permutation for 17-19 boards so that some 16-pixel tiles hold only border pixels, whose out-of-board taps are all zero. The board conv mainloop then skips those MFMA taps via a scalar skip mask, and the load and epilogue paths (including the generated tower seam assembly) map slots back to real pixel addresses through per-tile packed words. This aims to cut wasted matrix work on padding. In exchange it adds scalar branches around MFMAs, extra address arithmetic in the epilogue, and a larger tower layer stride.

```diff
diff --git a/include/sayuri_hip.h b/include/sayuri_hip.h
--- a/include/sayuri_hip.h
+++ b/include/sayuri_hip.h
@@ -148,6 +148,8 @@
                               const float* w1, const float* b1, const float* w2, const float* b2, int chain, const float* x,
                               float* y);
 int sayuri_hip_test_last_tower_run(int out[3]);
+int sayuri_hip_test_last_edge_layers(void);
+int sayuri_hip_test_edge_map(int board_size, int n, int* slot_pixel, int* pixel_slot, int* tile_words);
 int sayuri_hip_test_conv_sx(int device, int n, const int* board_sizes, int max_board, int channels, int se_size, int act,
                             const float* x, const float* w, const float* bias, const float* res, const float* w1,
                             const float* b1, const float* w2, const float* b2, float* y);
diff --git a/sayuri_amd/_lib.py b/sayuri_amd/_lib.py
--- a/sayuri_amd/_lib.py
+++ b/sayuri_amd/_lib.py
@@ -75,6 +75,8 @@
     "sayuri_hip_test_last_se_form": (_I, []),
     "sayuri_hip_test_tower_run": (_I, [_I] * 2 + [_IP] + [_I] * 4 + [_IP, _IP, _F, _F, _I, _I] + [_F] * 4 + [_I, _F, _F]),
     "sayuri_hip_test_last_tower_run": (_I, [_IP]),
+    "sayuri_hip_test_last_edge_layers": (_I, []),
+    "sayuri_hip_test_edge_map": (_I, [_I, _I, _IP, _IP, _IP]),
     "sayuri_hip_test_conv_sx": (_I, [_I] * 2 + [_IP] + [_I] * 4 + [_F] * 9),
     "sayuri_hip_test_last_sx_kts": (_I, []),
     "sayuri_hip_test_head_board": (_I, [_I] * 2 + [_IP] + [_I] * 8 + [_F] * 5 + [_W12] + _OUT),
diff --git a/sayuri_amd/csrc/hip/conv_board.h b/sayuri_amd/csrc/hip/conv_board.h
--- a/sayuri_amd/csrc/hip/conv_board.h
+++ b/sayuri_amd/csrc/hip/conv_board.h
@@ -17,6 +17,70 @@
 __host__ __device__ constexpr int board_row_channel(int row) {
     return (row & ~31) + 8 * ((row & 15) >> 2) + 4 * ((row >> 4) & 1) + (row & 3);
 }
+
+__host__ __device__ constexpr bool board_edge_size(int bs) { return bs >= 17 && bs <= 19; }
+__host__ __device__ constexpr bool board_edge_member(int bs, int pixel) {
+    const int y = pixel / bs, x = pixel - y * bs, ncols = (bs * bs + 15) / 16, used = bs * bs - 16 * (ncols - 1);
+    return (y == 0 && x < 16) || (x == 0 && y >= 1 && y <= 16) || (x == bs - 1 && y >= bs - 17 && y <= bs - 2) ||
+           (y == bs - 1 && x >= bs - used);
+}
+__host__ __device__ constexpr int board_edge_pixel(int bs, int slot) {
+    const int npix = bs * bs, ncols = (npix + 15) / 16, used = npix - 16 * (ncols - 1), r0 = 16 * (ncols - 2);
+    if (!board_edge_size(bs) || slot < 0 || slot >= npix) return slot;
+    if (slot < 16) return slot;
+    if (slot < 32) return (slot - 15) * bs;
+    if (slot >= r0 + 16) return npix - used + (slot - r0 - 16);
+    if (slot >= r0) return (bs - 17 + slot - r0) * bs + bs - 1;
+    int k = slot - 32;
+    for (int p = 0; p < npix; ++p)
+        if (!board_edge_member(bs, p) && k-- == 0) return p;
+    return -1;
+}
+__host__ __device__ constexpr int board_edge_slot(int bs, int pixel) {
+    const int npix = bs * bs, ncols = (npix + 15) / 16, used = npix - 16 * (ncols - 1), r0 = 16 * (ncols - 2);
+    if (!board_edge_size(bs) || pixel < 0 || pixel >= npix) return pixel;
+    const int y = pixel / bs, x = pixel - y * bs;
+    if (y == 0 && x < 16) return x;
+    if (x == 0 && y >= 1 && y <= 16) return 15 + y;
+    if (x == bs - 1 && y >= bs - 17 && y <= bs - 2) return r0 + y - (bs - 17);
+    if (y == bs - 1 && x >= bs - used) return r0 + 16 + x - (bs - used);
+    int k = 32;
+    for (int p = 0; p < pixel; ++p)
+        if (!board_edge_member(bs, p)) ++k;
+    return k;
+}
+struct BoardSlotTab { unsigned w[kBoardCols]; };
+__host__ __device__ constexpr int board_slot_pixel(unsigned word, int px, int bs) {
+    return (int)(word & 0x3ffu) + ((word >> 20 & 1u) ? px * bs : px) + (px >= (int)(word >> 10 & 31u) ? 1 : 0) + (px >= (int)(word >> 15 & 31u) ? 1 : 0);
+}
+constexpr BoardSlotTab board_slot_tab(int bs, bool edge) {
+    BoardSlotTab tab{};
+    for (int t = 0; t < kBoardCols; ++t) tab.w[t] = (unsigned)(t * 16) | 16u << 10 | 16u << 15;
+    if (!edge || !board_edge_size(bs)) return tab;
+    const int npix = bs * bs, ncols = (npix + 15) / 16;
+    int pix[kBoardPT] = {};
+    for (int s = 0; s < npix; ++s)
+        if (s < 32 || s >= 16 * (ncols - 2)) pix[s] = board_edge_pixel(bs, s);
+    for (int p = 0, s = 32; p < npix; ++p)
+        if (!board_edge_member(bs, p)) pix[s++] = p;
+    for (int t = 0; t < ncols; ++t) {
+        const int n = npix - t * 16 < 16 ? npix - t * 16 : 16;
+        const bool strided = n > 1 && pix[t * 16 + 1] - pix[t * 16] == bs;
+        unsigned th[2] = {16, 16};
+        int nth = 0;
+        for (int px = 1; px < n; ++px)
+            for (int extra = pix[t * 16 + px] - pix[t * 16 + px - 1] - (strided ? bs : 1); extra > 0 && nth < 2; --extra) th[nth++] = (unsigned)px;
+        tab.w[t] = (unsigned)pix[t * 16] | th[0] << 10 | th[1] << 15 | (strided ? 1u << 20 : 0u);
+    }
+    return tab;
+}
+constexpr bool board_slot_tab_spot(int bs) {
+    const BoardSlotTab t = board_slot_tab(bs, true);
+    const int ncols = (bs * bs + 15) / 16;
+    return board_slot_pixel(t.w[0], 15, bs) == 15 && board_slot_pixel(t.w[1], 15, bs) == 16 * bs && board_slot_pixel(t.w[2], 0, bs) == board_edge_pixel(bs, 32) &&
+           board_slot_pixel(t.w[ncols - 2], 15, bs) == (bs - 2) * bs + bs - 1 && board_slot_pixel(t.w[ncols - 1], 0, bs) == 16 * (ncols - 1);
+}
+static_assert(board_slot_tab_spot(17) && board_slot_tab_spot(18) && board_slot_tab_spot(19), "board_slot_tab against board_edge_pixel");
 
 struct BoardParams {
     ConvParams c;
@@ -30,6 +94,8 @@
     const void* w_next;
     int w_ready;
     int row_order;
+    int edge;
+    unsigned slot_tab[kBoardCols];
 };
 
 struct BoardPack {
@@ -179,6 +245,30 @@
     else mma_vgpr(acc, a, b);
 }
 
+template <int WMT, int I, int J, int B0, int B1 = -1>
+__device__ __forceinline__ void mma_tile_unless(f32x4& acc, const f16x8& a, const f16x8& b, unsigned mask) {
+    if constexpr (B1 < 0) {
+        if constexpr (WMT * J + I < 32)
+            asm volatile("s_bitcmp1_b32 %3, %4\n\ts_cbranch_scc1 .Lmma_skip%=\n\tv_mfma_f32_16x16x32_f16 %0, %1, %2, %0\n.Lmma_skip%=:"
+                         : "+a"(acc) : "v"(a), "v"(b), "s"(mask), "n"(B0) : "scc");
+        else
+            asm volatile("s_bitcmp1_b32 %3, %4\n\ts_cbranch_scc1 .Lmma_skip%=\n\tv_mfma_f32_16x16x32_f16 %0, %1, %2, %0\n.Lmma_skip%=:"
+                         : "+v"(acc) : "v"(a), "v"(b), "s"(mask), "n"(B0) : "scc");
+    } else {
+        if constexpr (WMT * J + I < 32)
+            asm volatile("s_bitcmp1_b32 %3, %4\n\ts_cbranch_scc1 .Lmma_skip%=\n\ts_bitcmp1_b32 %3, %5\n\ts_cbranch_scc1 .Lmma_skip%=\n\t"
+                         "v_mfma_f32_16x16x32_f16 %0, %1, %2, %0\n.Lmma_skip%=:"
+                         : "+a"(acc) : "v"(a), "v"(b), "s"(mask), "n"(B0), "n"(B1) : "scc");
+        else
+            asm volatile("s_bitcmp1_b32 %3, %4\n\ts_cbranch_scc1 .Lmma_skip%=\n\ts_bitcmp1_b32 %3, %5\n\ts_cbranch_scc1 .Lmma_skip%=\n\t"
+                         "v_mfma_f32_16x16x32_f16 %0, %1, %2, %0\n.Lmma_skip%=:"
+                         : "+v"(acc) : "v"(a), "v"(b), "s"(mask), "n"(B0), "n"(B1) : "scc");
+    }
+}
+constexpr int kSkipTopLeft = 0;
+constexpr int skip_right_bit(int j) { return 4 + j; }
+constexpr int skip_bottom_bit(int j) { return 16 + j; }
+
 __device__ __forceinline__ void glds16_s(uint32_t voff, const void* sbase, uint32_t lds_dst) {
     unsigned keep;
     asm volatile("s_mov_b32 %0, m0\n\ts_mov_b32 m0, %3\n\ts_nop 4\n\tglobal_load_lds_dwordx4 %1, %2\n\ts_mov_b32 m0, %0"
@@ -200,7 +290,7 @@
 
 template <int WMT, bool DBG = false, int CHAIN = 0>
 __device__ __forceinline__ void board_mainloop(const BoardParams& bp, unsigned char* smem, f32x4 (&acc)[WMT][kBoardNJ], int tile,
-                                               int kt, int wave, int lane, int col0, bool full, int bs,
+                                               int kt, int wave, int lane, int col0, int nj, int bs,
                                                unsigned long long* dbg = nullptr,
                                                const __attribute__((address_space(4))) BoardParams* chain = nullptr) {
     using Cfg = BoardCfg<WMT>;
@@ -213,6 +303,9 @@
     const int wave_m = wave & 3;
     const int kg = lane >> 4;
     const int ls16 = (bs + 2) * 16;
+    const bool full = nj == NJ;
+    unsigned skipmask = 0;
+    if (bp.arith && bp.edge) skipmask = wave < 4 ? 1u << kSkipTopLeft : 1u << skip_right_bit(nj - 2) | 1u << skip_bottom_bit(nj - 1);
 
     const unsigned char* gin0 = (const unsigned char*)p.in - kZeroPrefix;
     const unsigned char* gw = (const unsigned char*)p.w;
@@ -250,11 +343,16 @@
             const bool in = q < nbinstr && r >= 1 && r <= bs && xc >= 1 && xc <= bs;
             src[i] = in ? tile * p.g.slot_pix + (r - 1) * bs + (xc - 1) : -1;
         }
+        unsigned words[NJ];
+#pragma unroll
+        for (int j = 0; j < NJ; ++j) words[j] = bp.slot_tab[col0 + j];
+#pragma unroll
+        for (int j = 0; j < NJ; ++j) asm volatile("" : "+s"(words[j]));
 #pragma unroll
         for (int j = 0; j < NJ; ++j) {
-            const int px = (col0 + j) * 16 + (lane & 15);
-            const int y = (int)(((float)px + 0.5f) * r_bs), x = px - y * bs;
-            lp[j] = px < npix ? (y + 1) * w2 + x + 1 : w2 + 1;
+            const int px = board_slot_pixel(words[j], lane & 15, bs);
+            const int y = (int)(((float)px + 0.5f) * r_bs);
+            lp[j] = (col0 + j) * 16 + (lane & 15) < npix ? px + 2 * y + w2 + 1 : w2 + 1;
         }
     } else {
 #pragma unroll
@@ -349,11 +447,14 @@
                 static_for<WMT>([&](auto ic) {
                     constexpr int i = decltype(ic)::value;
                     if constexpr (j == 0 && dx > 0) wait_lgkm2<WMT - i>(afr[i], bfr[b % 3]);
+                    constexpr bool right = j >= 7 && j <= 9 && dx == 2, bottom = j >= 8 && j <= 10 && row == 2;
                     if constexpr (j == NJ - 1) {
                         if (full) mma_tile<WMT, i, j>(acc[i][j], afr[i], bfr[b % 3]);
-                    } else {
-                        mma_tile<WMT, i, j>(acc[i][j], afr[i], bfr[b % 3]);
-                    }
+                    } else if constexpr ((j == 0 && row == 0) || (j == 1 && dx == 0)) mma_tile_unless<WMT, i, j, kSkipTopLeft>(acc[i][j], afr[i], bfr[b % 3], skipmask);
+                    else if constexpr (right && bottom) mma_tile_unless<WMT, i, j, skip_right_bit(j), skip_bottom_bit(j)>(acc[i][j], afr[i], bfr[b % 3], skipmask);
+                    else if constexpr (right) mma_tile_unless<WMT, i, j, skip_right_bit(j)>(acc[i][j], afr[i], bfr[b % 3], skipmask);
+                    else if constexpr (bottom) mma_tile_unless<WMT, i, j, skip_bottom_bit(j)>(acc[i][j], afr[i], bfr[b % 3], skipmask);
+                    else mma_tile<WMT, i, j>(acc[i][j], afr[i], bfr[b % 3]);
                     if constexpr (j == NJ - 1 && dx < 2)
                         board_read_a<(dx + 1) * Cfg::A_TAP_BYTES + i * 256>(afr[i], abase);
                 });
@@ -433,11 +534,16 @@
         constexpr int JH = NJ / 2, NRT = ND / NPAIR;
         auto load_orow = [&] {
             if (bp.arith) {
-                const int npix = (bp.uniform_info >> 8) * (bp.uniform_info >> 8);
+                const int bsz = bp.uniform_info >> 8, npix = bsz * bsz;
+                unsigned words[NJ];
+#pragma unroll
+                for (int j = 0; j < NJ; ++j) words[j] = bp.slot_tab[col0 + j];
+#pragma unroll
+                for (int j = 0; j < NJ; ++j) asm volatile("" : "+s"(words[j]));
 #pragma unroll
                 for (int j = 0; j < NJ; ++j) {
                     const int pxl = (col0 + j) * 16 + px;
-                    orow[j] = (j < nj && pxl < npix) ? tile * p.g.slot_pix + pxl : -1;
+                    orow[j] = (j < nj && pxl < npix) ? tile * p.g.slot_pix + board_slot_pixel(words[j], px, bsz) : -1;
                 }
             } else {
 #pragma unroll
@@ -784,7 +890,7 @@
         dbg[0] = __builtin_amdgcn_s_memtime();
     }
     f32x4 acc[WMT][kBoardNJ];
-    board_mainloop<WMT>(bp, smem, acc, tile, 0, wave, lane, col0, nj == kBoardNJ, bs);
+    board_mainloop<WMT>(bp, smem, acc, tile, 0, wave, lane, col0, nj, bs);
     if (dbg) dbg[1] = __builtin_amdgcn_s_memtime();
     board_se_stage<WMT>(sp, smem, acc, tile, wave, lane, col0, nj, bs, dbg);
     asm volatile("s_waitcnt lgkmcnt(0)" ::: "memory");
@@ -830,7 +936,7 @@
     const int nj = wave_n ? ncols - nj0 : nj0;
 
     f32x4 acc[WMT][kBoardNJ];
-    board_mainloop<WMT, DBG>(bp, smem, acc, tile, kt, wave, lane, col0, nj == kBoardNJ, bs, dbg);
+    board_mainloop<WMT, DBG>(bp, smem, acc, tile, kt, wave, lane, col0, nj, bs, dbg);
 
     switch (p.act) {
     case kMish: board_epilogue<WMT, kMish>(bp, smem, acc, tile, kt, wave, lane, col0, nj); break;
diff --git a/sayuri_amd/csrc/hip/conv_board_sx.h b/sayuri_amd/csrc/hip/conv_board_sx.h
--- a/sayuri_amd/csrc/hip/conv_board_sx.h
+++ b/sayuri_amd/csrc/hip/conv_board_sx.h
@@ -67,7 +67,7 @@
         dbg[0] = __builtin_amdgcn_s_memtime();
     }
     f32x4 acc[WMT][kBoardNJ];
-    board_mainloop<WMT>(bp, smem, acc, tile, kt, wave, lane, col0, nj == kBoardNJ, bs);
+    board_mainloop<WMT>(bp, smem, acc, tile, kt, wave, lane, col0, nj, bs);
     if (dbg) dbg[1] = __builtin_amdgcn_s_memtime();
 
     float* stage = (float*)(smem + SxLds::stage);
diff --git a/sayuri_amd/csrc/hip/conv_tower.h b/sayuri_amd/csrc/hip/conv_tower.h
--- a/sayuri_amd/csrc/hip/conv_tower.h
+++ b/sayuri_amd/csrc/hip/conv_tower.h
@@ -3,7 +3,7 @@
 
 namespace sayuri {
 
-constexpr int kTowerStride = 320;
+constexpr int kTowerStride = 384;
 
 struct alignas(16) TowerLayer {
     const TowerLayer* self;
@@ -64,7 +64,7 @@
     f32x4 acc[WMT][kBoardNJ];
     {
         const BoardParams& bp = *(const BoardParams*)&L->sp.b;
-        board_mainloop<WMT, false, 2>(bp, smem, acc, tile, 0, wave, lane, col0, nj == kBoardNJ, bs, nullptr,
+        board_mainloop<WMT, false, 2>(bp, smem, acc, tile, 0, wave, lane, col0, nj, bs, nullptr,
                                       (const __attribute__((address_space(4))) BoardParams*)&L->sp.b);
     }
     TowerLayerCP L2 = L;
@@ -72,7 +72,7 @@
     tower_anchor<WMT, 0>(acc);
     asm volatile("; TOWER_SE_HOOK elem=%0 tid=%1 wmt=%2 ui=%3 cols=%4 w1h=%5 w2h=%6 w1b=%7 w2b=%8 psum=%9 pmax=%10 gate=%11 kot=%12 "
                  "res=%13 out=%14 couts=%15 slotpix=%16 act=%17 arith=%18 mish=%19 roword=%20 relu=%21 identity=%22 "
-                 "stride=%23 last=%24 hasse=%25 freev=%26 frees=%27 nj=%28 epilds=%29 lds=%30"
+                 "stride=%23 last=%24 hasse=%25 freev=%26 frees=%27 nj=%28 epilds=%29 lds=%30 edge=%31 slottab=%32"
                  : "+s"(L2), "+v"(tid2)
                  : "n"(WMT), "n"(offsetof(TowerLayer, sp.b.uniform_info)), "n"(offsetof(TowerLayer, sp.b.tab_cols)),
                    "n"(offsetof(TowerLayer, sp.w1h)), "n"(offsetof(TowerLayer, sp.w2h)), "n"(offsetof(TowerLayer, sp.w1_bytes)),
@@ -81,7 +81,8 @@
                    "n"(offsetof(TowerLayer, sp.b.c.cout_s)), "n"(offsetof(TowerLayer, sp.b.c.g.slot_pix)), "n"(offsetof(TowerLayer, sp.b.c.act)),
                    "n"(offsetof(TowerLayer, sp.b.arith)), "n"((int)kMish), "n"(offsetof(TowerLayer, sp.b.row_order)), "n"((int)kReLU), "n"((int)kIdentity),
                    "n"(kTowerStride), "n"(offsetof(TowerLayer, last)), "n"(offsetof(TowerLayer, has_se)), "n"(kTowerFreeVgpr),
-                   "n"(kTowerFreeSgprs), "n"(kBoardNJ), "n"(kBoardWaveLds), "n"(kBoardLdsBytes)
+                   "n"(kTowerFreeSgprs), "n"(kBoardNJ), "n"(kBoardWaveLds), "n"(kBoardLdsBytes), "n"(offsetof(TowerLayer, sp.b.edge)),
+                   "n"(offsetof(TowerLayer, sp.b.slot_tab))
                  : "memory", "vcc", "scc", SAYURI_TOWER_CLOBBER_V, SAYURI_TOWER_CLOBBER_S);
     const BoardSeParams& sp = *(const BoardSeParams*)&L2->sp;
     const BoardParams& bp = sp.b;
diff --git a/sayuri_amd/csrc/hip/engine_graph.h b/sayuri_amd/csrc/hip/engine_graph.h
--- a/sayuri_amd/csrc/hip/engine_graph.h
+++ b/sayuri_amd/csrc/hip/engine_graph.h
@@ -950,6 +950,7 @@
         if (!f.chained && tower_ok(be->kot) && L.w_board && L.bias_board && board_row_order_ok(bp, be->kot, flags_.tower_gen_epi)) {
             p.w = L.w_board; p.bias = L.bias_board; bp.row_order = 1;
         }
+        if (board_edge_ok(bp, be->kot, has_se, flags_.board_edge)) board_set_edge(bp);
         if (!f.run.empty() && !(to_run && f.run_kot == be->kot) && tower_flush(f)) return -1;
         if (rows_use(f, p, name)) return -1;
         if (to_run) return tower_append(f, be->kot, sp, has_se, flops, bytes);
diff --git a/sayuri_amd/csrc/hip/engine_plan.h b/sayuri_amd/csrc/hip/engine_plan.h
--- a/sayuri_amd/csrc/hip/engine_plan.h
+++ b/sayuri_amd/csrc/hip/engine_plan.h
@@ -4,6 +4,7 @@
 static thread_local std::string g_err;
 static std::atomic<unsigned> g_host_free_gen{0};
 static thread_local int g_test_conv_kind = 0;
+static thread_local int g_test_edge_layers = 0;
 static int fail(const std::string& m) { g_err = m; return -1; }
 
 #define HIP_OK(expr)                                                                      \
@@ -124,6 +125,7 @@
     int latency_split = 0;
     bool tower_chain = true;
     bool tower_gen_epi = true;
+    bool board_edge = true;
     bool se_split = true;
     int tower_noepi_after = -1;
     unsigned dbg_sx_epoch0 = 0;
@@ -147,6 +149,7 @@
         f.tower = !off("SAYURI_TOWER");
         f.tower_chain = !off("SAYURI_TOWER_CHAIN");
         f.tower_gen_epi = !off("SAYURI_TOWER_GEN_EPI");
+        f.board_edge = !off("SAYURI_BOARD_EDGE");
         if (const char* e = getenv("SAYURI_DEBUG_RECYCLE_INPUT")) f.dbg_recycle_input = atoi(e);
         f.se_split = !off("SAYURI_SE_SPLIT");
         if (const char* e = getenv("SAYURI_SX_DBG")) f.sx_dbg = atoi(e);
@@ -380,6 +383,16 @@
     bp.npos = plan.npos;
     bp.uniform_info = plan.uniform_info;
     bp.arith = plan.single && plan.uniform_info >= 0 && arith ? 1 : 0;
+    static constexpr BoardSlotTab raster = board_slot_tab(0, false);
+    std::copy_n(raster.w, kBoardCols, bp.slot_tab);
+}
+static bool board_edge_ok(const BoardParams& bp, int kot, bool has_se, bool enabled) {
+    return enabled && !has_se && bp.arith && board_edge_size(bp.uniform_info >> 8) && board_uses_row_order(kot) && bp.c.ko_pad <= 2 * kot;
+}
+static void board_set_edge(BoardParams& bp) {
+    static constexpr BoardSlotTab tabs[3] = {board_slot_tab(17, true), board_slot_tab(18, true), board_slot_tab(19, true)};
+    bp.edge = 1;
+    std::copy_n(tabs[(bp.uniform_info >> 8) - 17].w, kBoardCols, bp.slot_tab);
 }
 static bool board_row_order_ok(const BoardParams& bp, int kot, bool gen_epi) {
     const ConvParams& p = bp.c;
diff --git a/sayuri_amd/csrc/hip/engine_taps.h b/sayuri_amd/csrc/hip/engine_taps.h
--- a/sayuri_amd/csrc/hip/engine_taps.h
+++ b/sayuri_amd/csrc/hip/engine_taps.h
@@ -89,6 +89,7 @@
 static int test_conv_impl(int device, int n, const int* board_sizes, int max_board, int cin, int cout, int k,
                           int depthwise, int act, int post_residual, const float* x, const float* w, const float* bias,
                           const float* res, float* y) {
+    g_test_edge_layers = 0;
     HIP_OK(hipSetDevice(device));
     enable_big_lds<T>();
     if (sizeof(T) == 2 && k == 3) enable_big_lds_glds();
@@ -126,6 +127,8 @@
             board_params(bp, plan, tabs.src, tabs.pix, tabs.cols, true);
             conv_params(bp.c, dx, dw, db, dres, dy, tg.g, cin_s, cout_s, ko_pad, 9, act);
             bp.c.npos = 0; bp.c.num_pix_tiles = plan.ntiles;
+            if (board_edge_ok(bp, r.board->kot, false, EngineFlags::from_env().board_edge)) board_set_edge(bp);
+            g_test_edge_layers = bp.edge;
             hipLaunchKernelGGL(r.board->fn, dim3(plan.ntiles * r.tiles), dim3(512), r.board->lds(plan.npos), 0, bp);
         } else if (r.glds) {
             const float* dz = (const float*)A.alloc(256);
@@ -359,6 +362,7 @@
                                const int* res_from, const float* w, const float* bias, const TestSeUnit& se, int chain, const float* x, float* y) {
     typedef f16 T;
     g_test_tower_run[0] = g_test_tower_run[1] = g_test_tower_run[2] = 0;
+    g_test_edge_layers = 0;
     g_test_se_form = 0;
     if (C != 128 && C != 256) return fail("test_tower_run: the run's channels are a channel tile of the tower kernel, 128 or 256");
     if (nlayers < 1 || nlayers > 8) return fail("test_tower_run: 1 to 8 layers");
@@ -408,7 +412,7 @@
     }
     std::vector<TowerLayer> run;
     size_t w_off = 0;
-    int row_ordered = 0;
+    int row_ordered = 0, edge_layers = 0;
     for (int l = 0; l < nlayers; ++l) {
         const int cin = l ? C : cin0, cin_s = l ? C : cin0_s;
         const bool unit = l == se.layer;
@@ -422,6 +426,8 @@
         p.npos = 0; p.num_pix_tiles = plan.ntiles;
         bp.row_order = board_row_order_ok(bp, be->kot, flags.tower_gen_epi) ? 1 : 0;
         row_ordered += bp.row_order;
+        if (board_edge_ok(bp, be->kot, unit, flags.board_edge)) board_set_edge(bp);
+        edge_layers += bp.edge;
         const std::vector<T> img = conv_image<T>(w + w_off, cin, C, 9, ko_pad);
         const std::vector<float> hb = padded_bias(bias + (size_t)l * C, C, ko_pad);
         w_off += (size_t)C * cin * 9;
@@ -449,6 +455,7 @@
     if (load_tower_module(&mod, fn)) return -1;
     if (has_unit) g_test_se_form = staged ? 1 : 2;
     g_test_tower_run[0] = nlayers; g_test_tower_run[1] = row_ordered; g_test_tower_run[2] = links;
+    g_test_edge_layers = edge_layers;
     const TowerLayer* arg = dt;
     void* params[] = {(void*)&arg};
     hipError_t rc = hipModuleLaunchKernel(fn[be->kot == 256 ? 0 : 1], plan.ntiles, 1, 1, 512, 1, 1, 0, nullptr, params, nullptr);
@@ -590,6 +597,19 @@
     return 0;
 }
 
+extern "C" int sayuri_hip_test_last_edge_layers(void) { return sayuri::g_test_edge_layers; }
+extern "C" int sayuri_hip_test_edge_map(int board_size, int n, int* slot_pixel, int* pixel_slot, int* tile_words) {
+    if (board_size < 2 || board_size > 19 || n != board_size * board_size || !slot_pixel || !pixel_slot || !tile_words)
+        return sayuri::fail("test_edge_map: bad argument");
+    for (int i = 0; i < n; ++i) {
+        slot_pixel[i] = sayuri::board_edge_pixel(board_size, i);
+        pixel_slot[i] = sayuri::board_edge_slot(board_size, i);
+    }
+    const sayuri::BoardSlotTab tab = sayuri::board_slot_tab(board_size, true);
+    for (int t = 0; t < sayuri::kBoardCols; ++t) tile_words[t] = (int)tab.w[t];
+    return 0;
+}
+
 extern "C" int sayuri_hip_test_last_sx_kts(void) { return sayuri::g_test_sx_kts; }
 
 extern "C" int sayuri_hip_test_head_board(int device, int n, const int* board_sizes, int max_board, int channels, int policy_channels,
diff --git a/sayuri_amd/csrc/hip/tower_seam.py b/sayuri_amd/csrc/hip/tower_seam.py
--- a/sayuri_amd/csrc/hip/tower_seam.py
+++ b/sayuri_amd/csrc/hip/tower_seam.py
@@ -16,7 +16,7 @@
 
 HOOK_KEYS = ("elem", "tid", "wmt", "ui", "cols", "w1h", "w2h", "w1b", "w2b", "psum", "pmax", "gate", "kot", "res", "out", "couts",
              "slotpix", "act", "arith", "mish", "relu", "identity", "roword",
-             "stride", "last", "hasse", "freev", "frees", "nj", "epilds", "lds")
+             "stride", "last", "hasse", "freev", "frees", "nj", "epilds", "lds", "edge", "slottab")
 
 
 def die(msg):
@@ -234,13 +234,14 @@
 
 
 def choose_parked(w, conv, fc, fv, hook):
-    B = (max(conv["sgprs"], fc["sgprs"]) + 1) & ~1
+    B = max(conv["sgprs"], fc["sgprs"], hook.frees + 2)
     if B + 5 > 102:
         die(f"width {w}: no five SGPRs left above the compiler's {B}")
-    B = max(B, hook.frees + 2)
     if conv["accum"] < hook.freev + fv + 1:
         die(f"width {w}: accum_offset {conv['accum']} below the FC body's renamed VGPRs")
     s = Reg("s", B, 5)
+    if B % 2:
+        return SimpleNamespace(all=s, has_se=s[0], tab=s[1:3], wg=s[3], wave=s[4])
     return SimpleNamespace(all=s, tab=s[0:2], wg=s[2], wave=s[3], has_se=s[4])
 
 
@@ -539,8 +540,10 @@
     r = SimpleNamespace()
     r.res, r.out, r.l2e, r.valid, r.save = e.s(2), e.s(2), e.s(2), e.s(2), e.s(2)
     (r.arith, r.act, r.couts, r.slotpix, r.ui, r.ncols, r.bs, r.nj0, r.wave_n, r.wave_m, r.col0, r.nj, r.npix, r.t0, r.t1, r.late,
-     r.step, r.mylds) = (e.s() for _ in range(18))
-    r.lane, r.R, r.px, r.cb, r.off, r.pxl, r.t, r.lds, r.a, r.r, r.so = (e.v() for _ in range(11))
+     r.rowb, r.mylds, r.t2) = (e.s() for _ in range(19))
+    r.strided = e.s(2)
+    r.words = [w for quad in (e.s(4, keep=True) for _ in range((hook.nj + 3) // 4)) for w in quad][:hook.nj]
+    r.lane, r.R, r.px, r.cb, r.off, r.pxl, r.t, r.lds, r.a, r.r, r.so, r.pxbs = (e.v() for _ in range(12))
     r.rreg = [e.v(4, 4) for _ in range(p.nd)]
     r.X, r.Y, r.RR = e.v(4, 4), e.v(4, 4), e.v(4, 4)
     r.Tm, r.U = e.v(8, 2), e.v(8, 4)
@@ -581,25 +584,49 @@
     return e.lines
 
 
+def epi_slot_words(e, hook, park, r):
+    e(f"s_lshl_b32 {r.t0}, {r.col0}, 2")
+    e(f"s_add_u32 {r.l2e[0]}, {hook.elem[0]}, {r.t0}")
+    e(f"s_addc_u32 {r.l2e[1]}, {hook.elem[1]}, 0")
+    for k in range(0, hook.nj, 4):
+        e(f"s_load_dwordx4 {Reg('s', r.words[k].lo, 4)}, {r.l2e}, {hex(hook.slottab + 4 * k)}")
+
+
+def tile_pixel(e, r, j, dst):
+    w = r.words[j]
+    e(f"s_bitcmp1_b32 {w}, 20")
+    e(f"s_cselect_b64 {r.strided}, -1, 0")
+    e(f"s_and_b32 {r.t0}, {w}, 0x3ff")
+    e(f"s_bfe_u32 {r.t1}, {w}, 0x5000a")
+    e(f"s_bfe_u32 {r.t2}, {w}, 0x5000f")
+    e(f"v_cndmask_b32_e64 {dst}, {r.px}, {r.pxbs}, {r.strided}")
+    e(f"v_add_u32_e32 {dst}, {r.t0}, {dst}")
+    for t in (r.t1, r.t2):
+        e(f"v_cmp_le_u32_e32 vcc, {t}, {r.px}")
+        e(f"v_addc_co_u32_e32 {dst}, vcc, 0, {dst}, vcc")
+
+
 def epi_geometry(e, hook, park, r):
     e(f"v_and_b32_e32 {r.lane}, 63, {hook.tid}")
     e(f"v_lshrrev_b32_e32 {r.R}, 4, {r.lane}")
     e(f"v_and_b32_e32 {r.px}, 15, {r.lane}")
     wave_geometry(e, r, r.ui, park.wave, r.t0)
+    epi_slot_words(e, hook, park, r)
     e(f"s_mul_i32 {r.npix}, {r.bs}, {r.bs}")
     e(f"s_mul_i32 {r.t0}, {r.wave_m}, {hook.wmt * 16}")
     e(f"v_lshl_add_u32 {r.cb}, {r.R}, 3, {r.t0}")
     e(f"s_lshl_b32 {r.t1}, {r.col0}, 4")
     e(f"v_add_u32_e32 {r.pxl}, {r.t1}, {r.px}")
+    e(f"v_mul_u32_u24_e32 {r.pxbs}, {r.bs}, {r.px}")
     e(f"s_mul_i32 {r.t0}, {park.wg}, {r.slotpix}")
-    e(f"v_add_u32_e32 {r.off}, {r.t0}, {r.pxl}")
-    e(f"v_mul_lo_u32 {r.off}, {r.off}, {r.couts}")
-    e(f"v_add_u32_e32 {r.off}, {r.off}, {r.cb}")
+    e(f"s_mul_i32 {r.t0}, {r.t0}, {r.couts}")
+    e(f"v_add_u32_e32 {r.off}, {r.t0}, {r.cb}")
     e(f"v_lshlrev_b32_e32 {r.off}, 1, {r.off}")
-    e(f"s_lshl_b32 {r.step}, {r.couts}, 5")
+    e(f"s_lshl_b32 {r.rowb}, {r.couts}, 1")
     e(f"s_mul_i32 {r.mylds}, {park.wave}, {hook.epilds}")
     e(f"v_lshlrev_b32_e32 {r.lds}, 4, {r.lane}")
     e(f"v_add_u32_e32 {r.lds}, {r.mylds}, {r.lds}")
+    e("s_waitcnt lgkmcnt(0)")
     e(f"s_mov_b32 {r.l2e[0]}, 0x3fb8aa3b")
     e(f"s_mov_b32 {r.l2e[1]}, 0x3fb8aa3b")
 
@@ -609,10 +636,10 @@
     e("s_barrier")
 
     def tile_offset(j):
+        tile_pixel(e, r, j, r.a)
+        e(f"v_mad_u32_u24 {r.a}, {r.a}, {r.rowb}, {r.off}")
         e(f"v_add_u32_e32 {r.t}, {16 * j}, {r.pxl}")
         e(f"v_cmp_gt_u32_e32 vcc, {r.npix}, {r.t}")
-        e(f"s_mul_i32 {r.t0}, {r.step}, {j}")
-        e(f"v_add_u32_e32 {r.a}, {r.t0}, {r.off}")
 
     for j in (j for j in range(hook.nj) if not p.JH <= j < p.JH + p.NRT):
         e(f"s_cmp_le_u32 {r.nj}, {j}")
@@ -689,8 +716,8 @@
             e("s_waitcnt vmcnt(0)")
         e(f"v_add_u32_e32 {r.t}, {16 * j}, {r.pxl}")
         e(f"v_cmp_gt_u32_e64 {r.valid}, {r.npix}, {r.t}")
-        e(f"s_mul_i32 {r.t0}, {r.step}, {j}")
-        e(f"v_add_u32_e32 {r.so}, {r.t0}, {r.off}")
+        tile_pixel(e, r, j, r.so)
+        e(f"v_mad_u32_u24 {r.so}, {r.so}, {r.rowb}, {r.off}")
         for pr in range(p.npair):
             in_lds = not (p.JH <= j < p.JH + p.NRT)
             rr = r.RR
```

After: 73390. -1.7%, worse.
